# ictnlp/StreamSpeech

Measured on AMD Instinct MI355X. Metric: real-time factor (RTFx = audio seconds / wall seconds) + utterances/sec, offline S2ST fr-en, higher is better.
Workload: dtype f32

## Files before the change

### include/streamspeech_hip.h

```cpp
#ifndef STREAMSPEECH_HIP_H
#define STREAMSPEECH_HIP_H

#include <stddef.h>
#include <stdint.h>

#ifdef __cplusplus
extern "C" {
#endif

#define SS_ABI_VERSION 2

typedef struct ss_model ss_model;
typedef struct ss_vocoder ss_vocoder;
typedef struct ss_scratch ss_scratch;
typedef struct ss_stream_pool ss_stream_pool;

typedef struct ss_config {
  int32_t input_feat, conv_channels, conv_kernel;
  int32_t enc_dim, enc_ffn, enc_heads, enc_layers, dw_kernel;
  int32_t src_vocab, tgt_vocab;
  int32_t mt_layers, dec_dim, dec_ffn, dec_heads;
  int32_t t2u_layers, unit_layers, unit_vocab, ctc_upsample;
  int32_t pad, eos, unk;
  int32_t max_rel_pos;
// ... 155 lines not shown
int ss_flac_unpack(const uint8_t* h_data, size_t n_bytes, int64_t cap, int32_t* h_res, ss_flac_subframe* h_rec, int64_t res_cap,
                   ss_flac_info* h_info);
int ss_flac_restore_host(const int32_t* h_res, const ss_flac_subframe* h_rec, int64_t n_rec, const ss_flac_file* h_files, int n_files,
                         int mono, float* h_out, int32_t* h_pcm);
int ss_flac_restore(void* stream, const int32_t* d_res, const ss_flac_subframe* d_rec, int64_t n_rec, int64_t n_res,
                    const ss_flac_file* h_files, int n_files, int mono, float* d_out, int64_t out_floats,
                    void* d_work, size_t* work_bytes);

enum { SS_PCM_F32LE = 0, SS_PCM_S16LE = 1, SS_PCM_ULAW = 2, SS_PCM_ALAW = 3 };

typedef struct ss_pcm_seg {
  int64_t src_offset;
  int64_t dst_offset;
  int32_t frames;
  int32_t fmt, channels, dst;
} ss_pcm_seg;

int ss_pcm_scatter(void* stream, const void* d_stage, int64_t stage_bytes, const ss_pcm_seg* h_segs, int n_segs,
                   float* const* h_dst, const int64_t* h_dst_cap, int n_dst);
int ss_pcm_pack_s16(void* stream, const float* d_src, int64_t n, int16_t* d_out);
int ss_pcm_decode_host(const void* h_src, int fmt, int channels, int64_t frames, float* h_dst);
int ss_pcm_pack_s16_host(const float* h_src, int64_t n, int16_t* h_out);

typedef struct ss_pcm_emit_seg {
  float* carry;
  const float* tail;
  const float* taps;
  int64_t n_before;
  int64_t k0, k1;
  int64_t out_offset;
  int32_t carry_len;
  int32_t n_new;
  int32_t up, down, half;
  int32_t fmt;
  int32_t finished;
  int32_t reserved;
} ss_pcm_emit_seg;

int64_t ss_pcm_emit_count(int64_t n, int up, int down, int half, int finished);
int ss_pcm_emit(void* stream, const ss_pcm_emit_seg* h_segs, int n_segs, void* d_out, int64_t out_bytes);
int ss_pcm_emit_host(const ss_pcm_emit_seg* h_segs, int n_segs, void* h_out, int64_t out_bytes);
int ss_pcm_encode_host(const float* h_src, int64_t n, int fmt, void* h_out);

enum { SS_VAD_IDLE = 0, SS_VAD_SPEECH = 1 };
enum { SS_VAD_START = 1, SS_VAD_END = 2, SS_VAD_FORCED = 4 };

typedef struct ss_vad_state {
  int64_t onset;
  int64_t last_speech;
  int64_t utt_first_frame;
  float floor;
  int32_t mode;
  int32_t run;
  int32_t reserved;
} ss_vad_state;

typedef struct ss_vad_seg {
  const float* hist;
  ss_vad_state* state;
  float* powers;
  int64_t hist_first;
  int64_t n_hist;
  int64_t first_frame;
  int32_t n_frames;
  int32_t H, W;
  float p_abs, p_min, snr, rise;
  int32_t min_speech, end_silence, post_roll, max_frames;
  int32_t reserved;
} ss_vad_seg;

typedef struct ss_vad_result {
  int64_t consumed;
  int64_t start_frame;
  int64_t cut_sample;
  int64_t last_speech;
  int32_t events;
  int32_t mode;
} ss_vad_result;

int ss_vad_scan(void* stream, const ss_vad_seg* h_segs, int n_segs, ss_vad_result* d_results);
int ss_vad_scan_host(const ss_vad_seg* h_segs, int n_segs, ss_vad_result* h_results);

int ss_row_max_logprob(void* stream, const float* d_logits, int rows, int vocab, int mask0, int mask1, int mask2,
                       float* d_out);

int ss_log_softmax(void* stream, const float* d_logits, int rows, int vocab, int mask0, int mask1, int as_probs,
                   float* d_out);

int ss_encoder_out_len(int T);
int ss_encoder_forward(ss_model* m, void* stream, const float* d_fbank, int T, int attn_chunk,
                       int conv_chunk, float* d_enc_out);

int ss_encoder_stream_reset(ss_model* m);
int ss_encoder_stream_set_tail(ss_model* m, int unsettled_fbank_frames);
int ss_encoder_stream_forward(ss_model* m, void* stream, const float* d_fbank, int T, int attn_chunk,
                              int conv_chunk, float* d_enc_out, int32_t* n_final, int32_t* n_computed);
int ss_encoder_stream_set_deferred(ss_model* m, int on);
int ss_encoder_stream_status(ss_model* m, void* stream, int32_t* repeat);

int ss_stream_pool_create(ss_model* m, int max_sessions, int max_rows, ss_stream_pool** out);
void ss_stream_pool_destroy(ss_stream_pool* p);
int ss_stream_pool_reset(ss_stream_pool* p, int slot);
int ss_stream_pool_set_tail(ss_stream_pool* p, int slot, int unsettled_fbank_frames);
int ss_encoder_stream_forward_batch(ss_model* m, void* stream, ss_stream_pool* p, int n, const int32_t* h_slots,
                                    const float* const* h_fbank, const int32_t* h_T, const int32_t* h_attn_chunk,
                                    const int32_t* h_conv_chunk, float* d_enc_packed, int32_t* h_n_final, int32_t* h_n_computed);
int ss_stream_pool_ctc(ss_model* m, void* stream, ss_stream_pool* p, int head, int n, const int32_t* h_slots,
                       const float* d_enc_packed, int32_t* d_raw, int32_t* d_tokens, int32_t* d_index, int32_t* d_counts);
int ss_stream_pool_set_scores(ss_stream_pool* p, int on);
int ss_stream_pool_ctc_scored(ss_model* m, void* stream, ss_stream_pool* p, int head, int n, const int32_t* h_slots,
                              const float* d_enc_packed, int32_t* d_raw, int32_t* d_tokens, int32_t* d_index, int32_t* d_counts,
                              float* d_lprob, int32_t* d_last, float* d_tok_lprob);
int ss_stream_pool_stats(ss_stream_pool* p, int64_t* launches, int64_t* head_rows);

int ss_ctc_greedy(ss_model* m, void* stream, int head, const float* d_enc_out, int Tp,
                  int32_t* d_raw, int32_t* d_tokens, int32_t* d_index, int32_t* d_count,
                  float* d_logits);

int ss_ctc_greedy_scored(ss_model* m, void* stream, int head, const float* d_enc_out, int Tp,
                         int32_t* d_raw, int32_t* d_tokens, int32_t* d_index, int32_t* d_count,
                         float* d_logits, float* d_lprob, int32_t* d_last, float* d_tok_lprob);

int ss_mt_set_persistent(ss_model* m, int workgroups);
int ss_mt_get_persistent(ss_model* m);

int ss_mt_begin(ss_model* m, void* stream, const float* d_enc_out, int Tp);
int ss_mt_append(ss_model* m, void* stream, const int32_t* d_tokens, int n, int pos0, int ban_eos,
                 int force_eos, float* d_feats, int32_t* d_next, int n_tail_pad);
int ss_mt_greedy(ss_model* m, void* stream, const float* d_enc_out, int Tp, const int32_t* h_prefix,
                 int n_prefix, int max_len, int min_len, int32_t* h_out_tokens, int* h_n_out,
                 float* d_feats, int* h_n_feats);
int ss_mt_truncate(ss_model* m, int len);

int ss_t2u_units(ss_model* m, void* stream, const float* d_mt_feats, int n, int t2u_causal,
                 int mask_eos, int32_t* d_raw, int32_t* d_tokens, int32_t* d_count, float* d_logits,
                 int n_tail_pad);

int ss_vocoder_create(const ss_vocoder_config* cfg, const float* d_blob, size_t blob_floats,
                      const char* const* names, const int64_t* offsets, const int64_t* numels,
                      int n_slots, ss_vocoder** out);
void ss_vocoder_destroy(ss_vocoder* v);
int ss_vocoder_set_bf16x3(ss_vocoder* v, int on);
int ss_vocoder_set_f16(ss_vocoder* v, int on);
int ss_vocoder_forward(ss_vocoder* v, void* stream, const int32_t* d_codes, int K, int dur_prediction,
                       const int32_t* d_forced_dur, float* d_wav, int64_t wav_capacity,
                       int32_t* d_dur, int64_t* h_n_samples);
int ss_vocoder_num_speakers(const ss_vocoder* v);
int ss_vocoder_forward_spkr(ss_vocoder* v, void* stream, const int32_t* d_codes, int K, int dur_prediction,
                            const int32_t* d_forced_dur, float* d_wav, int64_t wav_capacity,
                            int32_t* d_dur, int64_t* h_n_samples, int32_t spkr);

int ss_batch_fbank_cmvn(ss_model* m, void* stream, int B, const float* d_pcm, const int64_t* h_pcm_start,
                        const int32_t* h_n_samples, float pcm_scale, float* d_feat, int32_t* h_T);
int ss_batch_cmvn(ss_model* m, void* stream, const float* d_in, int64_t rows, float* d_out);
int ss_batch_encoder_forward(ss_model* m, void* stream, int B, const float* d_fbank, const int32_t* h_T,
                             int attn_chunk, int conv_chunk, float* d_enc_out, int32_t* h_Tp);
int ss_batch_ctc_greedy(ss_model* m, void* stream, int head, int B, const float* d_enc_out,
                        const int32_t* h_Tp, int32_t* d_raw, int32_t* d_tokens, int32_t* d_index,
                        int32_t* d_counts);
int ss_batch_ctc_greedy_scored(ss_model* m, void* stream, int head, int B, const float* d_enc_out,
                               const int32_t* h_Tp, int32_t* d_raw, int32_t* d_tokens, int32_t* d_index,
                               int32_t* d_counts, float* d_lprob, int32_t* d_last, float* d_tok_lprob);
typedef struct ss_ctc_align_result {
  double score;
  double viterbi;
  int32_t status;
  int32_t n_tokens;
} ss_ctc_align_result;
#define SS_CTC_ALIGN_MAX_FRAMES 1500
#define SS_CTC_ALIGN_MAX_LABELS 1500
int ss_batch_ctc_align(ss_model* m, void* stream, int head, int B, const float* d_enc_out, const int32_t* h_Tp,
                       const int32_t* h_targets, const int32_t* h_n_targets, ss_ctc_align_result* d_results, int32_t* d_path,
                       int32_t* d_first, int32_t* d_last, float* d_tok_lprob);
int ss_ctc_align_host(const float* h_logits, int ld, int V, int pad, int B, const int32_t* h_T, const int32_t* h_targets,
                      const int32_t* h_n_targets, ss_ctc_align_result* h_results, int32_t* h_path, int32_t* h_first, int32_t* h_last,
                      float* h_tok_lprob, float* h_frame_lprob);
int ss_batch_mt_greedy(ss_model* m, void* stream, int B, const float* d_enc_out, const int32_t* h_Tp,
                       const int32_t* h_max_len, int min_len, int32_t* h_out_tokens, int out_stride,
                       int32_t* h_n_out, float* d_feats, int feat_rows);
int ss_batch_mt_beam(ss_model* m, void* stream, int B, int beam, const float* d_enc_out, const int32_t* h_Tp,
                     const int32_t* h_max_len, int min_len, float unk_penalty, int normalize, int32_t* h_out_tokens,
                     int out_stride, int32_t* h_n_out, float* h_scores, float* h_pos_scores, float* d_feats, int feat_rows);
int ss_batch_mt_continue(ss_model* m, void* stream, int B, const float* d_enc_out, const int32_t* h_Tp, const int32_t* h_prefix,
                         const int32_t* h_n_prefix, const int32_t* h_max_len, int min_len, int32_t* h_out_tokens, int out_stride,
                         int32_t* h_n_out, float* d_feats, int feat_rows, int32_t* h_n_feats);
int ss_batch_mt_continue_plan(int B, const int32_t* h_Tp, const int32_t* h_prefix, const int32_t* h_n_prefix, const int32_t* h_max_len,
                              int min_len, int out_stride, int feat_rows, int max_tgt_pos, int vocab, int eos, int32_t* h_dims,
                              int32_t* h_tables, int64_t tables_cap, int64_t* h_n_tables);
int ss_batch_mt_beam_continue(ss_model* m, void* stream, int B, int beam, const float* d_enc_out, const int32_t* h_Tp,
                              const int32_t* h_prefix, const int32_t* h_n_prefix, const int32_t* h_max_len, int min_len,
                              float unk_penalty, int normalize, int32_t* h_out_tokens, int out_stride, int32_t* h_n_out,
                              float* h_scores, float* h_pos_scores, float* d_feats, int feat_rows);
int ss_batch_mt_beam_continue_plan(int B, int beam, const int32_t* h_Tp, const int32_t* h_prefix, const int32_t* h_n_prefix,
                                   const int32_t* h_max_len, int min_len, int out_stride, int feat_rows, int max_tgt_pos, int vocab,
                                   int eos, int pad, int32_t* h_dims, int32_t* h_tables, int64_t tables_cap, int64_t* h_n_tables);
typedef struct ss_mt_search_opts {
  int32_t size;
  int32_t no_repeat_ngram;
  float len_penalty;
  float temperature;
} ss_mt_search_opts;
int ss_batch_mt_beam_opts(ss_model* m, void* stream, int B, int beam, const float* d_enc_out, const int32_t* h_Tp,
                          const int32_t* h_max_len, int min_len, float unk_penalty, int normalize, int32_t* h_out_tokens,
                          int out_stride, int32_t* h_n_out, float* h_scores, float* h_pos_scores, float* d_feats, int feat_rows,
                          const ss_mt_search_opts* opts);
int ss_batch_mt_beam_continue_opts(ss_model* m, void* stream, int B, int beam, const float* d_enc_out, const int32_t* h_Tp,
                                   const int32_t* h_prefix, const int32_t* h_n_prefix, const int32_t* h_max_len, int min_len,
                                   float unk_penalty, int normalize, int32_t* h_out_tokens, int out_stride, int32_t* h_n_out,
                                   float* h_scores, float* h_pos_scores, float* d_feats, int feat_rows,
                                   const ss_mt_search_opts* opts);
int ss_batch_mt_beam_continue_plan_opts(int B, int beam, const int32_t* h_Tp, const int32_t* h_prefix, const int32_t* h_n_prefix,
                                        const int32_t* h_max_len, int min_len, int out_stride, int feat_rows, int max_tgt_pos,
                                        int vocab, int eos, int pad, int32_t* h_dims, int32_t* h_tables, int64_t tables_cap,
                                        int64_t* h_n_tables, const ss_mt_search_opts* opts);
typedef struct ss_mt_sample_opts {
  int32_t size;
  int32_t topk;
  float topp;
  int32_t reserved;
  uint64_t seed;
} ss_mt_sample_opts;
int ss_batch_mt_sample(ss_model* m, void* stream, int B, int beam, const float* d_enc_out, const int32_t* h_Tp,
                       const int32_t* h_max_len, int min_len, float unk_penalty, int normalize, int32_t* h_out_tokens, int out_stride,
                       int32_t* h_n_out, float* h_scores, float* h_pos_scores, float* d_feats, int feat_rows,
                       const ss_mt_search_opts* opts, const int64_t* h_keys, const ss_mt_sample_opts* sample);
int ss_batch_mt_sample_continue(ss_model* m, void* stream, int B, int beam, const float* d_enc_out, const int32_t* h_Tp,
                                const int32_t* h_prefix, const int32_t* h_n_prefix, const int32_t* h_max_len, int min_len,
                                float unk_penalty, int normalize, int32_t* h_out_tokens, int out_stride, int32_t* h_n_out,
                                float* h_scores, float* h_pos_scores, float* d_feats, int feat_rows, const ss_mt_search_opts* opts,
                                const int64_t* h_keys, const ss_mt_sample_opts* sample);
int ss_batch_fbank_frames(ss_model* m, void* stream, int B, const float* const* h_pcm, const int32_t* h_first, const int32_t* h_n,
                          float pcm_scale, float* const* h_feat);
int ss_batch_fbank_frames_sr(ss_model* m, void* stream, int B, const float* const* h_pcm, const int32_t* h_n_in, const int32_t* h_up,
                             const int32_t* h_down, const float* const* h_taps, const int32_t* h_half_len, const int32_t* h_first,
                             const int32_t* h_n, float pcm_scale, float* const* h_feat);
int ss_fbank_sr_rows(int64_t n_in, int up, int down, int half_len, int32_t* h_n_rows, int32_t* h_n_final);
int ss_fbank_mel_ranges(const float* h_melw, int rows, int cols, int32_t* h_lo_hi);
int ss_batch_t2u_units(ss_model* m, void* stream, int B, const float* d_feats, int feat_rows,
                       const int32_t* h_n, int t2u_causal, int mask_eos, int32_t* d_raw, int32_t* d_tokens,
                       int32_t* d_counts);
int ss_batch_vocoder_forward(ss_vocoder* v, void* stream, int B, const int32_t* d_codes, const int32_t* h_K,
                             int dur_prediction, const int32_t* d_forced_dur, float* d_wav,
                             int64_t wav_capacity, int32_t* d_dur, int64_t* h_wav_start,
                             int64_t* h_n_samples);
int ss_batch_vocoder_forward_spkr(ss_vocoder* v, void* stream, int B, const int32_t* d_codes, const int32_t* h_K,
                                  int dur_prediction, const int32_t* d_forced_dur, float* d_wav,
                                  int64_t wav_capacity, int32_t* d_dur, int64_t* h_wav_start,
                                  int64_t* h_n_samples, const int32_t* h_spkr );
int ss_batch_t2u_units_pad(ss_model* m, void* stream, int B, const float* d_feats, int feat_rows, const int32_t* h_n,
                           const int32_t* h_n_tail_pad, int t2u_causal, int mask_eos, int32_t* d_raw, int32_t* d_tokens,
                           int32_t* d_counts);
int ss_batch_mt_features(ss_model* m, void* stream, int B, const float* d_enc_out, const int32_t* h_Tp, const int32_t* h_tokens,
                         const int32_t* h_n_tokens, const int32_t* h_n_tail_pad, float* d_feats, int feat_rows);
int ss_batch_mt_attention(ss_model* m, void* stream, int B, const float* d_enc_out, const int32_t* h_Tp, const int32_t* h_tokens,
                          const int32_t* h_n_tokens, const int32_t* h_first, float* d_feats, int feat_rows, float* d_attn,
                          int64_t* h_attn_off, int64_t attn_capacity, int32_t* d_peak, float* d_stat);
int ss_batch_mt_score(ss_model* m, void* stream, int U, const float* d_enc_out, const int32_t* h_Tp, int B, const int32_t* h_src,
                      const int32_t* h_tokens, const int32_t* h_n_tokens, float* d_feats, int feat_rows, float* d_stat,
                      int32_t* d_idx);
int ss_batch_vocoder_tail(ss_vocoder* v, void* stream, int B, const int32_t* d_codes, const int32_t* h_K, const int32_t* h_n_new,
                          const int32_t* h_ctx, const int32_t* h_rf, int dur_prediction, float* d_out, int64_t out_capacity,
                          int32_t* h_win_first, int32_t* h_dur, int64_t* h_out_start, int64_t* h_n_out);
int ss_batch_vocoder_tail_spkr(ss_vocoder* v, void* stream, int B, const int32_t* d_codes, const int32_t* h_K, const int32_t* h_n_new,
                               const int32_t* h_ctx, const int32_t* h_rf, int dur_prediction, float* d_out, int64_t out_capacity,
                               int32_t* h_win_first, int32_t* h_dur, int64_t* h_out_start, int64_t* h_n_out,
                               const int32_t* h_spkr );

int ss_batch_unit_spans(ss_model* m, void* stream, int B, const int32_t* d_raw, const int32_t* h_n, const int32_t* h_K,
                        const int32_t* h_dur_first, const int32_t* h_unit0, const int32_t* d_dur, const int32_t* h_dur,
                        int32_t* h_spans, int32_t* h_K_out);
int ss_unit_spans_host(int B, const int32_t* h_raw, const int32_t* h_n, const int32_t* h_K, const int32_t* h_dur_first,
                       const int32_t* h_unit0, const int32_t* h_dur, int up, int blank, int pad, int bos, int eos, int32_t* h_spans,
                       int32_t* h_K_out);

int ss_prof_enable(int cls_mask);
int ss_prof_enable_hi(int cls_mask);
int ss_prof_reset(void);
int ss_prof_read(int cls, double* h_ms_total, double* h_flops_total, int64_t* h_launches,
                 double* h_bytes_total);
int ss_prof_totals(int cls, double* h_flops_total, double* h_bytes_total, int64_t* h_launches);
int ss_prof_read_issued(int cls, double* h_issued_flops_total);
int ss_prof_shape_log(int on);
int ss_prof_shape_dump(char* buf, int cap);
int ss_prof_num_classes(void);
const char* ss_prof_class_name(int cls);

int ss_model_set_pack_invariant(ss_model* m, int on);
int ss_model_get_pack_invariant(ss_model* m);
int ss_debug_canon(int mode);

int ss_debug_last_logits(ss_model* m, void* stream, float* d_out, int64_t cap_floats, int* h_rows, int* h_cols);

int ss_op_ffn_fused(void* stream, const float* dX, int ldx, float* dY, int ldy, const float* ln_g, const float* ln_b,
                    const float* dW1, const float* db1, const float* dW2, const float* db2, float alpha,
                    const float* ln2_g, const float* ln2_b, int M, int D, int F);
int ss_debug_ffn(int grid, int row_tiles_per_wave, int enable);
int ss_debug_rtlin(int grid, int enable);
int ss_debug_rtlin_kb(int uw, int order);
int ss_debug_rtlin_kb_last(int32_t out[4]);
int ss_debug_unit_l0_distinct(int on);
int ss_debug_fbank_dense(int dense);
int ss_debug_conv_c64(int enable);
int ss_debug_conv_c256_rows(int rows);
int ss_debug_conv_c32(int enable);
int ss_debug_conv_c16(int enable);
int64_t ss_debug_enc_step_launches(void);
int ss_op_ln_linear(void* stream, const float* dX, int ldx, const float* ln_g, const float* ln_b, const float* dW,
                    const float* dbias, const float* dR, int ldr, float* dC, int ldc, int M, int N, int K, int act, float alpha,
                    int glu);
int ss_op_ln_linear_ex(void* stream, const float* dX, int ldx, const float* ln_g, const float* ln_b, float* ln_out, const float* dW,
                       const float* dbias, const float* dR, int ldr, float* dC, int ldc, int M, int N, int K, int act, float alpha,
                       int glu, int canon);

int ss_debug_force_tile(int bm, int bn, int ks);
int ss_debug_sk_errors(void);
int ss_debug_attention_split(int v);
int ss_debug_attention_q16(int v);
int ss_debug_enc_step_inject_timeout(ss_model* m);
int ss_debug_scratch_audit(ss_scratch* sc, size_t* booked, size_t* held);
int ss_debug_mt_inject_timeout(ss_model* m);

int ss_op_conv_gemm(void* stream, const float* dA, int lda, const float* dW, const float* dbias,
                    const float* dR, int ldr, const float* dR2, int ldr2, float* dC, int ldc,
                    int M, int N, int Cin, int taps, int dil, int stride, int pad, int in_len,
                    int chunk, int in_act, float in_slope, int act, float alpha, float div, int glu);
typedef struct ss_op_conv_args {
  const float* A; const float* W; const float* bias; const float* R; const float* R2; float* C; float* C2;
  int32_t lda, ldc, ldr, ldr2, ldc2;
  int32_t M, N, Cin, taps, dil, stride, pad, in_len, chunk;
  int32_t in_act; float in_slope;
  int32_t act; float act_slope, alpha, div, c2_slope;
  int32_t glu;
  const int32_t* segs; int32_t nseg, max_seg_out;
  int32_t same_rows;
} ss_op_conv_args;
int ss_op_conv_gemm_ex(void* stream, const ss_op_conv_args* a);
int ss_op_conv_gemm_rows(void* stream, const ss_op_conv_args* a, int m_begin, const int32_t* seg_mb, const float* const* seg_A, int canon);
int ss_op_conv_pair(void* stream, const float* dA, int lda, const float* dW1, const float* db1, const float* dW2, const float* db2,
                    float* dC, int ldc, const float* dR2, int ldr2, float div, float* dC2, int ldc2, float c2_slope, int C, int taps,
                    int dil, int M, int in_len, float slope, const int32_t* d_segs, int nseg);
int ss_op_resblock_fused(void* stream, const float* dX, int ldx, const float* const* dW1, const float* const* dB1,
                         const float* const* dW2, const float* const* dB2, const int32_t* dil, float* dY, int ldy, const float* dR2,
                         int ldr2, float div, int C, int taps, int M, float slope, const int32_t* d_segs, int nseg);
int ss_debug_slab(int grid, long long min_rows);
int ss_op_conv_f16(void* stream, const float* dA, const float* dW, const float* dbias, const float* dR, const float* dR2,
                   float* dC, float* dC2, int M, int C, int taps, int dil, int in_act, float in_slope, int act, float div,
                   const int32_t* d_segs, int nseg);
int ss_op_layernorm(void* stream, const float* dx, int ldx, float* dy, int ldy, const float* dg,
                    const float* db, int M, int D, float eps);
int ss_op_attention(void* stream, const float* dQ, int ldq, const float* dK, int ldk, const float* dV,
                    int ldv, float* dO, int ldo, int Tq, int Tk, int H, float scale, int causal,
                    int chunk, const float* dP, int ldp, const float* du, const float* dv);
typedef struct ss_op_attn_args {
  const float* Q; const float* K; const float* V; float* O;
  int32_t ldq, ldk, ldv, ldo;
  int32_t Tq, Tk, H;
  float scale;
  int32_t causal, chunk, q0, k_mask_tail;
  const float* P; int32_t ldp;
  const float* bias_u; const float* bias_v;
  const int32_t* segs; int32_t nseg, max_q, p_tmax;
  const int32_t* seg_tail;
  int32_t no_decode_kernel;
  const int32_t* anc; int32_t anc_ld, anc_slots;
  int32_t use_split;
} ss_op_attn_args;
int ss_op_attention_ex(void* stream, const ss_op_attn_args* a);
typedef struct ss_op_attn_probs_args {
  const float* Q; const float* K;
  int32_t ldq, ldk, H;
  float scale;
  const int32_t* segs; int32_t nseg;
  const int32_t* q_first; const int32_t* row_off; const int64_t* p_off;
  float* P; int32_t* peak; float* stat;
  int32_t max_rows;
} ss_op_attn_probs_args;
int ss_op_attention_probs(void* stream, const ss_op_attn_probs_args* a);
typedef struct ss_op_pool_attn_args {
  const float* Qs; float* cache; float* O;
  int32_t ld, ldo, slot_rows;
  const float* P; int32_t ldp, p_tmax;
  const float* bias_u; const float* bias_v;
  const int32_t* sess; const int32_t* qt_pre;
  int32_t nsess, qtiles, H;
  float scale;
} ss_op_pool_attn_args;
int ss_op_attention_pool(void* stream, const ss_op_pool_attn_args* a);
int ss_debug_attention_no_mfma(int v);
int ss_op_dwconv_bn_silu(void* stream, const float* dx, int ldx, float* dy, int ldy, const float* dwt,
                         int K, const float* mean, const float* var, const float* gamma,
                         const float* beta, float eps, int T, int C, int chunk);
int ss_op_dwconv_bn_silu_ex(void* stream, const float* dx, int ldx, float* dy, int ldy, const float* dwt, int K, const float* mean,
                            const float* var, const float* gamma, const float* beta, float eps, int T, int C, int chunk,
                            const int32_t* segs, int nseg, int t_begin);
int ss_op_pool_dwconv(void* stream, const float* gs, float* cache, int slot_rows, float* y, const float* wt, int K, const float* bn_mean,
                      const float* bn_var, const float* bn_gamma, const float* bn_beta, float bn_eps, int C, const int32_t* sess,
                      int nsess, int max_n);
int ss_op_pool_gather_rows(void* stream, float* out, const float* stk, float* cache, int slot_rows, int W, const int32_t* tab,
                           const int32_t* pre, int nsess, int total);
int ss_op_pool_gather_ids(void* stream, int32_t* out, const int32_t* stk, int32_t* cache, int slot_rows, const int32_t* tab,
                          const int32_t* pre, int nsess, int total);
int ss_op_pool_stack_rows(void* stream, float* out, const float* enc, int W, const int32_t* src, const int32_t* pre, int nsess,
                          int total);

int ss_op_masked_argmax(void* stream, const float* logits, int ld, int M, int N, int mask0, int mask1, int mask2, int force,
                        int32_t* ids, const int32_t* row_max_len, int step, int force_id, const int32_t* row_min_len, int ban_id);
int ss_op_ctc_collapse(void* stream, const int32_t* raw, int T, int blank, int pad, int32_t* tokens, int32_t* index, int32_t* count,
                       const int32_t* segs, int nseg);
int ss_op_masked_argmax_lprob(void* stream, const float* logits, int ld, int M, int N, int mask0, int mask1, int mask2, int32_t* ids,
                              float* lprob);
int ss_op_ctc_collapse_spans(void* stream, const int32_t* raw, const float* lprob, int T, int blank, int pad, int32_t* tokens,
                             int32_t* index, int32_t* last, float* tok_lprob, int32_t* count, const int32_t* segs, int nseg);
int ss_op_mt_token_scores(void* stream, const float* d_logits, int ld, int rows, int V, const int32_t* d_target, float* d_stat,
                          int32_t* d_idx);
int ss_debug_mt_score_form(int force_strided);
int ss_op_ctc_align(void* stream, const float* d_logits, int ld, int V, int pad, int B, const int32_t* h_T, const int32_t* h_targets,
                    const int32_t* h_n_targets, ss_ctc_align_result* d_results, int32_t* d_path, int32_t* d_first, int32_t* d_last,
                    float* d_tok_lprob, float* d_frame_lprob);
int ss_op_unit_spans(void* stream, int B, const int32_t* d_raw, const int32_t* h_n, const int32_t* h_K, const int32_t* h_dur_first,
                     const int32_t* h_unit0, const int32_t* d_dur, int up, int blank, int pad, int bos, int eos, int32_t* d_spans,
                     int32_t* d_K_out);
int ss_op_dur_predict(void* stream, const float* logdur, const int32_t* forced, int K, int32_t* dur, int32_t* cum,
                      const int32_t* segs, int nseg);
int ss_op_repeat_rows(void* stream, const float* emb, const int32_t* cum, int K, int D, float* out, int F, const int32_t* segs,
                      int nseg);
int ss_op_embed_tokens(void* stream, const int32_t* tok, const float* emb, const float* pos_table, float scale, int pos0, float* out,
                       int n, int D, int pos_stride, int pad_id, int vocab);
int ss_op_embed_tokens_rows(void* stream, const int32_t* tok, const float* emb, const float* pos_table, int pos_rows, float scale,
                            int pos0, const int32_t* row_pos, float* out, int n, int D, int pad_id, int vocab);
int ss_op_upsample_add_pos(void* stream, const float* src, int n, int up, const float* pos_row, float pad_value, float* out, int D);
int ss_op_gather_rows(void* stream, const int32_t* idx, const float* table, int D, float* out, int n, int rows);
int ss_op_scatter_rows(void* stream, const int32_t* dst_row, const float* src, int lds, float* dst, int ldd, int D, int n,
                       int dst_rows);
int ss_op_conv_post_tanh(void* stream, const float* x, int T, int C, const float* w, const float* bias, float slope, float* wav,
                         const int32_t* segs, int nseg);
int ss_op_conv_post_tanh_crop(void* stream, const float* x, int C, const float* w, const float* bias, float slope, float* wav,
                              const int32_t* segs, int nseg, int max_keep);
int ss_op_spkr_pre_add(void* stream, const float* x, float* y, int ld, int C0, const float* table, const int32_t* spkr, int spkr0,
                       const int32_t* segs, int nseg, int max_seg_out, int M, int act, float slope);

#define SS_OP_BEAM_CAND 64
int ss_op_beam_topk(void* stream, const float* logits, int R, int V, int k, int t_step, int min_len, const int32_t* max_len,
                    const int32_t* npre, const int32_t* done, const float* cum, int pad, int unk, int eos, float unk_pen,
                    float* cand_s, int32_t* cand_t);
typedef struct ss_op_beam_state {
  int32_t* tok; float* cum; int32_t* anc; float* cand_s; int32_t* cand_t; int32_t* ignore; int32_t* done; int32_t* max_len;
  int32_t* npre;
  int32_t* fin_cnt; float* fin_score; int32_t* fin_len; int32_t* fin_tok; float* fin_pos; int32_t* fin_anc;
} ss_op_beam_state;
int ss_op_beam_merge(void* stream, const ss_op_beam_state* st, int B, int k, int Lc, int V, int t_step, int c0, int eos,
                     int normalize);
int ss_op_beam_prefix_score(void* stream, const float* logits, int rows, int V, const int32_t* ftok, int pad, int unk, float unk_pen,
                            float* lp);
int ss_op_beam_prefix_chain(void* stream, const float* lp, const int32_t* row0, const int32_t* npre, int B, int k, float* cum0,
                            float* pos);
int ss_op_beam_topk_opts(void* stream, const float* logits, int R, int V, int k, int t_step, int min_len, const int32_t* max_len,
                         const int32_t* npre, const int32_t* done, const float* cum, int pad, int unk, int eos, float unk_pen,
                         float* cand_s, int32_t* cand_t, float temperature, int no_repeat_ngram, const int32_t* tok,
                         const int32_t* anc, int Lc, int c0, const int32_t* ptok, const int32_t* row0, float* row_scores);
int ss_op_beam_merge_opts(void* stream, const ss_op_beam_state* st, int B, int k, int Lc, int V, int t_step, int c0, int eos,
                          int normalize, float len_penalty);
int ss_op_beam_prefix_score_opts(void* stream, const float* logits, int rows, int V, const int32_t* ftok, int pad, int unk,
                                 float unk_pen, float* lp, float temperature);
int ss_op_sample_step(void* stream, const float* logits, int R, int V, int t_step, int min_len, const int32_t* max_len,
                      const int32_t* npre, int pad, int unk, int eos, float unk_pen, float temperature, int no_repeat_ngram,
                      const int32_t* tok, const int32_t* anc, int Lc, int c0, const int32_t* ptok, const int32_t* row0,
                      const int32_t* row_j, const int64_t* keys, const ss_mt_sample_opts* sample, int32_t* out_tok, float* out_score,
                      float* out_u, int32_t* out_kept);
int ss_op_sample_uniform(void* stream, int n, const uint64_t* seed, const int64_t* key, const int32_t* step, const int32_t* j,
                         float* u, uint32_t* words);

#ifdef __cplusplus
}
#endif
#endif
```

### streamspeech_amd/csrc/conv_c64w.hip

```cpp
#include "slab_common.hpp"

#include <type_traits>

namespace ss {

using u32x4 = __attribute__((ext_vector_type(4))) unsigned;

#ifndef CW_TIMING
#define CW_TIMING 0
#endif
#if CW_TIMING
__device__ unsigned long long g_cw_dbg[1024 * 8];
#define CW_STAMP(k) do { if (t == 0) { const unsigned long long _n = __builtin_amdgcn_s_memtime(); cw_acc[k] += _n - cw_last; cw_last = _n; } } while (0)
#else
#define CW_STAMP(k) do { } while (0)
#endif

namespace {
constexpr int CW_MAXSEG = 256;
constexpr int CW_MAXROWS = 320;
constexpr int CW_MAXROWS_128 = 192;
[[maybe_unused]] constexpr int CW_NUM_RECORDS = 0x7ffffff0;
constexpr int cw_bme(int dil, int rows = 256) { return rows == 128 ? (dil == 1 ? 128 : dil == 3 ? 126 : 120) : (dil == 1 ? 256 : dil == 3 ? 252 : 240); }
[[maybe_unused]] __host__ __device__ constexpr int cw_nc(int kind) { return kind == 0 ? 4 : kind == 1 ? 2 : 3; }
// ... 43 lines not shown
  const int t = threadIdx.x, lane = t & 63;
  const int wave = __builtin_amdgcn_readfirstlane((t >> 6) & (ROWS == 128 ? 1 : 3));
  const int cs = CH <= 64 ? 0 : __builtin_amdgcn_readfirstlane(ROWS == 128 ? t >> 7 : t >> 8);
  const int colh = CH == 256 && ROWS == 256 ? (int)((blockIdx.x >> 3) & 1) : 0;
  const int col0 = colh * 128 + cs * 64;
  const int r = lane & 15, g = lane >> 4;
  const int Kw = groups * 4 * C;

  SlabWalk<GemmArgs> w(p, s_blk, BME);
  __syncthreads();
  const int nblocks = w.nblocks();
  const float slope = p.in_act == ACT_LRELU ? p.in_slope : 1.0f;

  const __amdgpu_buffer_rsrc_t rsW = __builtin_amdgcn_make_buffer_rsrc((void*)p.W, 0, CW_NUM_RECORDS, 0x00020000);
  const int vo = (r * Kw + 4 * g) * 4;
  auto wload = [&](int idx, int cc, int ct, int kh) -> f32x4 {
    const int so = __builtin_amdgcn_readfirstlane(((col0 + ct * 16) * Kw + idx * C + kh * CS + cc * 16) * 4);
    const u32x4 v = __builtin_amdgcn_raw_buffer_load_b128(rsW, vo, so, 0);
    return f32x4{__uint_as_float(v[0]), __uint_as_float(v[1]), __uint_as_float(v[2]), __uint_as_float(v[3])};
  };

  constexpr bool HALVES = CH == 256 && ROWS == 256;
  int blk = HALVES ? (int)((blockIdx.x & 7) + 8 * (blockIdx.x >> 4)) : (int)blockIdx.x;
  const int blk_stride = HALVES ? (int)(gridDim.x >> 1) : (int)gridDim.x;
  if (blk >= nblocks) return;
  f32x4 ring[RING];
#pragma unroll
  for (int q = 0; q < RING; ++q) ring[q] = wload(q / CT, 0, q % CT, 0);

  int toff[2];
  bool pv[2];
#pragma unroll
  for (int i = 0; i < 2; ++i) {
    const int pp = wave * 32 + i * 16 + r;
    pv[i] = pp < NPAIR;
    const int pc = pv[i] ? pp : NPAIR - 1;
    toff[i] = 2 * DIL * (pc / DIL) + pc % DIL;
  }

#if CW_TIMING
  unsigned long long cw_acc[4] = {0, 0, 0, 0}, cw_last = __builtin_amdgcn_s_memtime(), cw_begin = cw_last, cw_blocks = 0;
#endif
  for (; blk < nblocks; blk += blk_stride) {
#if CW_TIMING
    ++cw_blocks;
#endif
    w.locate(blk, p.in_len);
    const int m0 = w.m0, seg_lo = w.seg_lo, seg_hi = w.seg_hi;
    const int m_hi = p.nseg > 0 ? seg_hi : min(seg_hi, p.M);
    const bool edge = (m0 - p.pad < seg_lo) || (m0 - p.pad + slab_rows > seg_hi);
    const int row_hi = ROWS == 128 ? min(seg_hi, m0 - p.pad + slab_rows) : seg_hi;
    f32x4 acc[4][2][CT];
#pragma unroll
    for (int f = 0; f < 4; ++f)
#pragma unroll
      for (int i = 0; i < 2; ++i)
#pragma unroll
        for (int j = 0; j < CT; ++j) acc[f][i][j] = f32x4{0.f, 0.f, 0.f, 0.f};
#pragma unroll 1
    for (int kh = 0; kh < KH; ++kh) {
    const int kh_wrap = kh + 1 < KH ? kh + 1 : 0;
    __syncthreads();
    CW_STAMP(kh == 0 ? 3 : 1);
#pragma unroll 1
    for (int u0 = 0; u0 < NP && (ROWS != 128 || u0 * RPP < slab_rows); u0 += NPC) {
      f32x4 pre[NPC];
#pragma unroll
      for (int u = 0; u < NPC; ++u) {
        const int rho = t / TPR + RPP * (u0 + u);
        const int gc = min(max(m0 - p.pad + rho, seg_lo), row_hi - 1);
        pre[u] = *reinterpret_cast<const f32x4*>(p.A + (size_t)gc * p.lda + kh * CS + (t % TPR) * 4);
      }
      float* dst = sA + (t / TPR + RPP * u0) * LDA + (t % TPR) * 4;
#pragma unroll
      for (int u = 0; u < NPC; ++u) {
        const int rho = t / TPR + RPP * (u0 + u);
        f32x4 v = pre[u];
        if (edge) {
          const int gin = m0 - p.pad + rho;
          const bool ok = gin >= seg_lo && gin < seg_hi;
#pragma unroll
          for (int e = 0; e < 4; ++e) v[e] = ok ? v[e] : 0.f;
        }
#pragma unroll
        for (int e = 0; e < 4; ++e) v[e] = fmaxf(v[e], v[e] * slope);
        if (rho < slab_rows) *reinterpret_cast<f32x4*>(dst + u * RPP * LDA) = v;
      }
    }
    __syncthreads();
    CW_STAMP(0);

    const float* pa0 = sA + toff[0] * LDA + 4 * g;
    const float* pa1 = sA + toff[1] * LDA + 4 * g;
    auto rd = [&](const float* base, int j, int cc) -> f32x4 { return *reinterpret_cast<const f32x4*>(base + j * DIL * LDA + cc * 16); };
    auto xform = [&](int op, const f32x4 a, const f32x4 b) -> f32x4 { return op == 1 ? a + b : op == 0 ? a : a - b; };
    f32x4 xa[2];
    xa[0] = xform(-1, rd(pa0, 0, 0), rd(pa0, 2, 0));
    xa[1] = xform(-1, rd(pa1, 0, 0), rd(pa1, 2, 0));
    auto group = [&](auto KIND, const int grp, const int kind_next, const float* pn0, const float* pn1, const int grp_next, const int kh_next) __attribute__((always_inline)) {
      constexpr int K = decltype(KIND)::value, NC = cw_nc(K), NS = CB * NC;
      static_assert(NS % 2 == 0 && NS >= 2, "ring slots keep their parity across groups");
#pragma unroll
      for (int ss = 0; ss < NS; ++ss) {
        const int slot = cw_slot(K, ss % NC);
        f32x4 na0, nb0, na1, nb1;
        if (ss + 1 < NS) {
          const int ccn = (ss + 1) / NC, nn = (ss + 1) % NC;
          na0 = rd(pa0, cw_ja(K, nn), ccn); nb0 = rd(pa0, cw_jb(K, nn), ccn);
          na1 = rd(pa1, cw_ja(K, nn), ccn); nb1 = rd(pa1, cw_jb(K, nn), ccn);
        } else {
          const int jb = kind_next == 0 ? 2 : 1;
          na0 = rd(pn0, 0, 0); nb0 = *reinterpret_cast<const f32x4*>(pn0 + jb * (DIL * LDA));
          na1 = rd(pn1, 0, 0); nb1 = *reinterpret_cast<const f32x4*>(pn1 + jb * (DIL * LDA));
        }
        f32x4 wf[CT];
#pragma unroll
        for (int j = 0; j < CT; ++j) {
          const int q = ss * CT + j;
          wf[j] = ring[q % RING];
          const int s2 = ss + 2;
          if (s2 < NS) ring[q % RING] = wload(grp * 4 + cw_slot(K, s2 % NC), s2 / NC, j, kh);
          else ring[q % RING] = wload(grp_next * 4 + (s2 == NS ? 0 : (kind_next == 1 ? 3 : 1)), 0, j, kh_next);
        }
#pragma unroll
        for (int e = 0; e < 4; ++e)
#pragma unroll
          for (int i = 0; i < 2; ++i)
#pragma unroll
            for (int j = 0; j < CT; ++j)
              acc[slot][i][j] = __builtin_amdgcn_mfma_f32_16x16x4f32(wf[j][e], xa[i][e], acc[slot][i][j], 0, 0, 0);
        if (ss + 1 < NS) {
          xa[0] = xform(cw_op(K, (ss + 1) % NC), na0, nb0);
          xa[1] = xform(cw_op(K, (ss + 1) % NC), na1, nb1);
        } else {
          xa[0] = kind_next == 1 ? na0 : na0 - nb0;
          xa[1] = kind_next == 1 ? na1 : na1 - nb1;
        }
        __builtin_amdgcn_sched_barrier(0);
      }
    };
    constexpr int tail = TAIL;
    const int groups_full = groups - (tail ? 1 : 0);
#pragma unroll 1
    for (int grp = 0; grp < groups_full; ++grp) {
      const bool more = grp + 1 < groups;
      const float* pn0 = more ? pa0 + 3 * DIL * LDA : pa0;
      const float* pn1 = more ? pa1 + 3 * DIL * LDA : pa1;
      group(std::integral_constant<int, 0>{}, grp, (more && grp + 1 == groups_full) ? tail : 0, pn0, pn1, more ? grp + 1 : 0, more ? kh : kh_wrap);
      pa0 = pn0;
      pa1 = pn1;
    }
    if constexpr (TAIL == 1) group(std::integral_constant<int, 1>{}, groups_full, 0, pa0, pa1, 0, kh_wrap);
    if constexpr (TAIL == 2) group(std::integral_constant<int, 2>{}, groups_full, 0, pa0, pa1, 0, kh_wrap);
    CW_STAMP(1);
    }

    int le = lane;
    asm volatile("" : "+v"(le));
    const int g_e = le >> 4;
    const int cole = col0 + g_e * 4;
    f32x4 y[4 * CT];
    int mrow[4];
#pragma unroll
    for (int i = 0; i < 2; ++i) {
#pragma unroll
      for (int j = 0; j < CT; ++j) {
        y[(i * 2) * CT + j] = (acc[0][i][j] + acc[1][i][j]) + acc[2][i][j];
        y[(i * 2 + 1) * CT + j] = (acc[1][i][j] - acc[2][i][j]) - acc[3][i][j];
      }
      mrow[i * 2] = m0 + toff[i];
      mrow[i * 2 + 1] = m0 + toff[i] + DIL;
    }
#pragma unroll
    for (int n = 0; n < 4 * CT; ++n) asm volatile("" : "+v"(y[n]));
    f32x4 bb[CT];
#pragma unroll
    for (int j = 0; j < CT; ++j) bb[j] = f32x4{0.f, 0.f, 0.f, 0.f};
    if (p.bias) {
#pragma unroll
      for (int j = 0; j < CT; ++j) bb[j] = *reinterpret_cast<const f32x4*>(p.bias + cole + j * 16);
    }
    slab_epi_batch(p, y, bb, [&](int q, int n) -> size_t {
      return (size_t)min(mrow[n / CT], m_hi - 1) * (q == 0 ? p.ldr : p.ldr2) + cole + (n % CT) * 16;
    });
#pragma unroll
    for (int q = 0; q < 4; ++q) {
      if (pv[q / 2] && mrow[q] < m_hi) {
#pragma unroll
        for (int j = 0; j < CT; ++j) slab_epi_store<CH >= 128>(p, mrow[q], cole + j * 16, y[q * CT + j]);
      }
    }
    CW_STAMP(2);
  }
#if CW_TIMING
  if (t == 0) {
    unsigned long long* d = g_cw_dbg + (size_t)(blockIdx.x & 1023) * 8;
    d[0] = cw_acc[0]; d[1] = cw_acc[1]; d[2] = cw_acc[2]; d[3] = cw_acc[3]; d[4] = cw_blocks; d[5] = cw_begin; d[6] = __builtin_amdgcn_s_memtime(); d[7] = 1;
  }
#endif
#endif
}

#if CW_TIMING
extern "C" int ss_debug_cw_timing(unsigned long long* h_out, int cap_wgs) {
  const int n = cap_wgs < 1024 ? cap_wgs : 1024;
  if (hipMemcpyFromSymbol(h_out, HIP_SYMBOL(g_cw_dbg), (size_t)n * 8 * sizeof(unsigned long long)) != hipSuccess) return -1;
  static unsigned long long zeros[1024 * 8];
  (void)hipMemcpyToSymbol(HIP_SYMBOL(g_cw_dbg), zeros, sizeof(zeros));
  return n;
}
#endif

void conv_c64w_debug(int enable) { if (enable >= 0) dispatch_edit([enable](Dispatch& d) { d.c64w_on = enable ? 1 : 0; }); }
bool conv_c64w_enabled() { return disp().c64w_on != 0; }
void conv_c128w_debug(int enable) { if (enable >= 0) dispatch_edit([enable](Dispatch& d) { d.c128w_on = enable ? 1 : 0; }); }
bool conv_c128w_enabled() { return disp().c128w_on != 0; }

void conv_c256w_debug(int enable) { if (enable >= 0) dispatch_edit([enable](Dispatch& d) { d.c256w_on = enable ? 1 : 0; }); }
bool conv_c256w_enabled() { return disp().c256w_on != 0; }

static int cw_groups(const GemmArgs& a) { return (a.taps + 2) / 3; }
static size_t cw_lds(const GemmArgs& a, int ch, int rows = 256) { return slab_lds_bytes(cw_bme(a.dil, rows) + 3 * cw_groups(a) * a.dil, ch + 4, CW_MAXSEG); }
static bool cw_rows128(const GemmArgs& a) {
  return disp().c256w_rows == 128 && cw_bme(a.dil, 128) + 3 * cw_groups(a) * a.dil <= CW_MAXROWS_128;
}

bool conv_c64w_eligible(const GemmArgs& a) {
  if (!disp().c64w_on || !a.Wwino || a.taps < disp().c64w_min_k || a.taps < 3 || (a.dil != 1 && a.dil != 3 && a.dil != 5) || a.C2) return false;
  if (a.pad != a.dil * (a.taps - 1) / 2) return false;
  if (a.taps <= 8 && a.taps > 3 && a.dil == 5) return false;
  const int slab_rows = cw_bme(a.dil) + 3 * cw_groups(a) * a.dil;
  return slab_rows <= CW_MAXROWS && 2 * cw_lds(a, 64) <= 158 * 1024 && (size_t)cw_groups(a) * 4 * 64 * 64 * 4 < 0x7ff00000ull;
}

bool conv_wide_winograd_eligible(const GemmArgs& a, int ch) {
  if (ch != 128 && ch != 256) return false;
  const Dispatch& d = disp();
  if (!(ch == 128 ? d.c128w_on : d.c256w_on) || !a.Wwino || !slab_conv_ok(a, ch)) return false;
  if (a.taps < 3 || (a.dil != 1 && a.dil != 3 && a.dil != 5) || a.pad != a.dil * (a.taps - 1) / 2) return false;
  if (a.nseg > CW_MAXSEG || a.M < (ch == 128 ? d.c128w_min_rows : d.c256w_min_rows) || !slab_rows_ok(a.M)) return false;
  if (ch == 256 && (size_t)256 * cw_groups(a) * 4 * 256 * 4 >= 0x7ff00000ull) return false;
  if (ch == 256 && cw_rows128(a)) return cw_lds(a, 128, 128) <= 160 * 1024;
  const int slab_rows = cw_bme(a.dil) + 3 * cw_groups(a) * a.dil;
  return slab_rows <= CW_MAXROWS && cw_lds(a, 128) <= 160 * 1024;
}

int launch_wino_pack(const float* W, float* WW, int C, int taps, hipStream_t stream) {
  const int groups = (taps + 2) / 3, n = C * groups * C;
  hipLaunchKernelGGL(wino_pack_kernel, dim3((n + 255) / 256), dim3(256), 0, stream, W, WW, C, taps, groups);
  SS_LAUNCH_CHECK();
  return SS_OK;
}

template <int DIL, int CH, int TAIL, int ROWS = 256>
static int launch_cw_t(GemmArgs a, hipStream_t stream) {
  if constexpr (CH == 256 && ROWS == 256) {
    if (cw_rows128(a)) return launch_cw_t<DIL, CH, TAIL, 128>(a, stream);
  }
  constexpr int BME = cw_bme(DIL, ROWS);
  const int groups = cw_groups(a);
  const int slab_rows = BME + 3 * groups * DIL;
  const size_t lds = cw_lds(a, CH == 256 ? 128 : CH, ROWS);
  SS_MAX_LDS_ONCE((&conv_c64w_kernel<DIL, CH, TAIL, ROWS>), CH >= 128 ? 160 * 1024 : 96 * 1024);
  SkWorkspace* st = nullptr;
  int rc = sk_workspace_acquire(stream, &st);
  if (rc != SS_OK) return rc;
  int grid = slab_grid(CH >= 128 ? 1 : CH == 64 ? 2 : 3, st->cus, a.M, BME, a.nseg);
  if (CH == 256 && ROWS == 256) {
    long long want = std::min<long long>(st->cus, 2 * ((slab_max_blocks(a.M, BME, a.nseg) + 7) / 8 * 8));
    if (disp().slab_grid_cap > 0) want = std::min<long long>(want, disp().slab_grid_cap);
    grid = (int)std::max<long long>(16, want / 16 * 16);
  }
  ProfRec rec{}; bool prof = false;
  rc = prof_begin(a, stream, CH == 64 ? PROF_CONV_C64W : CH == 128 ? PROF_CONV_C128W : CH == 256 ? PROF_CONV_C256W : PROF_CONV_C32W, rec, prof);
  if (rc != SS_OK) return rc;
  a.W = a.Wwino;
  hipLaunchKernelGGL((conv_c64w_kernel<DIL, CH, TAIL, ROWS>), dim3(grid), dim3(CH >= 128 ? 512 : 256), lds, stream, a, groups, slab_rows);
  SS_LAUNCH_CHECK();
  return prof_end(stream, rec, prof);
}

template <int CH>
static int launch_cw(const GemmArgs& a, hipStream_t stream) {
  if (a.in_act != ACT_NONE && a.in_act != ACT_LRELU) return SS_ERR_ARG;
  const int key = a.dil * 10 + a.taps % 3;
  switch (key) {
    case 10: return launch_cw_t<1, CH, 0>(a, stream);
    case 11: return launch_cw_t<1, CH, 1>(a, stream);
    case 12: return launch_cw_t<1, CH, 2>(a, stream);
    case 30: return launch_cw_t<3, CH, 0>(a, stream);
    case 31: return launch_cw_t<3, CH, 1>(a, stream);
    case 32: return launch_cw_t<3, CH, 2>(a, stream);
    case 50: return launch_cw_t<5, CH, 0>(a, stream);
    case 51: return launch_cw_t<5, CH, 1>(a, stream);
    case 52: return launch_cw_t<5, CH, 2>(a, stream);
    default: return SS_ERR_ARG;
  }
}

int launch_conv_c64w(const GemmArgs& a, hipStream_t stream) {
  if (!conv_c64_eligible(a) || !conv_c64w_eligible(a)) return SS_ERR_ARG;
  return launch_cw<64>(a, stream);
}
void conv_c32w_debug(int enable) { if (enable >= 0) dispatch_edit([enable](Dispatch& d) { d.c32w_on = enable ? 1 : 0; }); }
bool conv_c32w_enabled() { return disp().c32w_on != 0; }
bool conv_c32w_eligible(const GemmArgs& a) {
  if (!disp().c32w_on || !a.Wwino || a.taps < 3 || (a.dil != 1 && a.dil != 3 && a.dil != 5) || a.C2) return false;
  if (a.pad != a.dil * (a.taps - 1) / 2) return false;
  const int slab_rows = cw_bme(a.dil) + 3 * cw_groups(a) * a.dil;
  return slab_rows <= CW_MAXROWS && 3 * cw_lds(a, 32) <= 158 * 1024;
}
int launch_conv_c32w(const GemmArgs& a, hipStream_t stream) {
  if (!conv_c32_eligible(a) || !conv_c32w_eligible(a)) return SS_ERR_ARG;
  return launch_cw<32>(a, stream);
}
int launch_conv_c128w(const GemmArgs& a, hipStream_t stream) {
  if (!conv_wide_winograd_eligible(a, 128)) return SS_ERR_ARG;
  return launch_cw<128>(a, stream);
}
int launch_conv_c256w(const GemmArgs& a, hipStream_t stream) {
  if (!conv_wide_winograd_eligible(a, 256)) return SS_ERR_ARG;
  return launch_cw<256>(a, stream);
}

}
```

### streamspeech_amd/csrc/debug_ops.hip

```cpp
#include "model_internal.hpp"
#include "ctc_align.hpp"

static int op_bind_wino(GemmArgs& a, void* stream) {
  static thread_local std::map<hipStream_t, DevBuf> wino_tmps;
  DevBuf& wino_tmp = wino_tmps[(hipStream_t)stream];
  const int N = a.N, Cin = a.Cin, taps = a.taps;
  if ((conv_c64w_enabled() && N == 64 && Cin == 64 && taps >= 3 && conv_c64_eligible(a)) ||
      (conv_c128w_enabled() && N == 128 && Cin == 128 && taps >= 3 && a.same_rows && !a.glu) ||
      (conv_c256w_enabled() && N == 256 && Cin == 256 && taps >= 3 && a.same_rows && !a.glu) ||
      (conv_c32w_enabled() && N == 32 && Cin == 32 && taps >= 3 && conv_c32_eligible(a))) {
    RET(wino_tmp.ensure((size_t)N * ((taps + 2) / 3) * 4 * N * sizeof(float)));
    RET(launch_wino_pack(a.W, wino_tmp.f(), N, taps, (hipStream_t)stream));
    a.Wwino = wino_tmp.f();
  }
  return SS_OK;
}

extern "C" int ss_op_conv_gemm(void* stream, const float* dA, int lda, const float* dW, const float* dbias,
                               const float* dR, int ldr, const float* dR2, int ldr2, float* dC, int ldc, int M,
                               int N, int Cin, int taps, int dil, int stride, int pad, int in_len, int chunk,
                               int in_act, float in_slope, int act, float alpha, float div, int glu) {
  GemmArgs a;
  a.A = dA; a.lda = lda; a.W = dW; a.bias = dbias; a.R = dR; a.ldr = ldr; a.R2 = dR2; a.ldr2 = ldr2; a.C = dC; a.ldc = ldc;
  a.M = M; a.N = N; a.Cin = Cin; a.taps = taps; a.dil = dil; a.stride = stride; a.pad = pad; a.in_len = in_len;
  a.chunk = chunk; a.in_act = in_act; a.in_slope = in_slope; a.act = act; a.alpha = alpha; a.div = div; a.glu = glu;
  a.same_rows = (stride == 1 && M == in_len) ? 1 : 0;
  RET(op_bind_wino(a, stream));
  return launch_conv_gemm(a, (hipStream_t)stream);
}

static void op_fill_conv(GemmArgs& a, const ss_op_conv_args* x) {
  a.A = x->A; a.W = x->W; a.bias = x->bias; a.R = x->R; a.R2 = x->R2; a.C = x->C; a.C2 = x->C2;
  a.lda = x->lda; a.ldc = x->ldc; a.ldr = x->ldr; a.ldr2 = x->ldr2; a.ldc2 = x->ldc2;
  a.M = x->M; a.N = x->N; a.Cin = x->Cin; a.taps = x->taps; a.dil = x->dil; a.stride = x->stride; a.pad = x->pad;
  a.in_len = x->in_len; a.chunk = x->chunk;
  a.in_act = x->in_act; a.in_slope = x->in_slope; a.act = x->act; a.act_slope = x->act_slope; a.alpha = x->alpha; a.div = x->div;
  a.c2_slope = x->c2_slope; a.glu = x->glu;
  a.segs = x->segs; a.nseg = x->nseg; a.max_seg_out = x->max_seg_out; a.same_rows = x->same_rows;
}
extern "C" int ss_op_conv_gemm_ex(void* stream, const ss_op_conv_args* x) {
  if (!x) return SS_ERR_ARG;
  GemmArgs a;
  op_fill_conv(a, x);
  if (a.W && a.N > 0 && a.taps > 0) RET(op_bind_wino(a, stream));
  return launch_conv_gemm(a, (hipStream_t)stream);
}
extern "C" int ss_op_conv_gemm_rows(void* stream, const ss_op_conv_args* x, int m_begin, const int32_t* seg_mb,
                                    const float* const* seg_A, int canon) {
  if (!x || canon < 0 || canon > 2) return SS_ERR_ARG;
  GemmArgs a;
  op_fill_conv(a, x);
  a.m_begin = m_begin; a.seg_mb = seg_mb; a.seg_A = seg_A; a.canon = canon;
  if (a.W && a.N > 0 && a.taps > 0) RET(op_bind_wino(a, stream));
  return launch_conv_gemm(a, (hipStream_t)stream);
}
extern "C" int ss_op_conv_pair(void* stream, const float* dA, int lda, const float* dW1, const float* db1, const float* dW2,
                               const float* db2, float* dC, int ldc, const float* dR2, int ldr2, float div, float* dC2, int ldc2,
                               float c2_slope, int Cch, int taps, int dil, int M, int in_len, float slope, const int32_t* d_segs,
                               int nseg) {
  return launch_conv_pair(dA, lda, dW1, db1, dW2, db2, dC, ldc, dR2, ldr2, div, dC2, ldc2, c2_slope, Cch, taps, dil, M, in_len, slope,
                          d_segs, nseg, (hipStream_t)stream);
}
extern "C" int ss_op_resblock_fused(void* stream, const float* dX, int ldx, const float* const* dW1, const float* const* dB1,
                                    const float* const* dW2, const float* const* dB2, const int32_t* dil, float* dY, int ldy,
                                    const float* dR2, int ldr2, float div, int Cch, int taps, int M, float slope,
                                    const int32_t* d_segs, int nseg) {
  if (!dW1 || !dB1 || !dW2 || !dB2 || !dil) return SS_ERR_ARG;
  return launch_resblock_fused(dX, ldx, dW1, dB1, dW2, dB2, dil, dY, ldy, dR2, ldr2, div, Cch, taps, M, slope, d_segs, nseg,
                               (hipStream_t)stream);
}
extern "C" int ss_debug_slab(int grid, long long min_rows) {
  if (grid < 0) return SS_ERR_ARG;
  slab_debug(grid, min_rows);
  return SS_OK;
}

extern "C" int ss_op_conv_f16(void* stream, const float* dA, const float* dW, const float* dbias, const float* dR, const float* dR2,
                              float* dC, float* dC2, int M, int Cch, int taps, int dil, int in_act, float in_slope, int act, float div,
                              const int32_t* d_segs, int nseg) {
  if (!dA || !dW || !dC || M <= 0 || taps < 1 || dil < 1 || nseg < 0 || (nseg > 0 && !d_segs)) return SS_ERR_ARG;
  if (!(Cch == 64 || Cch == 128 || Cch == 256)) return SS_ERR_ARG;
  static thread_local std::map<hipStream_t, DevBuf> f16_tmps;
  DevBuf& wh = f16_tmps[(hipStream_t)stream];
  RET(wh.ensure(f16_pack_halves(Cch, taps) * sizeof(uint16_t)));
  RET(launch_f16_pack(dW, wh.p, Cch, taps, (hipStream_t)stream));
  GemmArgs a;
  a.A = dA; a.lda = Cch; a.W = dW; a.Wf16 = wh.p; a.bias = dbias; a.R = dR; a.ldr = Cch; a.R2 = dR2; a.ldr2 = Cch;
  a.C = dC; a.ldc = Cch; a.C2 = dC2; a.ldc2 = Cch; a.c2_slope = 0.1f;
  a.M = M; a.N = Cch; a.Cin = Cch; a.taps = taps; a.dil = dil; a.stride = 1; a.pad = dil * (taps - 1) / 2; a.in_len = M;
  a.same_rows = 1; a.in_act = in_act; a.in_slope = in_slope; a.act = act; a.act_slope = 0.1f; a.div = div;
  a.segs = d_segs; a.nseg = nseg;
  return launch_conv_f16(a, (hipStream_t)stream);
}

extern "C" int ss_debug_last_logits(ss_model* m, void* stream, float* d_out, int64_t cap_floats, int* h_rows, int* h_cols) {
  if (!m || !h_rows || !h_cols) return SS_ERR_ARG;
  *h_rows = m->sc->dbg_rows; *h_cols = m->sc->dbg_cols;
  if (!d_out) return SS_OK;
  if (!m->sc->dbg_logits || cap_floats < (int64_t)m->sc->dbg_rows * m->sc->dbg_cols) return SS_ERR_CAPACITY;
  SS_HIP_CHECK(hipMemcpyAsync(d_out, m->sc->dbg_logits, (size_t)m->sc->dbg_rows * m->sc->dbg_cols * sizeof(float), hipMemcpyDeviceToDevice,
                              (hipStream_t)stream));
  return SS_OK;
}

extern "C" int ss_op_ffn_fused(void* stream, const float* dX, int ldx, float* dY, int ldy, const float* ln_g, const float* ln_b,
                               const float* dW1, const float* db1, const float* dW2, const float* db2, float alpha,
                               const float* ln2_g, const float* ln2_b, int M, int D, int F) {
  return launch_ffn_fused(dX, ldx, dY, ldy, ln_g, ln_b, dW1, db1, dW2, db2, alpha, ln2_g, ln2_b, M, D, F, (hipStream_t)stream,
                          canon_mode() == CANON_SEQ);
}
extern "C" int ss_debug_canon(int mode) {
  if (mode < 0 || mode > 2) return SS_ERR_ARG;
  canon_debug_set(mode);
  return SS_OK;
}
extern "C" int ss_op_ln_linear(void* stream, const float* dX, int ldx, const float* ln_g, const float* ln_b, const float* dW,
                               const float* dbias, const float* dR, int ldr, float* dC, int ldc, int M, int N, int K, int act,
                               float alpha, int glu) {
  GemmArgs a;
  a.A = dX; a.lda = ldx; a.W = dW; a.bias = dbias; a.R = dR; a.ldr = ldr; a.C = dC; a.ldc = ldc;
  a.M = M; a.N = N; a.Cin = K; a.in_len = M; a.act = act; a.alpha = alpha; a.glu = glu; a.same_rows = 1;
  a.ln_g = ln_g; a.ln_b = ln_b;
  return launch_conv_gemm(a, (hipStream_t)stream);
}
extern "C" int ss_op_ln_linear_ex(void* stream, const float* dX, int ldx, const float* ln_g, const float* ln_b, float* ln_out,
                                  const float* dW, const float* dbias, const float* dR, int ldr, float* dC, int ldc, int M, int N, int K,
                                  int act, float alpha, int glu, int canon) {
  if (canon < 0 || canon > 2 || (ln_g == nullptr) != (ln_b == nullptr) || (ln_out && !ln_g)) return SS_ERR_ARG;
  GemmArgs a;
  a.A = dX; a.lda = ldx; a.W = dW; a.bias = dbias; a.R = dR; a.ldr = ldr; a.C = dC; a.ldc = ldc;
  a.M = M; a.N = N; a.Cin = K; a.in_len = M; a.act = act; a.alpha = alpha; a.glu = glu; a.same_rows = 1;
  a.ln_g = ln_g; a.ln_b = ln_b; a.ln_out = ln_out; a.canon = canon;
  return launch_conv_gemm(a, (hipStream_t)stream);
}
extern "C" int ss_debug_conv_c64(int enable) {
  if (enable == 4 || enable == 5) { conv_c64w_debug(enable == 5); return SS_OK; }
  if (enable == 6 || enable == 7) { conv_c128w_debug(enable == 7); return SS_OK; }
  if (enable == 8 || enable == 9) { conv_c256w_debug(enable == 9); return SS_OK; }
  conv_c64_debug(enable);
  return SS_OK;
}
extern "C" int ss_debug_conv_c256_rows(int rows) { return conv_c256w_rows_debug(rows); }
extern "C" int ss_debug_conv_c32(int enable) {
  if (enable == 4 || enable == 5) { conv_c32w_debug(enable == 5); return SS_OK; }
  conv_c32_debug(enable);
  return SS_OK;
}
extern "C" int ss_debug_conv_c16(int enable) { conv_c16_debug(enable); return SS_OK; }
extern "C" int64_t ss_debug_enc_step_launches(void) { return (int64_t)enc_step_launch_count(); }
extern "C" int ss_debug_scratch_audit(ss_scratch* sc, size_t* booked, size_t* held) {
  if (!sc || !booked || !held) return SS_ERR_ARG;
  size_t sum = 0;
  bool foreign = false;
  for (DevBuf* b : sc->all()) {
    sum += b->bytes;
    if (b->acct != &sc->acct) foreign = true;
  }
  *booked = sc->acct.used;
  *held = sum;
  return foreign ? SS_ERR_ARG : SS_OK;
}
extern "C" int ss_debug_rtlin(int grid, int enable) {
  if (grid < 0) return SS_ERR_ARG;
  rtlin_debug(grid, enable);
  return SS_OK;
}
extern "C" int ss_debug_rtlin_kb(int uw, int order) {
  if (!(uw == 0 || uw == 1 || uw == 2 || uw == 4) || order < -1 || order > 2) return SS_ERR_ARG;
  rtlin_kb_debug(uw, order);
  return SS_OK;
}
extern "C" int ss_debug_rtlin_kb_last(int32_t out[4]) {
  if (!out) return SS_ERR_ARG;
  int v[4];
  rtlin_kb_last(v);
  for (int i = 0; i < 4; ++i) out[i] = v[i];
  return SS_OK;
}
extern "C" int ss_debug_unit_l0_distinct(int on) {
  if (on < -1 || on > 1) return SS_ERR_ARG;
  dispatch_edit([on](Dispatch& d) { d.unit_l0_distinct = on < 0 ? (getenv("SS_UNIT_L0_DISTINCT") ? atoi(getenv("SS_UNIT_L0_DISTINCT")) != 0 : 1) : on; });
  return SS_OK;
}
extern "C" int ss_debug_fbank_dense(int dense) {
  if (dense < -1 || dense > 1) return SS_ERR_ARG;
  dispatch_edit([dense](Dispatch& d) { d.fbank_dense = dense < 0 ? (getenv("SS_FBANK_DENSE") ? atoi(getenv("SS_FBANK_DENSE")) != 0 : 0) : dense; });
  return SS_OK;
}
extern "C" int ss_debug_ffn(int grid, int row_tiles_per_wave, int enable) {
  if (grid < 0 || row_tiles_per_wave < -1 || row_tiles_per_wave > 4) return SS_ERR_ARG;
  ffn_fused_debug_grid(grid);
  ffn_fused_debug_rows(row_tiles_per_wave);
  if (enable >= 0) dispatch_edit([enable](Dispatch& d) { d.ffn_fusion = enable ? 1 : 0; });
  return SS_OK;
}

extern "C" int ss_op_layernorm(void* stream, const float* dx, int ldx, float* dy, int ldy, const float* dg,
                               const float* db, int M, int D, float eps) {
  return launch_layernorm(dx, ldx, dy, ldy, dg, db, M, D, eps, (hipStream_t)stream);
}

extern "C" int ss_op_masked_argmax(void* stream, const float* logits, int ld, int M, int N, int mask0, int mask1, int mask2, int force,
                                   int32_t* ids, const int32_t* row_max_len, int step, int force_id, const int32_t* row_min_len,
                                   int ban_id) {
  return launch_masked_argmax(logits, ld, M, N, mask0, mask1, mask2, force, ids, (hipStream_t)stream, row_max_len, step, force_id,
                              row_min_len, ban_id);
}
extern "C" int ss_op_ctc_collapse(void* stream, const int32_t* raw, int T, int blank, int pad, int32_t* tokens, int32_t* index,
                                  int32_t* count, const int32_t* segs, int nseg) {
  return launch_ctc_collapse(raw, T, blank, pad, tokens, index, count, (hipStream_t)stream, segs, nseg);
}
extern "C" int ss_op_masked_argmax_lprob(void* stream, const float* logits, int ld, int M, int N, int mask0, int mask1, int mask2,
                                         int32_t* ids, float* lprob) {
  return launch_masked_argmax_lprob(logits, ld, M, N, mask0, mask1, mask2, ids, lprob, (hipStream_t)stream);
}
static int g_mt_score_form = 0;
extern "C" int ss_debug_mt_score_form(int v) { g_mt_score_form = v ? 1 : 0; return SS_OK; }
extern "C" int ss_op_mt_token_scores(void* stream, const float* d_logits, int ld, int rows, int V, const int32_t* d_target,
                                     float* d_stat, int32_t* d_idx) {
  return launch_mt_token_scores(d_logits, ld, rows, V, d_target, d_stat, d_idx, (hipStream_t)stream, g_mt_score_form);
}
extern "C" int ss_op_ctc_collapse_spans(void* stream, const int32_t* raw, const float* lprob, int T, int blank, int pad, int32_t* tokens,
                                        int32_t* index, int32_t* last, float* tok_lprob, int32_t* count, const int32_t* segs, int nseg) {
  return launch_ctc_collapse_spans(raw, lprob, T, blank, pad, tokens, index, last, tok_lprob, count, (hipStream_t)stream, segs, nseg);
}
extern "C" int ss_op_ctc_align(void* stream, const float* d_logits, int ld, int V, int pad, int B, const int32_t* h_T,
                               const int32_t* h_targets, const int32_t* h_n_targets, ss_ctc_align_result* d_results, int32_t* d_path,
                               int32_t* d_first, int32_t* d_last, float* d_tok_lprob, float* d_frame_lprob) {
  if (!d_logits || ld < V || !d_results) return SS_ERR_ARG;
  CtcAlignPlan plan;
  RET(ctc_align_plan(V, pad, B, h_T, h_targets, h_n_targets, plan));
  if (plan.labels > 0 && (!d_first || !d_last || !d_tok_lprob)) return SS_ERR_ARG;
  static thread_local std::map<hipStream_t, std::pair<DevBuf, DevBuf>> tmps;
  auto& tmp = tmps[(hipStream_t)stream];
  RET(tmp.first.ensure(ctc_align_table_bytes(plan)));
  RET(tmp.second.ensure(plan.work_bytes()));
  return launch_ctc_align(d_logits, ld, V, plan, h_targets, tmp.first.p, tmp.second.p, d_results, d_path, d_first, d_last, d_tok_lprob,
                          d_frame_lprob, (hipStream_t)stream);
}
extern "C" int ss_op_dur_predict(void* stream, const float* logdur, const int32_t* forced, int K, int32_t* dur, int32_t* cum,
                                 const int32_t* segs, int nseg) {
  return launch_dur_predict(logdur, forced, K, dur, cum, (hipStream_t)stream, segs, nseg);
}
extern "C" int ss_op_repeat_rows(void* stream, const float* emb, const int32_t* cum, int K, int D, float* out, int F,
                                 const int32_t* segs, int nseg) {
  return launch_repeat_rows(emb, cum, K, D, out, F, (hipStream_t)stream, segs, nseg);
}
extern "C" int ss_op_embed_tokens(void* stream, const int32_t* tok, const float* emb, const float* pos_table, float scale, int pos0,
                                  float* out, int n, int D, int pos_stride, int pad_id, int vocab) {
  return launch_embed_tokens(tok, emb, pos_table, scale, pos0, out, n, D, (hipStream_t)stream, pos_stride, pad_id, vocab);
}
extern "C" int ss_op_embed_tokens_rows(void* stream, const int32_t* tok, const float* emb, const float* pos_table, int pos_rows,
                                       float scale, int pos0, const int32_t* row_pos, float* out, int n, int D, int pad_id, int vocab) {
  return launch_embed_tokens_rows(tok, emb, pos_table, pos_rows, scale, pos0, row_pos, out, n, D, (hipStream_t)stream, pad_id, vocab);
}
extern "C" int ss_op_upsample_add_pos(void* stream, const float* src, int n, int up, const float* pos_row, float pad_value, float* out,
                                      int D) {
  return launch_upsample_add_pos(src, n, up, pos_row, pad_value, out, D, (hipStream_t)stream);
}
extern "C" int ss_op_gather_rows(void* stream, const int32_t* idx, const float* table, int D, float* out, int n, int rows) {
  return launch_gather_rows(idx, table, D, out, n, (hipStream_t)stream, rows);
}
extern "C" int ss_op_scatter_rows(void* stream, const int32_t* dst_row, const float* src, int lds, float* dst, int ldd, int D, int n,
                                  int dst_rows) {
  return launch_scatter_rows(dst_row, src, lds, dst, ldd, D, n, dst_rows, (hipStream_t)stream);
}
extern "C" int ss_op_conv_post_tanh(void* stream, const float* x, int T, int C, const float* w, const float* bias, float slope,
                                    float* wav, const int32_t* segs, int nseg) {
  return launch_conv_post_tanh(x, T, C, w, bias, slope, wav, (hipStream_t)stream, segs, nseg);
}
extern "C" int ss_op_conv_post_tanh_crop(void* stream, const float* x, int C, const float* w, const float* bias, float slope, float* wav,
                                         const int32_t* segs, int nseg, int max_keep) {
  return launch_conv_post_tanh_crop(x, C, w, bias, slope, wav, segs, nseg, max_keep, (hipStream_t)stream);
}
extern "C" int ss_op_spkr_pre_add(void* stream, const float* x, float* y, int ld, int C0, const float* table, const int32_t* spkr,
                                   int spkr0, const int32_t* segs, int nseg, int max_seg_out, int M, int act, float slope) {
  return launch_spkr_pre_add(x, y, ld, C0, table, spkr, spkr0, segs, nseg, max_seg_out, M, act, slope, (hipStream_t)stream);
}

static int op_attn_bind_split(AttnArgs& a) {
  static void* scratch = nullptr;
  if (!scratch) {
    SS_HIP_CHECK(hipMalloc(&scratch, attention_split_bytes()));
    SS_HIP_CHECK(hipMemset(scratch, 0, attention_split_bytes()));
  }
  attention_bind_split(a, scratch);
  return SS_OK;
}

extern "C" int ss_op_attention(void* stream, const float* dQ, int ldq, const float* dK, int ldk, const float* dV,
                               int ldv, float* dO, int ldo, int Tq, int Tk, int H, float scale, int causal, int chunk,
                               const float* dP, int ldp, const float* du, const float* dv) {
  AttnArgs a;
  a.Q = dQ; a.ldq = ldq; a.K = dK; a.ldk = ldk; a.V = dV; a.ldv = ldv; a.O = dO; a.ldo = ldo;
  a.Tq = Tq; a.Tk = Tk; a.H = H; a.scale = scale; a.causal = causal; a.chunk = chunk;
  a.P = dP; a.ldp = ldp; a.bias_u = du; a.bias_v = dv;
  if (dP) RET(op_attn_bind_split(a));
  return launch_attention(a, (hipStream_t)stream);
}

extern "C" int ss_op_attention_ex(void* stream, const ss_op_attn_args* x) {
  if (!x) return SS_ERR_ARG;
  AttnArgs a;
  a.Q = x->Q; a.K = x->K; a.V = x->V; a.O = x->O;
  a.ldq = x->ldq; a.ldk = x->ldk; a.ldv = x->ldv; a.ldo = x->ldo;
  a.Tq = x->Tq; a.Tk = x->Tk; a.H = x->H; a.scale = x->scale;
  a.causal = x->causal; a.chunk = x->chunk; a.q0 = x->q0; a.k_mask_tail = x->k_mask_tail;
  a.P = x->P; a.ldp = x->ldp; a.bias_u = x->bias_u; a.bias_v = x->bias_v;
  a.segs = x->segs; a.nseg = x->nseg; a.max_q = x->max_q; a.p_tmax = x->p_tmax;
  a.seg_tail = x->seg_tail;
  a.no_decode_kernel = x->no_decode_kernel;
  a.anc = x->anc; a.anc_ld = x->anc_ld; a.anc_slots = x->anc_slots;
  if (x->use_split) RET(op_attn_bind_split(a));
  return launch_attention(a, (hipStream_t)stream);
}

extern "C" int ss_op_attention_probs(void* stream, const ss_op_attn_probs_args* x) {
  if (!x) return SS_ERR_ARG;
  AttnProbsArgs a;
  a.Q = x->Q; a.K = x->K; a.ldq = x->ldq; a.ldk = x->ldk; a.H = x->H; a.scale = x->scale;
  a.segs = x->segs; a.nseg = x->nseg; a.q_first = x->q_first; a.row_off = x->row_off;
  a.p_off = reinterpret_cast<const long long*>(x->p_off);
  a.P = x->P; a.peak = x->peak; a.stat = x->stat; a.max_rows = x->max_rows;
  return launch_attention_probs(a, (hipStream_t)stream);
}

extern "C" int ss_op_attention_pool(void* stream, const ss_op_pool_attn_args* x) {
  if (!x) return SS_ERR_ARG;
  PoolAttnArgs a;
  a.Qs = x->Qs; a.cache = x->cache; a.O = x->O;
  a.ld = x->ld; a.ldo = x->ldo; a.slot_rows = x->slot_rows;
  a.P = x->P; a.ldp = x->ldp; a.p_tmax = x->p_tmax;
  a.bias_u = x->bias_u; a.bias_v = x->bias_v;
  a.sess = x->sess; a.qt_pre = x->qt_pre;
  a.nsess = x->nsess; a.qtiles = x->qtiles; a.H = x->H; a.scale = x->scale;
  return launch_attention_pool(a, (hipStream_t)stream);
}

extern "C" int ss_debug_attention_split(int v) { attention_debug_split(v); return SS_OK; }
extern "C" int ss_debug_attention_q16(int v) { attention_debug_q16(v); return SS_OK; }
extern "C" int ss_debug_attention_no_mfma(int v) { attention_debug_no_mfma(v); return SS_OK; }

extern "C" int ss_op_dwconv_bn_silu(void* stream, const float* dx, int ldx, float* dy, int ldy, const float* dwt,
                                    int K, const float* mean, const float* var, const float* gamma,
                                    const float* beta, float eps, int T, int C, int chunk) {
  return launch_dwconv_bn_silu(dx, ldx, dy, ldy, dwt, K, mean, var, gamma, beta, eps, T, C, chunk, (hipStream_t)stream);
}

extern "C" int ss_op_dwconv_bn_silu_ex(void* stream, const float* dx, int ldx, float* dy, int ldy, const float* dwt, int K,
                                       const float* mean, const float* var, const float* gamma, const float* beta, float eps, int T,
                                       int C, int chunk, const int32_t* segs, int nseg, int t_begin) {
  return launch_dwconv_bn_silu(dx, ldx, dy, ldy, dwt, K, mean, var, gamma, beta, eps, T, C, chunk, (hipStream_t)stream, segs, nseg,
                               t_begin);
}

extern "C" int ss_prof_enable(int cls_mask) { prof_enable(cls_mask); return SS_OK; }
extern "C" int ss_prof_enable_hi(int cls_mask) { prof_enable_hi(cls_mask); return SS_OK; }
extern "C" int ss_prof_reset(void) { prof_reset(); return SS_OK; }
extern "C" int ss_prof_read(int cls, double* ms, double* flops, int64_t* launches, double* bytes) {
  long long n = 0;
  int rc = prof_read(cls, ms, flops, &n, bytes);
  if (launches) *launches = n;
  return rc;
}
extern "C" int ss_prof_totals(int cls, double* flops, double* bytes, int64_t* launches) {
  long long n = 0;
  int rc = prof_totals(cls, flops, bytes, &n);
  if (launches) *launches = n;
  return rc;
}
extern "C" int ss_prof_read_issued(int cls, double* issued_flops) { return prof_read_issued(cls, issued_flops); }
extern "C" int ss_prof_shape_log(int on) { prof_shape_log(on); return SS_OK; }
extern "C" int ss_prof_shape_dump(char* buf, int cap) { return prof_shape_dump(buf, cap); }
extern "C" int ss_prof_num_classes(void) { return kNumTileCfg; }
extern "C" const char* ss_prof_class_name(int cls) { return prof_cfg_name(cls); }

extern "C" int ss_debug_force_tile(int bm, int bn, int ks) {
  if (!(bm >= 0 && bm <= 6) && bm != 32 && bm != 64 && bm != 128) return SS_ERR_ARG;
  if (bm == 6 || bm == 0) dispatch_edit([bm](Dispatch& d) { d.no_resblock_fusion = (bm == 6); });
  if (bm == 3 || bm == 0) dispatch_edit([bm](Dispatch& d) { d.no_pair_fusion = (bm == 3); });
  debug_force_tile((bm == 3 || bm == 6) ? 0 : bm, bn, ks);
  return SS_OK;
}
extern "C" int ss_debug_sk_errors(void) { return conv_sk_error_count() + conv_sk2_error_count() + g_mt_timeouts.load(std::memory_order_relaxed); }
```

### streamspeech_amd/csrc/dispatch.hip

```cpp
#include "gemm.hpp"

#include <atomic>
#include <cstdlib>
#include <map>
#include <mutex>
#include <utility>
#include <vector>

namespace ss {

namespace {
std::mutex g_disp_mu;
std::atomic<unsigned> g_disp_gen{1};
Dispatch env_defaults() {
  Dispatch d;
  auto I = [](const char* k, int dflt) { const char* e = getenv(k); return e ? atoi(e) : dflt; };
  auto L = [](const char* k, long long dflt) { const char* e = getenv(k); return e ? atoll(e) : dflt; };
  d.attn_split = I("SS_ATTN_NO_SPLIT", 0) ? -1 : 0; d.attn_q16 = I("SS_ATTN_Q16", d.attn_q16);
  d.c16_off = I("SS_NO_CONV_C16", 0) ? 1 : 0; d.c32_off = I("SS_NO_CONV_C32", 0) ? 1 : 0; d.c64_off = I("SS_NO_CONV_C64", 0) ? 1 : 0;
  d.c16_min_rows = L("SS_CONV_C16_MIN_ROWS", d.c16_min_rows); d.c32_min_rows = L("SS_CONV_C32_MIN_ROWS", d.c32_min_rows);
  d.c64_min_rows = L("SS_CONV_C64_MIN_ROWS", d.c64_min_rows);
  d.c64w_on = I("SS_CONV_C64_WINOGRAD", 1); d.c128w_on = I("SS_CONV_C128_WINOGRAD", 1); d.c256w_on = I("SS_CONV_C256_WINOGRAD", 1);
  d.c32w_on = I("SS_CONV_C32_WINOGRAD", 1); d.c64w_min_k = I("SS_CONV_C64_WINOGRAD_MIN_K", 3);
  d.c128w_min_rows = L("SS_CONV_C128_MIN_ROWS", d.c128w_min_rows); d.c256w_min_rows = L("SS_CONV_C256_MIN_ROWS", d.c256w_min_rows);
  if (const int r = I("SS_CONV_C256_ROWS", d.c256w_rows); r == 128 || r == 256) d.c256w_rows = r;
  if (getenv("SS_FFN_WM")) { d.ffn_wm = I("SS_FFN_WM", 3); d.ffn_wm_forced = 1; d.ffn_wm_env = d.ffn_wm; }
  d.ffn_fusion = I("SS_NO_FFN_FUSION", 0) ? 0 : 1; d.ffn_min_rows = I("SS_FFN_MIN_ROWS", d.ffn_min_rows);
  if (getenv("SS_SK_MIN_GFLOP")) d.sk_min_flops = 1e9 * atof(getenv("SS_SK_MIN_GFLOP"));
  d.no_resblock_fusion = I("SS_NO_RESBLOCK_FUSION", 0); d.no_pair_fusion = I("SS_NO_PAIR_FUSION", 0);
  d.rt_off = I("SS_NO_RTLIN", 0) ? 1 : 0; d.rt_min_rows = I("SS_RTLIN_MIN_ROWS", d.rt_min_rows); d.rt_min_units = L("SS_RTLIN_MIN_UNITS", d.rt_min_units);
  d.rt_kb_min_units = L("SS_RTLIN_KB_MIN_UNITS", d.rt_kb_min_units); d.rt_kb_uw = I("SS_RTLIN_KB_UW", d.rt_kb_uw); d.rt_kb_xmap = I("SS_RTLIN_KB_XMAP", d.rt_kb_xmap);
  d.smallm_max_rows = I("SS_SMALLM_MAX_ROWS", d.smallm_max_rows); d.sk_min_units = L("SS_SK_MIN_UNITS", d.sk_min_units);
  d.no_sk2 = I("SS_NO_SK2", 0) ? 1 : 0; d.sk2_min_k64 = I("SS_SK2_MINK64", d.sk2_min_k64); d.sk2_spare_cus = I("SS_SK2_SPARE_CUS", 0);
  d.rt_wg_per_cu = I("SS_RTLIN_WG_PER_CU", 0); d.c32_min_k = I("SS_CONV_C32_MIN_K", d.c32_min_k); d.c16_min_k = I("SS_CONV_C16_MIN_K", d.c16_min_k);
  d.unit_l0_distinct = I("SS_UNIT_L0_DISTINCT", 1) ? 1 : 0; d.fbank_dense = I("SS_FBANK_DENSE", 0) ? 1 : 0;
  return d;
}
Dispatch& process_settings() { static Dispatch d = env_defaults(); return d; }
thread_local const Dispatch* t_disp = nullptr;
thread_local CtxDispatch t_disp_own;
}
void dispatch_edit(const std::function<void(Dispatch&)>& fn) {
  std::lock_guard<std::mutex> lk(g_disp_mu);
  fn(process_settings());
  g_disp_gen.fetch_add(1, std::memory_order_release);
}
void slab_debug(int grid, long long min_rows) {
  const Dispatch dflt = env_defaults();
  dispatch_edit([=](Dispatch& d) {
    d.slab_grid_cap = grid > 0 ? grid : 0;
    const bool set = min_rows >= 0;
    d.c16_min_rows = set ? min_rows : dflt.c16_min_rows; d.c32_min_rows = set ? min_rows : dflt.c32_min_rows;
    d.c64_min_rows = set ? min_rows : dflt.c64_min_rows;
    d.c128w_min_rows = set ? min_rows : dflt.c128w_min_rows; d.c256w_min_rows = set ? min_rows : dflt.c256w_min_rows;
  });
}
int conv_c256w_rows_debug(int rows) {
  if (rows != 0 && rows != 128 && rows != 256) return SS_ERR_ARG;
  const int dflt = env_defaults().c256w_rows;
  dispatch_edit([=](Dispatch& d) { d.c256w_rows = rows ? rows : dflt; });
  return SS_OK;
}
const Dispatch* CtxDispatch::refresh() {
  const unsigned now = g_disp_gen.load(std::memory_order_acquire);
  if (gen != now) {
    std::lock_guard<std::mutex> lk(g_disp_mu);
    d = process_settings();
    gen = g_disp_gen.load(std::memory_order_relaxed);
  }
  return &d;
}
const Dispatch& disp() { return t_disp ? *t_disp : *t_disp_own.refresh(); }
DispatchScope::DispatchScope(const Dispatch* d) : prev(t_disp) { t_disp = d; }
DispatchScope::~DispatchScope() { t_disp = prev; }

void debug_force_tile(int bm, int bn, int ks) {
  dispatch_edit([=](Dispatch& d) { d.force_bm = bm; d.force_bn = bn; d.force_ks = ks; d.sk_groups = (bm == 1 && bn == 8); });
}
bool debug_tile_forced() { return disp().force_bm != 0; }

static thread_local int t_canon = CANON_NONE;
CanonScope::CanonScope(int mode) : prev(t_canon) { t_canon = mode; }
CanonScope::~CanonScope() { t_canon = prev; }
int canon_mode() { return t_canon; }
void canon_debug_set(int mode) { t_canon = mode; }

constexpr size_t SKW_SYNC_BYTES = (16 + 1024) * sizeof(unsigned) + 256;
static std::mutex g_skw_mu;
static std::vector<SkWorkspace*> g_skw_live;
static std::map<std::pair<int, hipStream_t>, SkWorkspace*> g_skw_fallback;
static thread_local SkWorkspace* t_skw = nullptr;

SkWorkspace* sk_workspace_new() {
  SkWorkspace* w = new SkWorkspace();
  std::lock_guard<std::mutex> lk(g_skw_mu);
  g_skw_live.push_back(w);
  return w;
}
void sk_workspace_free(SkWorkspace* w) {
  if (!w) return;
  {
    std::lock_guard<std::mutex> lk(g_skw_mu);
    for (size_t i = 0; i < g_skw_live.size(); ++i)
      if (g_skw_live[i] == w) { g_skw_live.erase(g_skw_live.begin() + i); break; }
  }
  if (w->ws) (void)hipFree(w->ws);
  if (w->sync1) (void)hipFree(w->sync1);
  if (w->sync2) (void)hipFree(w->sync2);
  if (w->sync3) (void)hipFree(w->sync3);
  if (w->dbg) (void)hipFree(w->dbg);
  delete w;
}
SkScope::SkScope(SkWorkspace* w) : prev(t_skw), prev_disp(t_disp) { t_skw = w; t_disp = w ? w->disp.refresh() : nullptr; }
SkScope::~SkScope() { t_skw = prev; t_disp = prev_disp; }

int sk_workspace_acquire(hipStream_t stream, SkWorkspace** out) {
  *out = nullptr;
  int dev = 0;
  SS_HIP_CHECK(hipGetDevice(&dev));
  SkWorkspace* w = t_skw;
  if (!w) {
    std::lock_guard<std::mutex> lk(g_skw_mu);
    SkWorkspace*& slot = g_skw_fallback[std::make_pair(dev, stream)];
    if (!slot) { slot = new SkWorkspace(); g_skw_live.push_back(slot); }
    w = slot;
  }
  if (!w->ws) {
    int cus = 0;
    SS_HIP_CHECK(hipDeviceGetAttribute(&cus, hipDeviceAttributeMultiprocessorCount, dev));
    if (cus <= 0) cus = 256;
    if (cus > 512) cus = 512;
    w->dev = dev; w->cus = cus;
    SS_HIP_CHECK(hipMalloc(&w->ws, (size_t)cus * 256 * 128 * sizeof(float)));
    SS_HIP_CHECK(hipMalloc(&w->sync1, SKW_SYNC_BYTES));
    SS_HIP_CHECK(hipMalloc(&w->sync2, SKW_SYNC_BYTES));
    SS_HIP_CHECK(hipMemsetAsync(w->sync1, 0, SKW_SYNC_BYTES, stream));
    SS_HIP_CHECK(hipMemsetAsync(w->sync2, 0, SKW_SYNC_BYTES, stream));
    SS_HIP_CHECK(hipMalloc(&w->sync3, 4096 * sizeof(unsigned)));
    SS_HIP_CHECK(hipMemsetAsync(w->sync3, 0, 4096 * sizeof(unsigned), stream));
    SS_HIP_CHECK(hipStreamSynchronize(stream));
  } else if (w->dev != dev) {
    return SS_ERR_ARG;
  }
  *out = w;
  return SS_OK;
}

int device_cus(int& cus) {
  static std::mutex mu;
  static int n[128] = {0};
  int dev = 0;
  SS_HIP_CHECK(hipGetDevice(&dev));
  if (dev < 0 || dev >= 128) return SS_ERR_ARG;
  std::lock_guard<std::mutex> lk(mu);
  if (n[dev] == 0) {
    int v = 0;
    SS_HIP_CHECK(hipDeviceGetAttribute(&v, hipDeviceAttributeMultiprocessorCount, dev));
    n[dev] = v > 0 ? v : 256;
  }
  cus = n[dev];
  return SS_OK;
}

int sk_workspace_error_count() {
  std::lock_guard<std::mutex> lk(g_skw_mu);
  int total = 0;
  for (SkWorkspace* w : g_skw_live)
    for (unsigned* sy : {w->sync1, w->sync2}) {
      unsigned v = 0;
      if (sy && hipMemcpy(&v, sy + 8, sizeof(v), hipMemcpyDeviceToHost) == hipSuccess) total += (int)v;
    }
  return total;
}

}
```

### streamspeech_amd/csrc/dispatch.hpp

```cpp
#pragma once
#include <functional>

namespace ss {

struct Dispatch {
  int attn_no_mfma = 0;
  int attn_q16 = 1;
  int attn_split = 0;
  int c16_off = 0, c32_off = 0, c64_off = 0;
  long long c16_min_rows = 131072, c32_min_rows = 65536, c64_min_rows = 32768;
  int c64w_on = 1, c128w_on = 1, c256w_on = 1, c32w_on = 1;
  int c64w_min_k = 3;
  long long c128w_min_rows = 65536, c256w_min_rows = 32768;
  int c256w_rows = 128;
  int c32_min_k = 7, c16_min_k = 11;
  int slab_grid_cap = 0;
  int sk_groups = 0;
  int sk2_spare_cus = 0;
  int ffn_force_g = 0;
  int ffn_wm = 3, ffn_wm_forced = 0;
  int ffn_wm_env = 0;
  int ffn_fusion = 1;
  int ffn_min_rows = 1000;
  int force_bm = 0, force_bn = 0, force_ks = 0;
  double sk_min_flops = 4e9;
  int smallm_max_rows = 192;
  long long sk_min_units = 12 * 512;
  int no_sk2 = 0;
  int sk2_min_k64 = 192;
  int no_resblock_fusion = 0, no_pair_fusion = 0;
  int rt_off = 0, rt_min_rows = 193, rt_force_g = 0;
  long long rt_min_units = 4000;
  int rt_wg_per_cu = 0;
  long long rt_kb_min_units = 256;
  int rt_kb_xmap = 1;
  int rt_kb_uw = 0;
  int rt_kb_order = 1;
  int unit_l0_distinct = 1;
  int fbank_dense = 0;
};

const Dispatch& disp();
void dispatch_edit(const std::function<void(Dispatch&)>& fn);

struct CtxDispatch {
  Dispatch d;
  unsigned gen = 0xffffffffu;
  const Dispatch* refresh();
};
struct DispatchScope {
  explicit DispatchScope(const Dispatch* d);
  ~DispatchScope();
  const Dispatch* prev;
};

}
```

### streamspeech_amd/csrc/gemm.hpp

```cpp
#pragma once
#include "common.hpp"
#include "dispatch.hpp"
#include "prof.hpp"

namespace ss {

struct GemmArgs {
  const float* A = nullptr;
  const float* W = nullptr;
  const float* Wwino = nullptr;
  const void* Wf16 = nullptr;
  const float* bias = nullptr;
  const float* R = nullptr;
  const float* R2 = nullptr;
  float* C = nullptr;
  int lda = 0, ldc = 0, ldr = 0, ldr2 = 0;
  int M = 0, N = 0, Cin = 0;
  int taps = 1, dil = 1, stride = 1, pad = 0;
  int in_len = 0;
  int chunk = 0;
  int m_begin = 0;
  int in_act = ACT_NONE;
  float in_slope = 0.1f;
  int act = ACT_NONE;
  float alpha = 1.0f;
  float div = 0.0f;
  float act_slope = 0.1f;
  float* C2 = nullptr;
  int ldc2 = 0;
  float c2_slope = 0.1f;
  int glu = 0;
  const int* segs = nullptr;
  int nseg = 0;
  int max_seg_out = 0;
  const int* seg_mb = nullptr;
  const float* const* seg_A = nullptr;
  double algo_flops = 0.0;
  double algo_bytes = 0.0;
  const float* ln_g = nullptr;
  const float* ln_b = nullptr;
  float* ln_out = nullptr;
  int same_rows = 0;
  int x3 = 0;
  int canon = 0;
};
constexpr int CANON_NONE = 0, CANON_SEQ = 1, CANON_SMALLM = 2;
constexpr int CANON_KBLOCK = 64;
struct CanonScope {
  explicit CanonScope(int mode);
  ~CanonScope();
  int prev;
};
int canon_mode();
void canon_debug_set(int mode);

struct SkWorkspace {
  int dev = -1, cus = 0;
  float* ws = nullptr;
  unsigned* sync1 = nullptr;
  unsigned* sync2 = nullptr;
  unsigned* sync3 = nullptr;
  unsigned base1[8] = {0, 0, 0, 0, 0, 0, 0, 0}, epoch1 = 0;
  unsigned base2 = 0, epoch2 = 0;
  unsigned long long* dbg = nullptr;
  CtxDispatch disp;
};
SkWorkspace* sk_workspace_new();
void sk_workspace_free(SkWorkspace* w);
struct SkScope {
  explicit SkScope(SkWorkspace* w);
  ~SkScope();
  SkWorkspace* prev;
  const Dispatch* prev_disp;
};
int sk_workspace_acquire(hipStream_t stream, SkWorkspace** out);
int sk_workspace_error_count();

bool conv_sk_eligible(const GemmArgs& a);
int launch_conv_sk(const GemmArgs& a, hipStream_t stream, int g_force = 0);
int conv_sk_error_count();
void conv_sk_set_groups(int on);

bool conv_sk2_eligible(const GemmArgs& a);
int launch_conv_sk2(const GemmArgs& a, hipStream_t stream, int g_force = 0);
int conv_sk2_error_count();

inline bool slab_rows_ok(long long rows) { return rows > 0 && rows < (1ll << 30); }

inline size_t slab_lds_bytes(int slab_rows, int lda, int maxseg) {
  return (size_t)((slab_rows * lda + 3) & ~3) * sizeof(float) + (maxseg + 2) * sizeof(int);
}
inline long long slab_max_blocks(int M, int bm, int nseg) { return (long long)cdiv(M, bm) + (nseg > 0 ? nseg : 1); }
inline int slab_grid(int occ, int cus, int M, int bm, int nseg) {
  const long long g = std::min<long long>((long long)occ * cus, std::max<long long>(1, slab_max_blocks(M, bm, nseg)));
  const int cap = disp().slab_grid_cap;
  return (int)(cap > 0 ? std::min<long long>(g, cap) : g);
}
void slab_debug(int grid, long long min_rows);
bool slab_layout_ok(const GemmArgs& a);
bool slab_conv_ok(const GemmArgs& a, int c);
int device_cus(int& cus);

bool conv_slab_eligible(const GemmArgs& a);
int launch_conv_slab(const GemmArgs& a, hipStream_t stream);

bool conv_pair_eligible(int C, int taps, int dil, int lda, int ldc, int nseg, long long M);
int launch_conv_pair(const float* A, int lda, const float* W1, const float* b1, const float* W2, const float* b2, float* C,
                     int ldc, const float* R2, int ldr2, float div, float* C2, int ldc2, float c2_slope, int Cch, int taps,
                     int dil, int M, int in_len, float slope, const int* segs, int nseg, hipStream_t stream);

bool resblock_fused_eligible(int C, int taps, const int* dil, int ldx, int ldy, int nseg, long long M);
int launch_resblock_fused(const float* X, int ldx, const float* const* W1, const float* const* B1, const float* const* W2,
                          const float* const* B2, const int* dil, float* Y, int ldy, const float* R2, int ldr2, float div, int C,
                          int taps, int M, float slope, const int* segs, int nseg, hipStream_t stream);

bool conv_c64_eligible(const GemmArgs& a);
bool conv_c64_enabled();
int launch_conv_c64(const GemmArgs& a, hipStream_t stream);
bool conv_c64w_eligible(const GemmArgs& a);
int launch_conv_c64w(const GemmArgs& a, hipStream_t stream);
int launch_wino_pack(const float* W, float* WW, int C, int taps, hipStream_t stream);
void conv_c64w_debug(int enable);
bool conv_c64w_enabled();
bool conv_wide_winograd_eligible(const GemmArgs& a, int ch);
int launch_conv_c128w(const GemmArgs& a, hipStream_t stream);
void conv_c128w_debug(int enable);
bool conv_c128w_enabled();
int launch_conv_c256w(const GemmArgs& a, hipStream_t stream);
void conv_c256w_debug(int enable);
int conv_c256w_rows_debug(int rows);
bool conv_c256w_enabled();
bool conv_c32w_eligible(const GemmArgs& a);
int launch_conv_c32w(const GemmArgs& a, hipStream_t stream);
void conv_c32w_debug(int enable);
bool conv_c32w_enabled();
void conv_c64_debug(int enable);

bool conv_c32_eligible(const GemmArgs& a);
bool conv_c32_enabled();
int launch_conv_c32(const GemmArgs& a, hipStream_t stream);
void conv_c32_debug(int enable);

bool conv_c16_eligible(const GemmArgs& a);
bool conv_c16_enabled();
int launch_conv_c16(const GemmArgs& a, hipStream_t stream);
void conv_c16_debug(int enable);

bool conv_f16_eligible(const GemmArgs& a);
bool conv_f16_geometry_ok(int C, int taps, int dil);
int launch_conv_f16(const GemmArgs& a, hipStream_t stream);
size_t f16_pack_halves(int C, int taps);
int launch_f16_pack(const float* W, void* Wf, int C, int taps, hipStream_t stream);

bool rtlin_eligible(const GemmArgs& a);
bool rtlin_shape_ok(const GemmArgs& a);
int launch_rtlin(const GemmArgs& a, hipStream_t stream);
void rtlin_debug(int grid, int enable);
bool rtlin_kb_shape_ok(const GemmArgs& a);
bool rtlin_kb_eligible(const GemmArgs& a);
int launch_rtlin_kb(const GemmArgs& a, hipStream_t stream);
void rtlin_kb_debug(int uw, int order);
void rtlin_kb_last(int out[4]);

bool ffn_fused_eligible(int D, int F, int act, int M, int ldx, int ldy, bool canon = false);
int launch_ffn_fused(const float* X, int ldx, float* Y, int ldy, const float* ln_g, const float* ln_b, const float* W1,
                     const float* b1, const float* W2, const float* b2, float alpha, const float* ln2_g, const float* ln2_b,
                     int M, int D, int F, hipStream_t stream, int canon = 0);
void ffn_fused_debug_grid(int g);
void ffn_fused_debug_rows(int wm);

bool gemv_eligible(const GemmArgs& a);
bool smallm_eligible(const GemmArgs& a);

void debug_force_tile(int bm, int bn, int ks);
bool debug_tile_forced();

int launch_conv_gemm(const GemmArgs& a, hipStream_t stream);

}
```

### streamspeech_amd/csrc/prof.hip

```cpp
#include "gemm.hpp"

#include <atomic>
#include <cstdio>
#include <cstdlib>
#include <cstring>
#include <map>
#include <mutex>
#include <string>
#include <tuple>
#include <utility>
#include <vector>

namespace ss {

static const char* kTileNames[] = {
    "conv_gemm<128,16,16,4,1>", "conv_gemm<128,32,32,4,1>", "conv_gemm<128,32,16,4,1>", "conv_gemm<16,128,32,1,4>",
    "conv_gemm<16,128,16,1,4>", "conv_gemm<128,128,16,2,2>", "conv_gemm<128,64,32,2,2>", "conv_gemm<64,64,32,2,2>",
    "conv_gemm<64,64,16,2,2>", "conv_gemm<32,64,32,2,2>", "conv_gemm<32,64,16,2,2>", "conv_gemm<32,32,32,2,2>",
    "smallm_gemm<4,1>", "smallm_gemm<2,2>", "smallm_gemm<1,4>", "conv_sk<128,BN,32>",
    "conv_slab<32>", "conv_slab<16>", "conv_sk2<256,128,32>", "conv_sk2_bf16x3<256,128,32>",
    "resblock_fused<32>", "resblock_fused<16>", "ffn_fused<256,2048>", "rt_linear<48,256>", "conv_c64<256,64>", "conv_c32<256,32>", "conv_c16<256,16>", "conv_c64w<256,64>", "conv_c128w<256,128>", "conv_c32w<256,32>", "conv_c256w<256,128>", "rt_linear_kb<48,256>",
    "conv_f16<64>", "conv_f16<128>", "conv_f16<256>"};
static_assert(sizeof(kTileNames) / sizeof(kTileNames[0]) == kNumTileCfg, "one name per ProfCls, in enum order");
static std::atomic<int> g_prof_mask{0};
static std::atomic<int> g_prof_mask_hi{0};
static std::vector<ProfRec> g_prof_recs;
static std::vector<std::pair<hipEvent_t, hipEvent_t>> g_prof_pool;
static std::mutex g_prof_mu;

void prof_enable(int cls_mask) { g_prof_mask.store(cls_mask, std::memory_order_relaxed); }
void prof_enable_hi(int cls_mask) { g_prof_mask_hi.store(cls_mask, std::memory_order_relaxed); }
const char* prof_cfg_name(int cls) { return (cls >= 0 && cls < kNumTileCfg) ? kTileNames[cls] : "?"; }
void prof_reset() {
  for (auto& r : g_prof_recs) g_prof_pool.push_back({r.e0, r.e1});
  g_prof_recs.clear();
}
int prof_read_issued(int cls, double* issued) {
  double v = 0;
  for (auto& r : g_prof_recs) if (r.cls == cls) v += r.issued;
  if (issued) *issued = v;
  return SS_OK;
}
int prof_read(int cls, double* ms_total, double* flops_total, long long* launches, double* bytes_total) {
  double ms = 0, fl = 0, by = 0; long long n = 0;
  for (auto& r : g_prof_recs) {
    if (r.cls != cls) continue;
    if (hipEventSynchronize(r.e1) != hipSuccess) return SS_ERR_HIP;
    float t = 0.f;
    if (hipEventElapsedTime(&t, r.e0, r.e1) != hipSuccess) return SS_ERR_HIP;
    ms += t; fl += r.flops; by += r.bytes; ++n;
  }
  if (ms_total) *ms_total = ms;
  if (flops_total) *flops_total = fl;
  if (launches) *launches = n;
  if (bytes_total) *bytes_total = by;
  return SS_OK;
}

struct ProfTotals { std::atomic<unsigned long long> flops{0}, bytes{0}, launches{0}; };
static ProfTotals g_prof_totals[kNumTileCfg];
static std::mutex g_tot_mu;
struct ShapeTot { long launches = 0; double rows = 0, flops = 0, bytes = 0; };
using ShapeKey = std::tuple<int, int, int, int, int>;
static std::map<ShapeKey, ShapeTot>* g_shapes = nullptr;
static std::string shape_table() {
  std::string out = "class N taps Cin operands launches mean_rows gflop_per_launch mbyte_per_launch\n";
  if (!g_shapes) return out;
  char line[256];
  for (auto& kv : *g_shapes) {
    const ShapeTot& z = kv.second;
    snprintf(line, sizeof line, "%d %d %d %d %d %ld %.0f %.3f %.2f\n", std::get<0>(kv.first), std::get<1>(kv.first), std::get<2>(kv.first),
             std::get<3>(kv.first), std::get<4>(kv.first), z.launches, z.rows / z.launches, z.flops / z.launches * 1e-9, z.bytes / z.launches * 1e-6);
    out += line;
  }
  return out;
}
static void shape_log_dump() {
  const char* path = getenv("SS_SHAPE_LOG");
  FILE* f = path ? fopen(path, "w") : nullptr;
  if (!f) return;
  std::lock_guard<std::mutex> lk(g_tot_mu);
  fputs(shape_table().c_str(), f);
  fclose(f);
}
static std::atomic<int> g_shape_log{getenv("SS_SHAPE_LOG") != nullptr ? 1 : 0};
void prof_shape_log(int on) {
  std::lock_guard<std::mutex> lk(g_tot_mu);
  if (on && g_shapes && !getenv("SS_SHAPE_LOG")) g_shapes->clear();
  g_shape_log.store(on ? 1 : 0, std::memory_order_relaxed);
}
int prof_shape_dump(char* buf, int cap) {
  std::lock_guard<std::mutex> lk(g_tot_mu);
  const std::string t = shape_table();
  if (buf && cap > 0) { const int n = (int)std::min<size_t>(t.size(), (size_t)cap - 1); memcpy(buf, t.data(), n); buf[n] = 0; }
  return (int)t.size() + 1;
}
int prof_totals(int cls, double* flops, double* bytes, long long* launches) {
  if (cls < 0 || cls >= kNumTileCfg) return SS_ERR_ARG;
  if (flops) *flops = (double)g_prof_totals[cls].flops.load(std::memory_order_relaxed);
  if (bytes) *bytes = (double)g_prof_totals[cls].bytes.load(std::memory_order_relaxed);
  if (launches) *launches = (long long)g_prof_totals[cls].launches.load(std::memory_order_relaxed);
  return SS_OK;
}
static void algo_work(const GemmArgs& a, double& flops, double& bytes) {
  flops = a.algo_flops > 0 ? a.algo_flops : 2.0 * (double)a.M * a.N * a.taps * a.Cin;
  const double ncols = a.glu ? a.N / 2 : a.N;
  bytes = 4.0 * ((double)a.N * a.taps * a.Cin + (a.bias ? a.N : 0) + (double)a.in_len * a.Cin +
                 (double)a.M * ncols * (1 + (a.R ? 1 : 0) + (a.R2 ? 1 : 0)));
  if (a.algo_bytes > 0) bytes = a.algo_bytes;
}

static bool prof_cls_winograd(ProfCls cls) { return cls >= PROF_CONV_C64W && cls <= PROF_CONV_C256W; }

int prof_begin(const GemmArgs& a, hipStream_t stream, ProfCls cls, ProfRec& rec, bool& prof) {
  {
    double fl, by;
    algo_work(a, fl, by);
    g_prof_totals[cls].flops.fetch_add((unsigned long long)(fl + 0.5), std::memory_order_relaxed);
    g_prof_totals[cls].bytes.fetch_add((unsigned long long)(by + 0.5), std::memory_order_relaxed);
    g_prof_totals[cls].launches.fetch_add(1ull, std::memory_order_relaxed);
    if (g_shape_log.load(std::memory_order_relaxed)) {
      std::lock_guard<std::mutex> lk(g_tot_mu);
      if (!g_shapes) { g_shapes = new std::map<ShapeKey, ShapeTot>(); if (getenv("SS_SHAPE_LOG")) atexit(shape_log_dump); }
      const int ops = (a.R ? 1 : 0) | (a.R2 ? 2 : 0) | (a.C2 ? 4 : 0) | (a.in_act != ACT_NONE ? 8 : 0) | (a.act != ACT_NONE ? 16 : 0) | (a.glu ? 32 : 0) | (a.nseg > 0 ? 64 : 0);
      ShapeTot& z = (*g_shapes)[ShapeKey(cls, a.N, a.taps, a.Cin, ops)];
      z.launches += 1; z.rows += a.M; z.flops += fl; z.bytes += by;
    }
  }
  prof = cls < 32 ? ((unsigned)g_prof_mask.load(std::memory_order_relaxed) >> cls) & 1u
                  : ((unsigned)g_prof_mask_hi.load(std::memory_order_relaxed) >> (cls - 32)) & 1u;
  if (!prof) return SS_OK;
  std::lock_guard<std::mutex> lk(g_prof_mu);
  if (!g_prof_pool.empty()) { rec.e0 = g_prof_pool.back().first; rec.e1 = g_prof_pool.back().second; g_prof_pool.pop_back(); }
  else { SS_HIP_CHECK(hipEventCreate(&rec.e0)); SS_HIP_CHECK(hipEventCreate(&rec.e1)); }
  rec.cls = cls;
  algo_work(a, rec.flops, rec.bytes);
  rec.issued = (prof_cls_winograd(cls) && a.taps >= 3) ? rec.flops * (4.0 * (a.taps / 3) + (a.taps % 3 ? a.taps % 3 + 1 : 0)) / (2.0 * a.taps) : rec.flops;
  SS_HIP_CHECK(hipEventRecord(rec.e0, stream));
  return SS_OK;
}
int prof_end(hipStream_t stream, ProfRec& rec, bool prof) {
  if (prof) {
    std::lock_guard<std::mutex> lk(g_prof_mu);
    SS_HIP_CHECK(hipEventRecord(rec.e1, stream));
    g_prof_recs.push_back(rec);
  }
  return SS_OK;
}

}
```

### streamspeech_amd/csrc/prof.hpp

```cpp
#pragma once
#include "common.hpp"

namespace ss {

struct GemmArgs;

enum ProfCls : int {
  PROF_GEMM_128x16x16 = 0, PROF_GEMM_128x32x32 = 1, PROF_GEMM_128x32x16 = 2, PROF_GEMM_16x128x32 = 3, PROF_GEMM_16x128x16 = 4,
  PROF_GEMM_128x128x16 = 5, PROF_GEMM_128x64x32 = 6, PROF_GEMM_64x64x32 = 7, PROF_GEMM_64x64x16 = 8, PROF_GEMM_32x64x32 = 9,
  PROF_GEMM_32x64x16 = 10, PROF_GEMM_32x32x32 = 11,
  PROF_SMALLM_4x1 = 12, PROF_SMALLM_2x2 = 13, PROF_SMALLM_1x4 = 14,
  PROF_CONV_SK = 15, PROF_CONV_SLAB32 = 16, PROF_CONV_SLAB16 = 17, PROF_CONV_SK2 = 18, PROF_CONV_SK2_BF16X3 = 19,
  PROF_RESBLOCK32 = 20, PROF_RESBLOCK16 = 21, PROF_FFN = 22, PROF_RTLIN = 23,
  PROF_CONV_C64 = 24, PROF_CONV_C32 = 25, PROF_CONV_C16 = 26,
  PROF_CONV_C64W = 27, PROF_CONV_C128W = 28, PROF_CONV_C32W = 29, PROF_CONV_C256W = 30,
  PROF_RTLIN_KB = 31,
  PROF_CONV_F16_64 = 32, PROF_CONV_F16_128 = 33, PROF_CONV_F16_256 = 34,
};
constexpr int kNumTileCfg = PROF_CONV_F16_256 + 1;
void prof_enable(int cls_mask);
void prof_enable_hi(int cls_mask);
void prof_reset();
int prof_read(int cls, double* ms_total, double* flops_total, long long* launches, double* bytes_total = nullptr);
const char* prof_cfg_name(int cls);
int prof_totals(int cls, double* flops, double* bytes, long long* launches);
int prof_read_issued(int cls, double* issued_flops_total);
void prof_shape_log(int on);
int prof_shape_dump(char* buf, int cap);

struct ProfRec { hipEvent_t e0, e1; double flops, bytes, issued; int cls; };
int prof_begin(const GemmArgs& a, hipStream_t stream, ProfCls cls, ProfRec& rec, bool& prof);
int prof_end(hipStream_t stream, ProfRec& rec, bool prof);

}
```

### streamspeech_amd/csrc/vocoder.hip

```cpp
#include "model_internal.hpp"

#include <cstdint>
#include <tuple>


namespace {
struct WinoShared { DevBuf buf; size_t floats = 0; int refs = 0; };
struct WinoKey {
  int dev; const float* blob; uint64_t sig;
  bool operator<(const WinoKey& o) const { return std::tie(dev, blob, sig) < std::tie(o.dev, o.blob, o.sig); }
};
std::mutex g_wino_mu;
std::map<WinoKey, WinoShared> g_wino;
inline uint64_t fnv(uint64_t h, uint64_t v) { for (int i = 0; i < 8; ++i) { h ^= (v >> (8 * i)) & 0xff; h *= 1099511628211ull; } return h; }
uint64_t blob_sig(const ss_vocoder* v, const float* d_blob) {
  const ss_vocoder_config* cfg = &v->cfg;
  uint64_t sig = fnv(fnv(fnv(14695981039346656037ull, (uint64_t)cfg->upsample_initial_channel), (uint64_t)cfg->n_up), (uint64_t)cfg->n_res);
  for (int j = 0; j < cfg->n_res; ++j) sig = fnv(sig, (uint64_t)cfg->resblock_kernel_sizes[j]);
  for (size_t i = 0; i < v->rb_c1.size(); ++i) sig = fnv(fnv(sig, (uint64_t)(v->rb_c1[i].w - d_blob)), (uint64_t)(v->rb_c2[i].w - d_blob));
  return sig;
}
std::mutex g_f16_mu;
std::map<WinoKey, WinoShared> g_f16;
bool f16_stage(int ch) { return ch == 64 || ch == 128 || ch == 256; }
// ... 15 lines not shown
  v->dur_c1 = {w.get("voc.dur.conv1.w", (int64_t)Hd * kd * E), w.get("voc.dur.conv1.b", Hd)};
  v->dur_ln1 = {w.get("voc.dur.ln1.g", Hd), w.get("voc.dur.ln1.b", Hd)};
  v->dur_c2 = {w.get("voc.dur.conv2.w", (int64_t)Hd * kd * Hd), w.get("voc.dur.conv2.b", Hd)};
  v->dur_ln2 = {w.get("voc.dur.ln2.g", Hd), w.get("voc.dur.ln2.b", Hd)};
  v->dur_proj = {w.get("voc.dur.proj.w", Hd), w.get("voc.dur.proj.b", 1)};
  const int C0 = cfg->upsample_initial_channel;
  v->pre = {w.get("voc.pre.w", (int64_t)C0 * 7 * cfg->model_in_dim), w.get("voc.pre.b", C0)};
  int C = C0;
  for (int i = 0; i < cfg->n_up; ++i) {
    const int Co = C / 2, st = cfg->upsample_rates[i];
    v->ups.push_back({w.get("voc.up" + std::to_string(i) + ".w", (int64_t)st * Co * 3 * C),
                      w.get("voc.up" + std::to_string(i) + ".b", (int64_t)st * Co)});
    for (int j = 0; j < cfg->n_res; ++j) {
      const int kr = cfg->resblock_kernel_sizes[j];
      for (int dd = 0; dd < 3; ++dd) {
        const std::string p = "voc.rb" + std::to_string(i * cfg->n_res + j);
        v->rb_c1.push_back({w.get(p + ".c1." + std::to_string(dd) + ".w", (int64_t)Co * kr * Co),
                            w.get(p + ".c1." + std::to_string(dd) + ".b", Co)});
        v->rb_c2.push_back({w.get(p + ".c2." + std::to_string(dd) + ".w", (int64_t)Co * kr * Co),
                            w.get(p + ".c2." + std::to_string(dd) + ".b", Co)});
      }
    }
    C = Co;
  }
  v->post = {w.get("voc.post.w", (int64_t)7 * C), w.get("voc.post.b", 1)};
  {
    auto it = w.map.find("voc.spkr.table");
    if (it != w.map.end()) {
      const int64_t per = (int64_t)16 * C0;
      if (it->second.n <= 0 || it->second.n % per || it->second.n / per > INT32_MAX || (C0 & 3)) { scratch_unref(v->sc); delete v; return SS_ERR_ARG; }
      v->spk_table = it->second.p;
      v->n_spk = (int)(it->second.n / per);
    }
  }
  if (!w.missing.empty()) { scratch_unref(v->sc); delete v; return SS_ERR_MISSING_WEIGHT; }
  {
    auto wino_stage = [](int ch) { return ch == 32 || ch == 64 || ch == 128 || ch == 256; };
    size_t need = 0;
    int Cs = C0;
    for (int i = 0; i < cfg->n_up; ++i) {
      Cs /= 2;
      if (wino_stage(Cs)) for (int j = 0; j < cfg->n_res; ++j) need += 6 * (size_t)Cs * ((cfg->resblock_kernel_sizes[j] + 2) / 3) * 4 * Cs;
    }
    if (need) {
      int dev = 0;
      if (hipGetDevice(&dev) != hipSuccess) { scratch_unref(v->sc); delete v; return SS_ERR_HIP; }
      std::lock_guard<std::mutex> lk(g_wino_mu);
      const WinoKey key{dev, d_blob, blob_sig(v, d_blob)};
      WinoShared& sh = g_wino[key];
      const bool fresh = sh.refs == 0;
      if (!fresh && sh.floats != need) { scratch_unref(v->sc); delete v; return SS_ERR_ARG; }
      if (fresh) {
        rc = sh.buf.ensure(need * sizeof(float));
        if (rc != SS_OK) { g_wino.erase(key); scratch_unref(v->sc); delete v; return rc; }
        sh.floats = need;
      }
      float* dst = sh.buf.f();
      Cs = C0;
      for (int i = 0; i < cfg->n_up && rc == SS_OK; ++i) {
        Cs /= 2;
        if (!wino_stage(Cs)) continue;
        for (int j = 0; j < cfg->n_res && rc == SS_OK; ++j) {
          const int kr = cfg->resblock_kernel_sizes[j];
          const size_t n = (size_t)Cs * ((kr + 2) / 3) * 4 * Cs;
          for (int dd = 0; dd < 3 && rc == SS_OK; ++dd) {
            const int idx = (i * cfg->n_res + j) * 3 + dd;
            if (fresh) rc = launch_wino_pack(v->rb_c1[idx].w, dst, Cs, kr, nullptr);
            v->rb_c1[idx].ww = dst; dst += n;
            if (fresh && rc == SS_OK) rc = launch_wino_pack(v->rb_c2[idx].w, dst, Cs, kr, nullptr);
            v->rb_c2[idx].ww = dst; dst += n;
          }
        }
      }
      if (fresh && rc == SS_OK && hipDeviceSynchronize() != hipSuccess) rc = SS_ERR_HIP;
      if (rc != SS_OK) {
        if (fresh) { sh.buf.release(); g_wino.erase(key); }
        scratch_unref(v->sc); delete v; return rc;
      }
      ++sh.refs;
      v->wino = sh.buf.f(); v->wino_key = d_blob;
    }
  }
  *out = v;
  return SS_OK;
}

extern "C" int ss_vocoder_num_speakers(const ss_vocoder* v) { return v ? v->n_spk : 0; }

extern "C" int ss_vocoder_set_bf16x3(ss_vocoder* v, int on) {
  if (!v) return SS_ERR_ARG;
  v->x3 = on ? 1 : 0;
  return SS_OK;
}

static int f16_take(ss_vocoder* v) {
  const ss_vocoder_config& c = v->cfg;
  size_t need = 0;
  for (int i = 0, Cs = c.upsample_initial_channel; i < c.n_up; ++i) {
    Cs /= 2;
    if (f16_stage(Cs)) for (int j = 0; j < c.n_res; ++j) need += 6 * f16_pack_halves(Cs, c.resblock_kernel_sizes[j]);
  }
  if (!need) return SS_OK;
  for (int i = 0, Cs = c.upsample_initial_channel; i < c.n_up; ++i) {
    Cs /= 2;
    if (!f16_stage(Cs)) continue;
    for (int j = 0; j < c.n_res; ++j)
      for (int dd = 0; dd < 3; ++dd)
        if (!conv_f16_geometry_ok(Cs, c.resblock_kernel_sizes[j], c.resblock_dilations[j][dd]) ||
            !conv_f16_geometry_ok(Cs, c.resblock_kernel_sizes[j], 1))
          return SS_ERR_ARG;
  }
  int dev = 0;
  if (hipGetDevice(&dev) != hipSuccess) return SS_ERR_HIP;
  std::lock_guard<std::mutex> lk(g_f16_mu);
  const WinoKey key{dev, v->blob, blob_sig(v, v->blob)};
  WinoShared& sh = g_f16[key];
  const bool fresh = sh.refs == 0;
  if (!fresh && sh.floats != need) return SS_ERR_ARG;
  int rc = SS_OK;
  if (fresh) {
    rc = sh.buf.ensure(need * sizeof(uint16_t));
    if (rc != SS_OK) { g_f16.erase(key); return rc; }
    sh.floats = need;
  }
  char* dst = static_cast<char*>(sh.buf.p);
  std::vector<ConvW> rb1 = v->rb_c1, rb2 = v->rb_c2;
  for (int i = 0, Cs = c.upsample_initial_channel; i < c.n_up && rc == SS_OK; ++i) {
    Cs /= 2;
    if (!f16_stage(Cs)) continue;
    for (int j = 0; j < c.n_res && rc == SS_OK; ++j) {
      const int kr = c.resblock_kernel_sizes[j];
      const size_t n = f16_pack_halves(Cs, kr) * sizeof(uint16_t);
      for (int dd = 0; dd < 3 && rc == SS_OK; ++dd) {
        const int idx = (i * c.n_res + j) * 3 + dd;
        if (fresh) rc = launch_f16_pack(rb1[idx].w, dst, Cs, kr, nullptr);
        rb1[idx].wh = dst; dst += n;
        if (fresh && rc == SS_OK) rc = launch_f16_pack(rb2[idx].w, dst, Cs, kr, nullptr);
        rb2[idx].wh = dst; dst += n;
      }
    }
  }
  if (fresh && rc == SS_OK && hipDeviceSynchronize() != hipSuccess) rc = SS_ERR_HIP;
  if (rc != SS_OK) {
    if (fresh) { sh.buf.release(); g_f16.erase(key); }
    return rc;
  }
  ++sh.refs;
  v->rb_c1.swap(rb1); v->rb_c2.swap(rb2);
  v->f16w = sh.buf.p;
  return SS_OK;
}

extern "C" int ss_vocoder_set_f16(ss_vocoder* v, int on) {
  if (!v) return SS_ERR_ARG;
  if (on && !v->f16w) RET(f16_take(v));
  v->f16 = on ? 1 : 0;
  return SS_OK;
}

extern "C" void ss_vocoder_destroy(ss_vocoder* v) {
  if (!v) return;
  if (v->f16w) {
    std::lock_guard<std::mutex> lk(g_f16_mu);
    for (auto it = g_f16.begin(); it != g_f16.end(); ++it)
      if (it->first.blob == v->blob && it->second.buf.p == v->f16w) {
        if (--it->second.refs == 0) { it->second.buf.release(); g_f16.erase(it); }
        break;
      }
  }
  if (v->wino_key) {
    std::lock_guard<std::mutex> lk(g_wino_mu);
    for (auto it = g_wino.begin(); it != g_wino.end(); ++it)
      if (it->first.blob == v->wino_key && it->second.buf.f() == v->wino) {
        if (--it->second.refs == 0) { it->second.buf.release(); g_wino.erase(it); }
        break;
      }
  }
  scratch_unref(v->sc);
  delete v;
}

extern "C" int ss_vocoder_bind_scratch(ss_vocoder* v, ss_scratch* sc) {
  if (!v || !sc) return SS_ERR_ARG;
  if (sc != v->sc) {
    sc->refs.fetch_add(1);
    scratch_unref(v->sc);
    v->sc = sc;
  }
  return SS_OK;
}

struct GenBufs { float *bx, *bt, *br, *bs, *bxa, *bra, *bsa, *br2; };
struct SpkSel { const int* seg = nullptr; int one = 0; int max_frames = 0; };

template <class ConvFn, class StageFn, class GeomFn>
static int hifigan_stack(const ss_vocoder* v, hipStream_t s, ConvFn&& conv, StageFn&& on_stage, GeomFn&& geom,
                         const float* frames, int Ft, const GenBufs& b, int* out_scale, int* out_C, const SpkSel* spk = nullptr) {
  const ss_vocoder_config& c = v->cfg;
  const bool f16 = v->f16 && v->f16w;
  const bool x3 = v->x3 && !f16;
  auto slab_stage = [&](int channels) {
    if (x3 || !(channels == 64 ? conv_c64_enabled() : channels == 32 ? conv_c32_enabled() : channels == 16 ? conv_c16_enabled() : false)) return false;
    long long rows = Ft; int ch = c.upsample_initial_channel; bool found = false;
    for (int i = 0; i < c.n_up && !found; ++i) { rows *= c.upsample_rates[i]; ch /= 2; found = ch == channels; }
    if (!found || rows >= (1ll << 30)) return false;
    GemmArgs probe;
    probe.same_rows = 1; probe.Cin = probe.N = probe.lda = probe.ldc = channels; probe.taps = 3; probe.dil = 1; probe.pad = 1;
    probe.M = probe.in_len = (int)rows; probe.in_act = ACT_LRELU;
    return channels == 64 ? conv_c64_eligible(probe) : channels == 32 ? conv_c32_eligible(probe) : conv_c16_eligible(probe);
  };
  const bool c64 = slab_stage(64), c32 = slab_stage(32), c16 = slab_stage(16);
  auto wino_slab_stage = [&](int channels) {
    if (f16 || x3 || !(channels == 128 ? conv_c128w_enabled() : conv_c256w_enabled())) return false;
    long long rows = Ft; int ch = c.upsample_initial_channel, stage = -1;
    for (int i = 0; i < c.n_up && stage < 0; ++i) { rows *= c.upsample_rates[i]; ch /= 2; if (ch == channels) stage = i; }
    if (stage < 0 || rows >= (1ll << 30)) return false;
    int sc = 1, gM = 0, gnseg = 0; const int* gsegs = nullptr;
    for (int i = 0; i <= stage; ++i) sc *= c.upsample_rates[i];
    geom(sc, gM, gsegs, gnseg);
    for (int j = 0; j < c.n_res; ++j)
      for (int dd = 0; dd < 3; ++dd)
        for (int which = 0; which < 2; ++which) {
          const int idx = (stage * c.n_res + j) * 3 + dd;
          GemmArgs probe;
          probe.same_rows = 1; probe.Cin = probe.N = probe.lda = probe.ldc = probe.ldr = probe.ldr2 = probe.ldc2 = channels;
          probe.taps = c.resblock_kernel_sizes[j]; probe.dil = which ? 1 : c.resblock_dilations[j][dd];
          probe.pad = probe.dil * (probe.taps - 1) / 2; probe.M = probe.in_len = gM; probe.nseg = gnseg; probe.in_act = ACT_LRELU;
          probe.Wwino = which ? v->rb_c2[idx].ww : v->rb_c1[idx].ww;
          if (!conv_wide_winograd_eligible(probe, channels)) return false;
        }
    return true;
  };
  const bool c128 = wino_slab_stage(128), c256 = wino_slab_stage(256);
  auto preact = [c64, c128, c256, f16](int channels) {
    return channels >= 64 && !(c64 && channels == 64) && !(c128 && channels == 128) && !(c256 && channels == 256) && !(f16 && f16_stage(channels));
  };
  auto up_preact = [c64](int channels) { return channels >= 64 && !(c64 && channels == 64); };
  auto mk = [x3, f16](const float* A, int Cin, const ConvW& cw, int Cout, int k, int dil, float* Cc, int ldc) {
    GemmArgs a;
    a.A = A; a.lda = Cin; a.W = cw.w; a.Wwino = cw.ww; a.bias = cw.b; a.C = Cc; a.ldc = ldc; a.ldr = ldc; a.ldr2 = ldc; a.ldc2 = ldc;
    a.N = Cout; a.Cin = Cin; a.taps = k; a.dil = dil; a.stride = 1; a.pad = dil * (k - 1) / 2; a.same_rows = 1;
    a.x3 = x3;
    if (f16) a.Wf16 = cw.wh;
    return a;
  };
  int scale = 1, C = c.upsample_initial_channel;
  RET(on_stage(scale));
  {
    GemmArgs a = mk(frames, c.model_in_dim, v->pre, C, 7, 1, b.bx, C);
    if (up_preact(C) && !spk) a.C2 = b.bxa;
    if (f16) a.canon = CANON_SEQ;
    RET(conv(a, scale));
    if (spk) {
      int gM = 0, gnseg = 0; const int* gsegs = nullptr;
      geom(scale, gM, gsegs, gnseg);
      const bool pa0 = up_preact(C);
      RET(launch_spkr_pre_add(b.bx, pa0 ? b.bxa : b.bx, C, C, v->spk_table, spk->seg, spk->one, gsegs, gnseg, spk->max_frames, gM, pa0 ? 1 : 0,
                              0.1f, s));
    }
  }
  for (int i = 0; i < c.n_up; ++i) {
    const int st = c.upsample_rates[i], Co = C / 2;
    const bool pa_in = up_preact(C), pa = preact(Co);
    {
      GemmArgs a = mk(pa_in ? b.bxa : b.bx, C, v->ups[i], st * Co, 3, 1, b.bs, st * Co);
      if (!pa_in) { a.in_act = ACT_LRELU; a.in_slope = 0.1f; }
      if (pa) a.C2 = b.bsa;
      a.algo_flops = 2.0 * Ft * scale * C * Co * c.upsample_kernel_sizes[i];
      if (f16 && Co >= 64) a.canon = CANON_SEQ;
      RET(conv(a, scale));
    }
    scale *= st; C = Co;
    RET(on_stage(scale));
    const bool pa_next = (i + 1 < c.n_up) && up_preact(C);
    for (int j = 0; j < c.n_res; ++j) {
      const int kr = c.resblock_kernel_sizes[j];
      int gM = 0, gnseg = 0; const int* gsegs = nullptr;
      geom(scale, gM, gsegs, gnseg);
      const bool per_conv = (c32 && C == 32 && kr >= disp().c32_min_k) || (c16 && C == 16 && kr >= disp().c16_min_k);
      if (!pa && !per_conv && !disp().no_resblock_fusion && resblock_fused_eligible(C, kr, c.resblock_dilations[j], C, C, gnseg, gM)) {
        const float *W1[3], *B1[3], *W2[3], *B2[3];
        for (int dd = 0; dd < 3; ++dd) {
          const int idx = (i * c.n_res + j) * 3 + dd;
          W1[dd] = v->rb_c1[idx].w; B1[dd] = v->rb_c1[idx].b; W2[dd] = v->rb_c2[idx].w; B2[dd] = v->rb_c2[idx].b;
        }
        RET(launch_resblock_fused(b.bs, C, W1, B1, W2, B2, c.resblock_dilations[j], b.bx, C, j > 0 ? b.bx : nullptr, C,
                                  j == c.n_res - 1 ? (float)c.n_res : 0.f, C, kr, gM, 0.1f, gsegs, gnseg, s));
        continue;
      }
      const bool fuse = !pa && !per_conv && !disp().no_pair_fusion && kr == 3 &&
                        conv_pair_eligible(C, kr, c.resblock_dilations[j][2], C, C, gnseg, gM);
      const float* cur = b.bs;
      for (int dd = 0; dd < 3; ++dd) {
        const int idx = (i * c.n_res + j) * 3 + dd;
        if (fuse) {
          float* out = dd == 0 ? b.br : dd == 1 ? b.br2 : b.bx;
          const float* R2 = (dd == 2 && j > 0) ? b.bx : nullptr;
          const float div = (dd == 2 && j == c.n_res - 1) ? (float)c.n_res : 0.f;
          RET(launch_conv_pair(cur, C, v->rb_c1[idx].w, v->rb_c1[idx].b, v->rb_c2[idx].w, v->rb_c2[idx].b, out, C, R2, C, div,
                               nullptr, C, 0.1f, C, kr, c.resblock_dilations[j][dd], gM, gM, 0.1f, gsegs, gnseg, s));
          cur = out;
          continue;
        }
        const float* rin = dd == 0 ? b.bs : b.br;
        const float* rin_act = dd == 0 ? b.bsa : b.bra;
        GemmArgs a1 = mk(pa ? rin_act : rin, C, v->rb_c1[idx], C, kr, c.resblock_dilations[j][dd], b.bt, C);
        if (pa) { a1.act = ACT_LRELU; a1.act_slope = 0.1f; }
        else { a1.in_act = ACT_LRELU; a1.in_slope = 0.1f; }
        RET(conv(a1, scale));
        GemmArgs a2 = mk(b.bt, C, v->rb_c2[idx], C, kr, 1, dd < 2 ? b.br : b.bx, C);
        if (!pa) { a2.in_act = ACT_LRELU; a2.in_slope = 0.1f; }
        a2.R = rin;
        if (dd < 2) {
          if (pa) a2.C2 = b.bra;
        } else {
          a2.R2 = j == 0 ? nullptr : b.bx;
          a2.div = (j == c.n_res - 1) ? (float)c.n_res : 0.f;
          if (pa_next && j == c.n_res - 1) a2.C2 = b.bxa;
        }
        RET(conv(a2, scale));
      }
    }
  }
  *out_scale = scale; *out_C = C;
  return SS_OK;
}

static int conv1d(hipStream_t s, const float* A, int T, int Cin, const ConvW& cw, int Cout, int k, int dil,
                  float* C, int in_act, float slope, int act, const float* R, const float* R2, float div) {
  GemmArgs a;
  a.A = A; a.lda = Cin; a.W = cw.w; a.bias = cw.b; a.C = C; a.ldc = Cout; a.R = R; a.ldr = Cout; a.R2 = R2; a.ldr2 = Cout;
  a.M = T; a.N = Cout; a.Cin = Cin; a.taps = k; a.dil = dil; a.stride = 1; a.pad = dil * (k - 1) / 2; a.in_len = T;
  a.in_act = in_act; a.in_slope = slope; a.act = act; a.div = div; a.same_rows = 1;
  return launch_conv_gemm(a, s);
}

static bool spkr_args_ok(const ss_vocoder* v, bool have, const int32_t* h_spkr, int B) {
  if (!have) return v->n_spk == 0;
  if (v->n_spk == 0 || !h_spkr) return false;
  for (int b = 0; b < B; ++b)
    if (h_spkr[b] < 0 || h_spkr[b] >= v->n_spk) return false;
  return true;
}

static int vocoder_forward(ss_vocoder* v, void* stream, const int32_t* d_codes, int K, int dur_prediction,
                           const int32_t* d_forced_dur, float* d_wav, int64_t wav_capacity,
                           int32_t* d_dur, int64_t* h_n_samples, const int32_t* h_spkr) {
  if (!v || K <= 0 || !d_codes || !d_wav || !d_dur) return SS_ERR_ARG;
  if (!spkr_args_ok(v, h_spkr != nullptr, h_spkr, 1)) return SS_ERR_ARG;
  SkScope sk_scope(v->sc->skws);
  hipStream_t s = (hipStream_t)stream;
  const ss_vocoder_config& c = v->cfg;
  const int E = c.embedding_dim, Hd = c.dur_hidden;
  RET(v->sc->v_small.ensure(((size_t)K * (E + 2 * Hd + 1) + 2 * (K + 2)) * sizeof(float)));
  float* emb = v->sc->v_small.f();
  float* t1 = emb + (size_t)K * E;
  float* t2 = t1 + (size_t)K * Hd;
  float* logdur = t2 + (size_t)K * Hd;
  int* cum = reinterpret_cast<int*>(logdur + K);
  int* ones = cum + K + 1;
  RET(launch_gather_rows(d_codes, v->dict, E, emb, K, s, v->cfg.num_embeddings));
  const int* forced = d_forced_dur;
  if (!forced && dur_prediction) {
    RET(conv1d(s, emb, K, E, v->dur_c1, Hd, c.dur_kernel, 1, t1, ACT_NONE, 0.f, ACT_RELU, nullptr, nullptr, 0.f));
    RET(launch_layernorm(t1, Hd, t1, Hd, v->dur_ln1.g, v->dur_ln1.b, K, Hd, 1e-5f, s));
    RET(conv1d(s, t1, K, Hd, v->dur_c2, Hd, c.dur_kernel, 1, t2, ACT_NONE, 0.f, ACT_RELU, nullptr, nullptr, 0.f));
    RET(launch_layernorm(t2, Hd, t2, Hd, v->dur_ln2.g, v->dur_ln2.b, K, Hd, 1e-5f, s));
    RET(conv1d(s, t2, K, Hd, v->dur_proj, 1, 1, 1, logdur, ACT_NONE, 0.f, ACT_NONE, nullptr, nullptr, 0.f));
  } else if (!forced) {
    SS_HIP_CHECK(hipMemsetD32Async(reinterpret_cast<hipDeviceptr_t>(ones), 1, K, s));
    forced = ones;
  }
  RET(launch_dur_predict(logdur, forced, K, d_dur, cum, s));
  int total = 0;
  SS_HIP_CHECK(hipMemcpyAsync(&total, cum + K, sizeof(int), hipMemcpyDeviceToHost, s));
  SS_HIP_CHECK(hipStreamSynchronize(s));
  const int Fr = total;
  int hop = 1;
  for (int i = 0; i < c.n_up; ++i) hop *= c.upsample_rates[i];
  const int64_t S = (int64_t)Fr * hop;
  if (h_n_samples) *h_n_samples = S;
  if (S > wav_capacity) return SS_ERR_CAPACITY;
  if (Fr <= 0) return SS_OK;

  size_t stage_max = (size_t)Fr * c.upsample_initial_channel;
  {
    int T = Fr, C = c.upsample_initial_channel;
    for (int i = 0; i < c.n_up; ++i) { T *= c.upsample_rates[i]; C /= 2; stage_max = std::max(stage_max, (size_t)T * C); }
  }
  RET(v->sc->v_ws.ensure((8 * stage_max + (size_t)Fr * E) * sizeof(float)));
  float* frames = v->sc->v_ws.f();
  GenBufs gb;
  gb.bx = frames + (size_t)Fr * E;
  gb.bt = gb.bx + stage_max;
  gb.br = gb.bt + stage_max;
  gb.bs = gb.br + stage_max;
  gb.bxa = gb.bs + stage_max;
  gb.bra = gb.bxa + stage_max;
  gb.bsa = gb.bra + stage_max;
  gb.br2 = gb.bsa + stage_max;
  RET(launch_repeat_rows(emb, cum, K, E, frames, Fr, s));
  int T = 1, C = 0;
  SpkSel sel;
  if (h_spkr) { sel.one = h_spkr[0]; sel.max_frames = Fr; }
  RET(hifigan_stack(v, s, [&](GemmArgs& a, int scale) { a.M = Fr * scale; a.in_len = Fr * scale; return launch_conv_gemm(a, s); },
                    [](int) { return SS_OK; },
                    [&](int scale, int& M, const int*& segs, int& nseg) { M = Fr * scale; segs = nullptr; nseg = 0; },
                    frames, Fr, gb, &T, &C, h_spkr ? &sel : nullptr));
  T *= Fr;
  float* bx = gb.bx;
  return launch_conv_post_tanh(bx, T, C, v->post.w, v->post.b, 0.01f, d_wav, s);
}

extern "C" int ss_vocoder_forward(ss_vocoder* v, void* stream, const int32_t* d_codes, int K, int dur_prediction,
                                  const int32_t* d_forced_dur, float* d_wav, int64_t wav_capacity,
                                  int32_t* d_dur, int64_t* h_n_samples) {
  return vocoder_forward(v, stream, d_codes, K, dur_prediction, d_forced_dur, d_wav, wav_capacity, d_dur, h_n_samples, nullptr);
}

extern "C" int ss_vocoder_forward_spkr(ss_vocoder* v, void* stream, const int32_t* d_codes, int K, int dur_prediction,
                                       const int32_t* d_forced_dur, float* d_wav, int64_t wav_capacity,
                                       int32_t* d_dur, int64_t* h_n_samples, int32_t spkr) {
  return vocoder_forward(v, stream, d_codes, K, dur_prediction, d_forced_dur, d_wav, wav_capacity, d_dur, h_n_samples, &spkr);
}


static int batch_vocoder_forward(ss_vocoder* v, void* stream, int B, const int32_t* d_codes, const int32_t* h_K,
                                 int dur_prediction, const int32_t* d_forced_dur, float* d_wav,
                                 int64_t wav_capacity, int32_t* d_dur, int64_t* h_wav_start,
                                 int64_t* h_n_samples, bool with_spkr, const int32_t* h_spkr) {
  if (!v || B <= 0 || !d_codes || !d_wav || !d_dur) return SS_ERR_ARG;
  if (!spkr_args_ok(v, with_spkr, h_spkr, B)) return SS_ERR_ARG;
  SkScope sk_scope(v->sc->skws);
  hipStream_t s = (hipStream_t)stream;
  const ss_vocoder_config& c = v->cfg;
  const int E = c.embedding_dim, Hd = c.dur_hidden;
  for (int b = 0; b < B; ++b)
    if (h_K[b] <= 0) return SS_ERR_ARG;
  const Offsets ok = prefix(h_K, B);
  const int Kt = ok.total;
  RET(v->sc->v_small.ensure(((size_t)Kt * (E + 2 * Hd + 1) + 2 * (Kt + B + 2)) * sizeof(float)));
  float* emb = v->sc->v_small.f();
  float* t1 = emb + (size_t)Kt * E;
  float* t2 = t1 + (size_t)Kt * Hd;
  float* logdur = t2 + (size_t)Kt * Hd;
  int* cum = reinterpret_cast<int*>(logdur + Kt);
  int* ones = cum + Kt + B + 1;
  std::vector<int> tk(6 * B);
  for (int b = 0; b < B; ++b) {
    int* a = &tk[4 * b]; a[0] = ok.off[b]; a[1] = h_K[b]; a[2] = ok.off[b]; a[3] = h_K[b];
    tk[4 * B + 2 * b] = ok.off[b]; tk[4 * B + 2 * b + 1] = h_K[b];
  }
  RET(v->sc->v_segs.ensure((6 * B + 16 * B + (with_spkr ? B : 0)) * sizeof(int)));
  int* dk = (int*)v->sc->v_segs.p;
  RET(upload(s, dk, tk));
  RET(launch_gather_rows(d_codes, v->dict, E, emb, Kt, s, v->cfg.num_embeddings));
  const int* forced = d_forced_dur;
  auto sconv = [&](const float* A, int Cin, const ConvW& cw, int Cout, int k, float* Cc, int act) {
    GemmArgs a;
    a.A = A; a.lda = Cin; a.W = cw.w; a.bias = cw.b; a.C = Cc; a.ldc = Cout; a.N = Cout; a.Cin = Cin; a.taps = k;
    a.pad = (k - 1) / 2; a.act = act; a.segs = dk; a.nseg = B; a.max_seg_out = ok.mx; a.M = Kt; a.in_len = Kt;
    a.canon = CANON_SEQ;
    return launch_conv_gemm(a, s);
  };
  if (!forced && dur_prediction) {
    RET(sconv(emb, E, v->dur_c1, Hd, c.dur_kernel, t1, ACT_RELU));
    RET(launch_layernorm(t1, Hd, t1, Hd, v->dur_ln1.g, v->dur_ln1.b, Kt, Hd, 1e-5f, s));
    RET(sconv(t1, Hd, v->dur_c2, Hd, c.dur_kernel, t2, ACT_RELU));
    RET(launch_layernorm(t2, Hd, t2, Hd, v->dur_ln2.g, v->dur_ln2.b, Kt, Hd, 1e-5f, s));
    RET(sconv(t2, Hd, v->dur_proj, 1, 1, logdur, ACT_NONE));
  } else if (!forced) {
    std::vector<int> one(Kt, 1);
    RET(upload(s, ones, one));
    forced = ones;
  }
  RET(launch_dur_predict(logdur, forced, 0, d_dur, cum, s, dk + 4 * B, B));
  std::vector<int> hcum(Kt + B);
  SS_HIP_CHECK(hipMemcpyAsync(hcum.data(), cum, (size_t)(Kt + B) * sizeof(int), hipMemcpyDeviceToHost, s));
  SS_HIP_CHECK(hipStreamSynchronize(s));
  int hop = 1;
  for (int i = 0; i < c.n_up; ++i) hop *= c.upsample_rates[i];
  std::vector<int> Fr(B);
  for (int b = 0; b < B; ++b) Fr[b] = hcum[ok.off[b] + b + h_K[b]];
  const Offsets of = prefix(Fr.data(), B);
  for (int b = 0; b < B; ++b) { h_wav_start[b] = (int64_t)of.off[b] * hop; h_n_samples[b] = (int64_t)Fr[b] * hop; }
  if ((int64_t)of.total * hop > wav_capacity) return SS_ERR_CAPACITY;
  if (of.total <= 0) return SS_OK;
  const int Ft = of.total;

  size_t stage_max = (size_t)Ft * c.upsample_initial_channel;
  {
    int T = Ft, C = c.upsample_initial_channel;
    for (int i = 0; i < c.n_up; ++i) { T *= c.upsample_rates[i]; C /= 2; stage_max = std::max(stage_max, (size_t)T * C); }
  }
  RET(v->sc->v_ws.ensure((8 * stage_max + (size_t)Ft * E) * sizeof(float)));
  float* frames = v->sc->v_ws.f();
  GenBufs gb;
  gb.bx = frames + (size_t)Ft * E;
  gb.bt = gb.bx + stage_max;
  gb.br = gb.bt + stage_max;
  gb.bs = gb.br + stage_max;
  gb.bxa = gb.bs + stage_max;
  gb.bra = gb.bxa + stage_max;
  gb.bsa = gb.bra + stage_max;
  gb.br2 = gb.bsa + stage_max;
  int* dseg = dk + 6 * B;
  int* drep = dseg + 4 * B;
  int* dwav = drep + 4 * B;
  auto stage_segs = [&](int scale) {
    std::vector<int> t(4 * B);
    for (int b = 0; b < B; ++b) { t[4 * b] = of.off[b] * scale; t[4 * b + 1] = Fr[b] * scale; t[4 * b + 2] = t[4 * b]; t[4 * b + 3] = t[4 * b + 1]; }
    return upload(s, dseg, t);
  };
  {
    std::vector<int> t(4 * B);
    for (int b = 0; b < B; ++b) { t[4 * b] = ok.off[b]; t[4 * b + 1] = h_K[b]; t[4 * b + 2] = of.off[b]; t[4 * b + 3] = Fr[b]; }
    RET(upload(s, drep, t));
  }
  RET(launch_repeat_rows(emb, cum, 0, E, frames, of.mx, s, drep, B));
  SpkSel sel;
  if (with_spkr) {
    int* dspk = dk + 6 * B + 16 * B;
    RET(upload(s, dspk, std::vector<int>(h_spkr, h_spkr + B)));
    sel.seg = dspk; sel.max_frames = of.mx;
  }
  int scale = 1, C = 0;
  RET(hifigan_stack(v, s,
                    [&](GemmArgs& a, int sc) {
                      a.segs = dseg; a.nseg = B; a.max_seg_out = of.mx * sc; a.M = Ft * sc; a.in_len = Ft * sc;
                      return launch_conv_gemm(a, s);
                    },
                    stage_segs,
                    [&](int sc, int& M, const int*& segs, int& nseg) { M = Ft * sc; segs = dseg; nseg = B; },
                    frames, Ft, gb, &scale, &C, with_spkr ? &sel : nullptr));
  float* bx = gb.bx;
  {
    std::vector<int> t(2 * B);
    for (int b = 0; b < B; ++b) { t[2 * b] = of.off[b] * scale; t[2 * b + 1] = Fr[b] * scale; }
    RET(upload(s, dwav, t));
  }
  return launch_conv_post_tanh(bx, of.mx * scale, C, v->post.w, v->post.b, 0.01f, d_wav, s, dwav, B);
}

extern "C" int ss_batch_vocoder_forward(ss_vocoder* v, void* stream, int B, const int32_t* d_codes, const int32_t* h_K,
                                        int dur_prediction, const int32_t* d_forced_dur, float* d_wav,
                                        int64_t wav_capacity, int32_t* d_dur, int64_t* h_wav_start,
                                        int64_t* h_n_samples) {
  return batch_vocoder_forward(v, stream, B, d_codes, h_K, dur_prediction, d_forced_dur, d_wav, wav_capacity, d_dur, h_wav_start,
                               h_n_samples, false, nullptr);
}

extern "C" int ss_batch_vocoder_forward_spkr(ss_vocoder* v, void* stream, int B, const int32_t* d_codes, const int32_t* h_K,
                                             int dur_prediction, const int32_t* d_forced_dur, float* d_wav,
                                             int64_t wav_capacity, int32_t* d_dur, int64_t* h_wav_start,
                                             int64_t* h_n_samples, const int32_t* h_spkr) {
  return batch_vocoder_forward(v, stream, B, d_codes, h_K, dur_prediction, d_forced_dur, d_wav, wav_capacity, d_dur, h_wav_start,
                               h_n_samples, true, h_spkr);
}


static int batch_vocoder_tail(ss_vocoder* v, void* stream, int B, const int32_t* d_codes, const int32_t* h_K,
                              const int32_t* h_n_new, const int32_t* h_ctx, const int32_t* h_rf, int dur_prediction,
                              float* d_out, int64_t out_capacity, int32_t* h_win_first, int32_t* h_dur, int64_t* h_out_start,
                              int64_t* h_n_out, bool with_spkr, const int32_t* h_spkr) {
  if (!v || B <= 0 || B > 32768 || !d_codes || !h_K || !h_n_new || !h_ctx || !h_rf || !d_out || !h_win_first || !h_dur ||
      !h_out_start || !h_n_out)
    return SS_ERR_ARG;
  if (!spkr_args_ok(v, with_spkr, h_spkr, B)) return SS_ERR_ARG;
  const ss_vocoder_config& c = v->cfg;
  const int E = c.embedding_dim, Hd = c.dur_hidden;
  for (int b = 0; b < B; ++b)
    if (h_K[b] <= 0 || h_n_new[b] <= 0 || h_n_new[b] > h_K[b] || h_ctx[b] < 0 || (h_ctx[b] > 0 && h_rf[b] < 0)) return SS_ERR_ARG;
  const Offsets ok = prefix(h_K, B);
  std::vector<int> cu, cl, csrc, fall(B, -1);
  for (int b = 0; b < B; ++b) {
    const bool win = h_ctx[b] > 0 && h_K[b] > h_n_new[b] + h_ctx[b];
    const int first = win ? h_K[b] - (h_n_new[b] + h_ctx[b]) : 0;
    csrc.push_back(ok.off[b] + first); cl.push_back(h_K[b] - first);
  }
  for (int b = 0; b < B; ++b)
    if (cl[b] < h_K[b]) { fall[b] = (int)cl.size(); csrc.push_back(ok.off[b]); cl.push_back(h_K[b]); }
  const int S = (int)cl.size();
  const Offsets oc = prefix(cl.data(), S);
  const int Kc = oc.total;
  cu.assign(oc.off.begin(), oc.off.end() - 1);
  const size_t n_small = (size_t)ok.total * E + (size_t)Kc * (E + 2 * Hd + 1) + 3 * ((size_t)Kc + S + 2);
  RET(v->sc->v_small.ensure(n_small * sizeof(float)));
  RET(v->sc->v_segs.ensure(((size_t)Kc + 6 * S + 12 * B + (with_spkr ? B : 0)) * sizeof(int)));
  SkScope sk_scope(v->sc->skws);
  hipStream_t s = (hipStream_t)stream;
  float* emb_all = v->sc->v_small.f();
  float* emb = emb_all + (size_t)ok.total * E;
  float* t1 = emb + (size_t)Kc * E;
  float* t2 = t1 + (size_t)Kc * Hd;
  float* logdur = t2 + (size_t)Kc * Hd;
  int* dur = reinterpret_cast<int*>(logdur + Kc);
  int* cum = dur + Kc;
  int* aux = cum + Kc + S + 2;
  int* dk = (int*)v->sc->v_segs.p;
  {
    std::vector<int> tk((size_t)Kc + 6 * S);
    for (int z = 0; z < S; ++z) {
      for (int i = 0; i < cl[z]; ++i) tk[cu[z] + i] = csrc[z] + i;
      int* a = &tk[Kc + 4 * z]; a[0] = cu[z]; a[1] = cl[z]; a[2] = cu[z]; a[3] = cl[z];
      tk[Kc + 4 * S + 2 * z] = cu[z]; tk[Kc + 4 * S + 2 * z + 1] = cl[z];
    }
    RET(upload(s, dk, tk));
  }
  const int* dmap = dk;
  const int* dconv = dk + Kc;
  const int* ddur = dconv + 4 * S;
  RET(launch_gather_rows(d_codes, v->dict, E, emb_all, ok.total, s, v->cfg.num_embeddings));
  RET(launch_gather_rows(dmap, emb_all, E, emb, Kc, s, ok.total));
  const int* forced = nullptr;
  if (dur_prediction) {
    int mx = 0;
    for (int z = 0; z < S; ++z) mx = std::max(mx, cl[z]);
    auto sconv = [&](const float* A, int Cin, const ConvW& cw, int Cout, int k, float* Cc, int act) {
      GemmArgs a;
      a.A = A; a.lda = Cin; a.W = cw.w; a.bias = cw.b; a.C = Cc; a.ldc = Cout; a.N = Cout; a.Cin = Cin; a.taps = k;
      a.pad = (k - 1) / 2; a.act = act; a.segs = dconv; a.nseg = S; a.max_seg_out = mx; a.M = Kc; a.in_len = Kc;
      a.canon = CANON_SEQ;
      return launch_conv_gemm(a, s);
// ... 130 lines not shown
```

### streamspeech_amd/lib.py

```python
import ctypes as C
import os

_HERE = os.path.dirname(os.path.abspath(__file__))
LIB_PATH = os.environ.get("SS_HIP_LIB") or os.path.join(_HERE, "libstreamspeech_hip.so")


class SSConfig(C.Structure):
    _fields_ = [(n, C.c_int32) for n in (
        "input_feat", "conv_channels", "conv_kernel", "enc_dim", "enc_ffn", "enc_heads", "enc_layers",
        "dw_kernel", "src_vocab", "tgt_vocab", "mt_layers", "dec_dim", "dec_ffn", "dec_heads",
        "t2u_layers", "unit_layers", "unit_vocab", "ctc_upsample", "pad", "eos", "unk",
        "max_rel_pos", "max_tgt_pos")]


class SSVocoderConfig(C.Structure):
    _fields_ = [
        ("num_embeddings", C.c_int32), ("embedding_dim", C.c_int32), ("model_in_dim", C.c_int32),
        ("upsample_initial_channel", C.c_int32),
        ("n_up", C.c_int32), ("upsample_rates", C.c_int32 * 8), ("upsample_kernel_sizes", C.c_int32 * 8),
        ("n_res", C.c_int32), ("resblock_kernel_sizes", C.c_int32 * 4), ("resblock_dilations", (C.c_int32 * 3) * 4),
        ("dur_hidden", C.c_int32), ("dur_kernel", C.c_int32)]


_vp, _i, _f, _i64 = C.c_void_p, C.c_int, C.c_float, C.c_int64


class SSPcmSeg(C.Structure):
    _fields_ = [("src_offset", C.c_int64), ("dst_offset", C.c_int64), ("frames", C.c_int32), ("fmt", C.c_int32),
                ("channels", C.c_int32), ("dst", C.c_int32)]


class SSPcmEmitSeg(C.Structure):
    _fields_ = [("carry", _vp), ("tail", _vp), ("taps", _vp), ("n_before", C.c_int64), ("k0", C.c_int64), ("k1", C.c_int64),
                ("out_offset", C.c_int64), ("carry_len", C.c_int32), ("n_new", C.c_int32), ("up", C.c_int32), ("down", C.c_int32),
                ("half", C.c_int32), ("fmt", C.c_int32), ("finished", C.c_int32), ("reserved", C.c_int32)]


class SSVadState(C.Structure):
    _fields_ = [("onset", C.c_int64), ("last_speech", C.c_int64), ("utt_first_frame", C.c_int64), ("floor", C.c_float),
                ("mode", C.c_int32), ("run", C.c_int32), ("reserved", C.c_int32)]


class SSVadSeg(C.Structure):
    _fields_ = [("hist", _vp), ("state", _vp), ("powers", _vp), ("hist_first", C.c_int64), ("n_hist", C.c_int64),
                ("first_frame", C.c_int64), ("n_frames", C.c_int32), ("H", C.c_int32), ("W", C.c_int32),
                ("p_abs", C.c_float), ("p_min", C.c_float), ("snr", C.c_float), ("rise", C.c_float),
                ("min_speech", C.c_int32), ("end_silence", C.c_int32), ("post_roll", C.c_int32), ("max_frames", C.c_int32),
                ("reserved", C.c_int32)]


class SSVadResult(C.Structure):
    _fields_ = [("consumed", C.c_int64), ("start_frame", C.c_int64), ("cut_sample", C.c_int64), ("last_speech", C.c_int64),
                ("events", C.c_int32), ("mode", C.c_int32)]


class SSCtcAlignResult(C.Structure):
    _fields_ = [("score", C.c_double), ("viterbi", C.c_double), ("status", C.c_int32), ("n_tokens", C.c_int32)]


CTC_ALIGN_MAX_FRAMES = 1500
CTC_ALIGN_MAX_LABELS = 1500


class SSOpAttnArgs(C.Structure):
    _fields_ = [
        ("Q", _vp), ("K", _vp), ("V", _vp), ("O", _vp),
        ("ldq", C.c_int32), ("ldk", C.c_int32), ("ldv", C.c_int32), ("ldo", C.c_int32),
        ("Tq", C.c_int32), ("Tk", C.c_int32), ("H", C.c_int32),
        ("scale", _f),
        ("causal", C.c_int32), ("chunk", C.c_int32), ("q0", C.c_int32), ("k_mask_tail", C.c_int32),
        ("P", _vp), ("ldp", C.c_int32),
        ("bias_u", _vp), ("bias_v", _vp),
        ("segs", _vp), ("nseg", C.c_int32), ("max_q", C.c_int32), ("p_tmax", C.c_int32),
        ("seg_tail", _vp),
        ("no_decode_kernel", C.c_int32),
        ("anc", _vp), ("anc_ld", C.c_int32), ("anc_slots", C.c_int32),
        ("use_split", C.c_int32)]


class SSOpConvArgs(C.Structure):
    _fields_ = [
        ("A", _vp), ("W", _vp), ("bias", _vp), ("R", _vp), ("R2", _vp), ("C", _vp), ("C2", _vp),
        ("lda", C.c_int32), ("ldc", C.c_int32), ("ldr", C.c_int32), ("ldr2", C.c_int32), ("ldc2", C.c_int32),
        ("M", C.c_int32), ("N", C.c_int32), ("Cin", C.c_int32), ("taps", C.c_int32), ("dil", C.c_int32), ("stride", C.c_int32),
        ("pad", C.c_int32), ("in_len", C.c_int32), ("chunk", C.c_int32),
        ("in_act", C.c_int32), ("in_slope", _f),
        ("act", C.c_int32), ("act_slope", _f), ("alpha", _f), ("div", _f), ("c2_slope", _f),
        ("glu", C.c_int32),
        ("segs", _vp), ("nseg", C.c_int32), ("max_seg_out", C.c_int32),
        ("same_rows", C.c_int32)]


class SSOpPoolAttnArgs(C.Structure):
    _fields_ = [
        ("Qs", _vp), ("cache", _vp), ("O", _vp),
        ("ld", C.c_int32), ("ldo", C.c_int32), ("slot_rows", C.c_int32),
        ("P", _vp), ("ldp", C.c_int32), ("p_tmax", C.c_int32),
        ("bias_u", _vp), ("bias_v", _vp),
        ("sess", _vp), ("qt_pre", _vp),
        ("nsess", C.c_int32), ("qtiles", C.c_int32), ("H", C.c_int32),
        ("scale", _f)]

class SSOpAttnProbsArgs(C.Structure):
    _fields_ = [
        ("Q", _vp), ("K", _vp),
        ("ldq", C.c_int32), ("ldk", C.c_int32), ("H", C.c_int32),
        ("scale", _f),
        ("segs", _vp), ("nseg", C.c_int32),
        ("q_first", _vp), ("row_off", _vp), ("p_off", _vp),
        ("P", _vp), ("peak", _vp), ("stat", _vp),
        ("max_rows", C.c_int32)]


class SSOpBeamState(C.Structure):
    _fields_ = [(n, _vp) for n in (
        "tok", "cum", "anc", "cand_s", "cand_t", "ignore", "done", "max_len", "npre",
        "fin_cnt", "fin_score", "fin_len", "fin_tok", "fin_pos", "fin_anc")]


class SSMtSearchOpts(C.Structure):
    _fields_ = [("size", C.c_int32), ("no_repeat_ngram", C.c_int32), ("len_penalty", _f), ("temperature", _f)]


def search_opts(len_penalty: float = 1.0, temperature: float = 1.0, no_repeat_ngram_size: int = 0):
    if float(len_penalty) == 1.0 and float(temperature) == 1.0 and int(no_repeat_ngram_size) == 0:
        return None
    return SSMtSearchOpts(C.sizeof(SSMtSearchOpts), int(no_repeat_ngram_size), float(len_penalty), float(temperature))


class SSMtSampleOpts(C.Structure):
    _fields_ = [("size", C.c_int32), ("topk", C.c_int32), ("topp", _f), ("reserved", C.c_int32), ("seed", C.c_uint64)]


def sample_opts(topk: int = 0, topp: float = 0.0, seed: int = 1):
    return SSMtSampleOpts(C.sizeof(SSMtSampleOpts), int(topk), float(topp), 0, int(seed) & 0xFFFFFFFFFFFFFFFF)


SS_OP_BEAM_CAND = 64

SIGNATURES = {
    "ss_abi_version": (_i, []),
    "ss_error_string": (C.c_char_p, [_i]),
    "ss_model_create": (_i, [C.POINTER(SSConfig), _vp, C.c_size_t, C.POINTER(C.c_char_p), C.POINTER(_i64),
                             C.POINTER(_i64), _i, C.POINTER(_vp)]),
    "ss_model_destroy": (None, [_vp]),
    "ss_scratch_create": (_i, [C.POINTER(_vp)]),
    "ss_scratch_destroy": (None, [_vp]),
    "ss_scratch_set_cap": (_i, [_vp, C.c_size_t]),
    "ss_scratch_trim": (_i, [_vp, C.c_size_t]),
    "ss_scratch_bytes": (C.c_size_t, [_vp]),
    "ss_model_bind_scratch": (_i, [_vp, _vp]),
    "ss_vocoder_bind_scratch": (_i, [_vp, _vp]),
    "ss_fbank_num_frames": (_i, [_i]),
    "ss_fbank_cmvn": (_i, [_vp, _vp, _vp, _i, _f, _vp, C.POINTER(_i)]),
    "ss_encoder_out_len": (_i, [_i]),
    "ss_resample": (_i, [_vp, _vp, _i64, _i, _i, _vp, _i, _vp, _i64]),
    "ss_mp3_probe": (_i, [_vp, C.c_size_t, _vp]),
    "ss_mp3_unpack": (_i, [_vp, C.c_size_t, _i64, _vp, _vp, _vp]),
    "ss_mp3_synthesize": (_i, [_vp, _vp, _vp, _i64, _vp, _i, _i, _vp, _i64, _vp, C.POINTER(C.c_size_t)]),
    "ss_mp3_stream_create": (_i, [_i, C.POINTER(_vp)]),
    "ss_mp3_stream_destroy": (None, [_vp]),
    "ss_mp3_stream_reset": (_i, [_vp]),
    "ss_mp3_stream_bound": (_i64, [_vp, C.c_size_t]),
    "ss_mp3_stream_push": (_i, [_vp, _vp, C.c_size_t, _i, _i64, _vp, _vp, _vp, C.POINTER(_i64), _vp]),
    "ss_mp3_stream_query": (_i, [_vp, _vp]),
    "ss_mp3_stream_copy": (_i, [_vp, _vp]),
    "ss_mp3_stream_synthesize": (_i, [_vp, _vp, _vp, _i64, _vp, _i, C.POINTER(_vp), C.POINTER(_vp), C.POINTER(_i64), _i, _i, _vp,
                                      C.POINTER(C.c_size_t)]),
    "ss_flac_streaminfo": (_i, [_vp, C.c_size_t, _vp]),
    "ss_flac_probe": (_i, [_vp, C.c_size_t, _vp]),
    "ss_flac_unpack": (_i, [_vp, C.c_size_t, _i64, _vp, _vp, _i64, _vp]),
    "ss_flac_restore_host": (_i, [_vp, _vp, _i64, _vp, _i, _i, _vp, _vp]),
    "ss_flac_restore": (_i, [_vp, _vp, _vp, _i64, _i64, _vp, _i, _i, _vp, _i64, _vp, C.POINTER(C.c_size_t)]),
    "ss_pcm_scatter": (_i, [_vp, _vp, _i64, _vp, _i, C.POINTER(_vp), C.POINTER(_i64), _i]),
    "ss_pcm_pack_s16": (_i, [_vp, _vp, _i64, _vp]),
    "ss_pcm_decode_host": (_i, [_vp, _i, _i, _i64, _vp]),
    "ss_pcm_pack_s16_host": (_i, [_vp, _i64, _vp]),
    "ss_pcm_emit_count": (_i64, [_i64, _i, _i, _i, _i]),
    "ss_pcm_emit": (_i, [_vp, _vp, _i, _vp, _i64]),
    "ss_pcm_emit_host": (_i, [_vp, _i, _vp, _i64]),
    "ss_pcm_encode_host": (_i, [_vp, _i64, _i, _vp]),
    "ss_vad_scan": (_i, [_vp, _vp, _i, _vp]),
    "ss_vad_scan_host": (_i, [_vp, _i, _vp]),
    "ss_row_max_logprob": (_i, [_vp, _vp, _i, _i, _i, _i, _i, _vp]),
    "ss_log_softmax": (_i, [_vp, _vp, _i, _i, _i, _i, _i, _vp]),
    "ss_encoder_forward": (_i, [_vp, _vp, _vp, _i, _i, _i, _vp]),
    "ss_encoder_stream_reset": (_i, [_vp]),
    "ss_encoder_stream_set_tail": (_i, [_vp, _i]),
    "ss_encoder_stream_set_deferred": (_i, [_vp, _i]),
    "ss_encoder_stream_status": (_i, [_vp, _vp, _vp]),
    "ss_debug_enc_step_inject_timeout": (_i, [_vp]),
    "ss_encoder_stream_forward": (_i, [_vp, _vp, _vp, _i, _i, _i, _vp, C.POINTER(C.c_int32), C.POINTER(C.c_int32)]),
    "ss_ctc_greedy_scored": (_i, [_vp, _vp, _i, _vp, _i, _vp, _vp, _vp, _vp, _vp, _vp, _vp, _vp]),
    "ss_ctc_greedy": (_i, [_vp, _vp, _i, _vp, _i, _vp, _vp, _vp, _vp, _vp]),
    "ss_stream_pool_create": (_i, [_vp, _i, _i, C.POINTER(_vp)]),
    "ss_stream_pool_destroy": (None, [_vp]),
    "ss_stream_pool_reset": (_i, [_vp, _i]),
    "ss_stream_pool_set_tail": (_i, [_vp, _i, _i]),
    "ss_encoder_stream_forward_batch": (_i, [_vp, _vp, _vp, _i, C.POINTER(C.c_int32), C.POINTER(_vp), C.POINTER(C.c_int32),
                                             C.POINTER(C.c_int32), C.POINTER(C.c_int32), _vp, C.POINTER(C.c_int32),
                                             C.POINTER(C.c_int32)]),
    "ss_stream_pool_set_scores": (_i, [_vp, _i]),
    "ss_stream_pool_ctc_scored": (_i, [_vp, _vp, _vp, _i, _i, C.POINTER(C.c_int32), _vp, _vp, _vp, _vp, _vp, _vp, _vp, _vp]),
    "ss_stream_pool_ctc": (_i, [_vp, _vp, _vp, _i, _i, C.POINTER(C.c_int32), _vp, _vp, _vp, _vp, _vp]),
    "ss_stream_pool_stats": (_i, [_vp, C.POINTER(_i64), C.POINTER(_i64)]),
    "ss_mt_begin": (_i, [_vp, _vp, _vp, _i]),
    "ss_mt_set_persistent": (_i, [_vp, _i]),
    "ss_model_set_pack_invariant": (_i, [_vp, _i]),
    "ss_model_get_pack_invariant": (_i, [_vp]),
    "ss_debug_canon": (_i, [_i]),
    "ss_mt_get_persistent": (_i, [_vp]),
    "ss_debug_mt_inject_timeout": (_i, [_vp]),
    "ss_mt_append": (_i, [_vp, _vp, _vp, _i, _i, _i, _i, _vp, _vp, _i]),
    "ss_mt_truncate": (_i, [_vp, _i]),
    "ss_mt_greedy": (_i, [_vp, _vp, _vp, _i, C.POINTER(C.c_int32), _i, _i, _i, C.POINTER(C.c_int32), C.POINTER(_i),
                          _vp, C.POINTER(_i)]),
    "ss_t2u_units": (_i, [_vp, _vp, _vp, _i, _i, _i, _vp, _vp, _vp, _vp, _i]),
    "ss_vocoder_create": (_i, [C.POINTER(SSVocoderConfig), _vp, C.c_size_t, C.POINTER(C.c_char_p),
                               C.POINTER(_i64), C.POINTER(_i64), _i, C.POINTER(_vp)]),
    "ss_vocoder_destroy": (None, [_vp]),
    "ss_vocoder_set_bf16x3": (_i, [_vp, _i]),
    "ss_vocoder_set_f16": (_i, [_vp, _i]),
    "ss_vocoder_forward": (_i, [_vp, _vp, _vp, _i, _i, _vp, _vp, _i64, _vp, C.POINTER(_i64)]),
    "ss_vocoder_num_speakers": (_i, [_vp]),
    "ss_vocoder_forward_spkr": (_i, [_vp, _vp, _vp, _i, _i, _vp, _vp, _i64, _vp, C.POINTER(_i64), C.c_int32]),
    "ss_batch_vocoder_forward_spkr": (_i, [_vp, _vp, _i, _vp, C.POINTER(C.c_int32), _i, _vp, _vp, _i64, _vp,
                                           C.POINTER(_i64), C.POINTER(_i64), C.POINTER(C.c_int32)]),
    "ss_batch_vocoder_tail_spkr": (_i, [_vp, _vp, _i, _vp, C.POINTER(C.c_int32), C.POINTER(C.c_int32), C.POINTER(C.c_int32),
                                        C.POINTER(C.c_int32), _i, _vp, _i64, C.POINTER(C.c_int32), C.POINTER(C.c_int32),
                                        C.POINTER(_i64), C.POINTER(_i64), C.POINTER(C.c_int32)]),
    "ss_batch_fbank_cmvn": (_i, [_vp, _vp, _i, _vp, C.POINTER(_i64), C.POINTER(C.c_int32), _f, _vp, C.POINTER(C.c_int32)]),
    "ss_batch_cmvn": (_i, [_vp, _vp, _vp, _i64, _vp]),
    "ss_batch_encoder_forward": (_i, [_vp, _vp, _i, _vp, C.POINTER(C.c_int32), _i, _i, _vp, C.POINTER(C.c_int32)]),
    "ss_batch_ctc_greedy_scored": (_i, [_vp, _vp, _i, _i, _vp, C.POINTER(C.c_int32), _vp, _vp, _vp, _vp, _vp, _vp, _vp]),
    "ss_batch_ctc_greedy": (_i, [_vp, _vp, _i, _i, _vp, C.POINTER(C.c_int32), _vp, _vp, _vp, _vp]),
    "ss_batch_ctc_align": (_i, [_vp, _vp, _i, _i, _vp, C.POINTER(C.c_int32), C.POINTER(C.c_int32), C.POINTER(C.c_int32), _vp, _vp, _vp,
                                _vp, _vp]),
    "ss_ctc_align_host": (_i, [_vp, _i, _i, _i, _i, C.POINTER(C.c_int32), C.POINTER(C.c_int32), C.POINTER(C.c_int32), _vp, _vp, _vp,
                               _vp, _vp, _vp]),
    "ss_batch_mt_greedy": (_i, [_vp, _vp, _i, _vp, C.POINTER(C.c_int32), C.POINTER(C.c_int32), _i,
                                C.POINTER(C.c_int32), _i, C.POINTER(C.c_int32), _vp, _i]),
    "ss_batch_mt_beam": (_i, [_vp, _vp, _i, _i, _vp, C.POINTER(C.c_int32), C.POINTER(C.c_int32), _i, _f, _i,
                              C.POINTER(C.c_int32), _i, C.POINTER(C.c_int32), C.POINTER(_f), C.POINTER(_f), _vp, _i]),
    "ss_batch_mt_continue": (_i, [_vp, _vp, _i, _vp, C.POINTER(C.c_int32), C.POINTER(C.c_int32), C.POINTER(C.c_int32),
                                  C.POINTER(C.c_int32), _i, C.POINTER(C.c_int32), _i, C.POINTER(C.c_int32), _vp, _i,
                                  C.POINTER(C.c_int32)]),
    "ss_batch_mt_continue_plan": (_i, [_i, C.POINTER(C.c_int32), C.POINTER(C.c_int32), C.POINTER(C.c_int32),
                                       C.POINTER(C.c_int32), _i, _i, _i, _i, _i, _i, C.POINTER(C.c_int32), C.POINTER(C.c_int32),
                                       _i64, C.POINTER(_i64)]),
    "ss_batch_mt_beam_continue": (_i, [_vp, _vp, _i, _i, _vp, C.POINTER(C.c_int32), C.POINTER(C.c_int32), C.POINTER(C.c_int32),
                                       C.POINTER(C.c_int32), _i, _f, _i, C.POINTER(C.c_int32), _i, C.POINTER(C.c_int32),
                                       C.POINTER(_f), C.POINTER(_f), _vp, _i]),
    "ss_batch_mt_beam_continue_plan": (_i, [_i, _i, C.POINTER(C.c_int32), C.POINTER(C.c_int32), C.POINTER(C.c_int32),
                                            C.POINTER(C.c_int32), _i, _i, _i, _i, _i, _i, _i, C.POINTER(C.c_int32),
                                            C.POINTER(C.c_int32), _i64, C.POINTER(_i64)]),
    "ss_batch_mt_beam_opts": (_i, [_vp, _vp, _i, _i, _vp, C.POINTER(C.c_int32), C.POINTER(C.c_int32), _i, _f, _i,
                                   C.POINTER(C.c_int32), _i, C.POINTER(C.c_int32), C.POINTER(_f), C.POINTER(_f), _vp, _i,
                                   C.POINTER(SSMtSearchOpts)]),
    "ss_batch_mt_beam_continue_opts": (_i, [_vp, _vp, _i, _i, _vp, C.POINTER(C.c_int32), C.POINTER(C.c_int32), C.POINTER(C.c_int32),
                                            C.POINTER(C.c_int32), _i, _f, _i, C.POINTER(C.c_int32), _i, C.POINTER(C.c_int32),
                                            C.POINTER(_f), C.POINTER(_f), _vp, _i, C.POINTER(SSMtSearchOpts)]),
    "ss_batch_mt_beam_continue_plan_opts": (_i, [_i, _i, C.POINTER(C.c_int32), C.POINTER(C.c_int32), C.POINTER(C.c_int32),
                                                 C.POINTER(C.c_int32), _i, _i, _i, _i, _i, _i, _i, C.POINTER(C.c_int32),
                                                 C.POINTER(C.c_int32), _i64, C.POINTER(_i64), C.POINTER(SSMtSearchOpts)]),
    "ss_batch_mt_sample": (_i, [_vp, _vp, _i, _i, _vp, C.POINTER(C.c_int32), C.POINTER(C.c_int32), _i, _f, _i,
                                C.POINTER(C.c_int32), _i, C.POINTER(C.c_int32), C.POINTER(_f), C.POINTER(_f), _vp, _i,
                                C.POINTER(SSMtSearchOpts), C.POINTER(_i64), C.POINTER(SSMtSampleOpts)]),
    "ss_batch_mt_sample_continue": (_i, [_vp, _vp, _i, _i, _vp, C.POINTER(C.c_int32), C.POINTER(C.c_int32), C.POINTER(C.c_int32),
                                         C.POINTER(C.c_int32), _i, _f, _i, C.POINTER(C.c_int32), _i, C.POINTER(C.c_int32),
                                         C.POINTER(_f), C.POINTER(_f), _vp, _i, C.POINTER(SSMtSearchOpts), C.POINTER(_i64),
                                         C.POINTER(SSMtSampleOpts)]),
    "ss_batch_fbank_frames": (_i, [_vp, _vp, _i, C.POINTER(_vp), C.POINTER(C.c_int32), C.POINTER(C.c_int32), _f,
                                   C.POINTER(_vp)]),
    "ss_batch_fbank_frames_sr": (_i, [_vp, _vp, _i, C.POINTER(_vp), C.POINTER(C.c_int32), C.POINTER(C.c_int32), C.POINTER(C.c_int32),
                                      C.POINTER(_vp), C.POINTER(C.c_int32), C.POINTER(C.c_int32), C.POINTER(C.c_int32), _f,
                                      C.POINTER(_vp)]),
    "ss_fbank_sr_rows": (_i, [_i64, _i, _i, _i, C.POINTER(C.c_int32), C.POINTER(C.c_int32)]),
    "ss_batch_t2u_units": (_i, [_vp, _vp, _i, _vp, _i, C.POINTER(C.c_int32), _i, _i, _vp, _vp, _vp]),
    "ss_batch_vocoder_forward": (_i, [_vp, _vp, _i, _vp, C.POINTER(C.c_int32), _i, _vp, _vp, _i64, _vp,
                                      C.POINTER(_i64), C.POINTER(_i64)]),
    "ss_batch_t2u_units_pad": (_i, [_vp, _vp, _i, _vp, _i, C.POINTER(C.c_int32), C.POINTER(C.c_int32), _i, _i, _vp, _vp, _vp]),
    "ss_batch_mt_features": (_i, [_vp, _vp, _i, _vp, C.POINTER(C.c_int32), C.POINTER(C.c_int32), C.POINTER(C.c_int32),
                                  C.POINTER(C.c_int32), _vp, _i]),
    "ss_batch_mt_attention": (_i, [_vp, _vp, _i, _vp, C.POINTER(C.c_int32), C.POINTER(C.c_int32), C.POINTER(C.c_int32),
                                   C.POINTER(C.c_int32), _vp, _i, _vp, C.POINTER(_i64), _i64, _vp, _vp]),
    "ss_batch_mt_score": (_i, [_vp, _vp, _i, _vp, C.POINTER(C.c_int32), _i, C.POINTER(C.c_int32), C.POINTER(C.c_int32),
                               C.POINTER(C.c_int32), _vp, _i, _vp, _vp]),
    "ss_batch_vocoder_tail": (_i, [_vp, _vp, _i, _vp, C.POINTER(C.c_int32), C.POINTER(C.c_int32), C.POINTER(C.c_int32),
                                   C.POINTER(C.c_int32), _i, _vp, _i64, C.POINTER(C.c_int32), C.POINTER(C.c_int32),
                                   C.POINTER(_i64), C.POINTER(_i64)]),
    "ss_batch_unit_spans": (_i, [_vp, _vp, _i, _vp, C.POINTER(C.c_int32), C.POINTER(C.c_int32), C.POINTER(C.c_int32),
                                 C.POINTER(C.c_int32), _vp, _vp, _vp, _vp]),
    "ss_unit_spans_host": (_i, [_i, _vp, C.POINTER(C.c_int32), C.POINTER(C.c_int32), C.POINTER(C.c_int32), C.POINTER(C.c_int32), _vp,
                                _i, _i, _i, _i, _i, _vp, _vp]),
    "ss_op_unit_spans": (_i, [_vp, _i, _vp, C.POINTER(C.c_int32), C.POINTER(C.c_int32), C.POINTER(C.c_int32), C.POINTER(C.c_int32),
                              _vp, _i, _i, _i, _i, _i, _vp, _vp]),
    "ss_prof_enable": (_i, [_i]),
    "ss_prof_enable_hi": (_i, [_i]),
    "ss_prof_reset": (_i, []),
    "ss_prof_read": (_i, [_i, C.POINTER(C.c_double), C.POINTER(C.c_double), C.POINTER(_i64), C.POINTER(C.c_double)]),
    "ss_prof_totals": (_i, [_i, C.POINTER(C.c_double), C.POINTER(C.c_double), C.POINTER(_i64)]),
    "ss_prof_read_issued": (_i, [_i, C.POINTER(C.c_double)]),
    "ss_prof_shape_log": (_i, [_i]),
    "ss_prof_shape_dump": (_i, [C.c_char_p, _i]),
    "ss_prof_num_classes": (_i, []),
    "ss_prof_class_name": (C.c_char_p, [_i]),
    "ss_debug_force_tile": (_i, [_i, _i, _i]),
    "ss_op_ffn_fused": (_i, [_vp, _vp, _i, _vp, _i, _vp, _vp, _vp, _vp, _vp, _vp, _f, _vp, _vp, _i, _i, _i]),
    "ss_debug_ffn": (_i, [_i, _i, _i]),
    "ss_debug_rtlin": (_i, [_i, _i]),
    "ss_debug_rtlin_kb": (_i, [_i, _i]),
    "ss_debug_rtlin_kb_last": (_i, [C.POINTER(C.c_int32)]),
    "ss_debug_unit_l0_distinct": (_i, [_i]),
    "ss_debug_fbank_dense": (_i, [_i]),
    "ss_fbank_mel_ranges": (_i, [_vp, _i, _i, C.POINTER(C.c_int32)]),
    "ss_debug_conv_c64": (_i, [_i]),
    "ss_debug_conv_c256_rows": (_i, [_i]),
    "ss_debug_conv_c32": (_i, [_i]),
    "ss_debug_conv_c16": (_i, [_i]),
    "ss_debug_enc_step_launches": (_i64, []),
    "ss_debug_scratch_audit": (_i, [_vp, C.POINTER(C.c_size_t), C.POINTER(C.c_size_t)]),
    "ss_op_ln_linear": (_i, [_vp, _vp, _i, _vp, _vp, _vp, _vp, _vp, _i, _vp, _i, _i, _i, _i, _i, _f, _i]),
    "ss_op_ln_linear_ex": (_i, [_vp, _vp, _i, _vp, _vp, _vp, _vp, _vp, _vp, _i, _vp, _i, _i, _i, _i, _i, _f, _i, _i]),
    "ss_debug_last_logits": (_i, [_vp, _vp, _vp, _i64, C.POINTER(_i), C.POINTER(_i)]),
    "ss_debug_sk_errors": (_i, []),
    "ss_debug_attention_split": (_i, [_i]),
    "ss_debug_attention_q16": (_i, [_i]),
    "ss_op_conv_gemm": (_i, [_vp, _vp, _i, _vp, _vp, _vp, _i, _vp, _i, _vp, _i, _i, _i, _i, _i, _i, _i, _i, _i, _i,
                             _i, _f, _i, _f, _f, _i]),
    "ss_op_conv_gemm_ex": (_i, [_vp, C.POINTER(SSOpConvArgs)]),
    "ss_op_conv_gemm_rows": (_i, [_vp, C.POINTER(SSOpConvArgs), _i, _vp, _vp, _i]),
    "ss_op_conv_pair": (_i, [_vp, _vp, _i, _vp, _vp, _vp, _vp, _vp, _i, _vp, _i, _f, _vp, _i, _f, _i, _i, _i, _i, _i, _f, _vp, _i]),
    "ss_op_resblock_fused": (_i, [_vp, _vp, _i, _vp, _vp, _vp, _vp, _vp, _vp, _i, _vp, _i, _f, _i, _i, _i, _f, _vp, _i]),
    "ss_debug_slab": (_i, [_i, C.c_longlong]),
    "ss_op_conv_f16": (_i, [_vp, _vp, _vp, _vp, _vp, _vp, _vp, _vp, _i, _i, _i, _i, _i, _f, _i, _f, _vp, _i]),
    "ss_op_layernorm": (_i, [_vp, _vp, _i, _vp, _i, _vp, _vp, _i, _i, _f]),
    "ss_op_attention": (_i, [_vp, _vp, _i, _vp, _i, _vp, _i, _vp, _i, _i, _i, _i, _f, _i, _i, _vp, _i, _vp, _vp]),
    "ss_op_attention_ex": (_i, [_vp, C.POINTER(SSOpAttnArgs)]),
    "ss_op_attention_probs": (_i, [_vp, C.POINTER(SSOpAttnProbsArgs)]),
    "ss_op_attention_pool": (_i, [_vp, C.POINTER(SSOpPoolAttnArgs)]),
    "ss_debug_attention_no_mfma": (_i, [_i]),
    "ss_op_dwconv_bn_silu": (_i, [_vp, _vp, _i, _vp, _i, _vp, _i, _vp, _vp, _vp, _vp, _f, _i, _i, _i]),
    "ss_op_dwconv_bn_silu_ex": (_i, [_vp, _vp, _i, _vp, _i, _vp, _i, _vp, _vp, _vp, _vp, _f, _i, _i, _i, _vp, _i, _i]),
    "ss_op_pool_dwconv": (_i, [_vp, _vp, _vp, _i, _vp, _vp, _i, _vp, _vp, _vp, _vp, _f, _i, _vp, _i, _i]),
    "ss_op_pool_gather_rows": (_i, [_vp, _vp, _vp, _vp, _i, _i, _vp, _vp, _i, _i]),
    "ss_op_pool_gather_ids": (_i, [_vp, _vp, _vp, _vp, _i, _vp, _vp, _i, _i]),
    "ss_op_pool_stack_rows": (_i, [_vp, _vp, _vp, _i, _vp, _vp, _i, _i]),
    "ss_op_masked_argmax": (_i, [_vp, _vp, _i, _i, _i, _i, _i, _i, _i, _vp, _vp, _i, _i, _vp, _i]),
    "ss_op_ctc_collapse": (_i, [_vp, _vp, _i, _i, _i, _vp, _vp, _vp, _vp, _i]),
    "ss_op_masked_argmax_lprob": (_i, [_vp, _vp, _i, _i, _i, _i, _i, _i, _vp, _vp]),
    "ss_op_mt_token_scores": (_i, [_vp, _vp, _i, _i, _i, _vp, _vp, _vp]),
    "ss_debug_mt_score_form": (_i, [_i]),
    "ss_op_ctc_collapse_spans": (_i, [_vp, _vp, _vp, _i, _i, _i, _vp, _vp, _vp, _vp, _vp, _vp, _i]),
    "ss_op_ctc_align": (_i, [_vp, _vp, _i, _i, _i, _i, C.POINTER(C.c_int32), C.POINTER(C.c_int32), C.POINTER(C.c_int32), _vp, _vp, _vp,
                             _vp, _vp, _vp]),
    "ss_op_dur_predict": (_i, [_vp, _vp, _vp, _i, _vp, _vp, _vp, _i]),
    "ss_op_repeat_rows": (_i, [_vp, _vp, _vp, _i, _i, _vp, _i, _vp, _i]),
    "ss_op_embed_tokens": (_i, [_vp, _vp, _vp, _vp, _f, _i, _vp, _i, _i, _i, _i, _i]),
    "ss_op_embed_tokens_rows": (_i, [_vp, _vp, _vp, _vp, _i, _f, _i, _vp, _vp, _i, _i, _i, _i]),
    "ss_op_upsample_add_pos": (_i, [_vp, _vp, _i, _i, _vp, _f, _vp, _i]),
    "ss_op_gather_rows": (_i, [_vp, _vp, _vp, _i, _vp, _i, _i]),
    "ss_op_scatter_rows": (_i, [_vp, _vp, _vp, _i, _vp, _i, _i, _i, _i]),
    "ss_op_conv_post_tanh": (_i, [_vp, _vp, _i, _i, _vp, _vp, _f, _vp, _vp, _i]),
    "ss_op_conv_post_tanh_crop": (_i, [_vp, _vp, _i, _vp, _vp, _f, _vp, _vp, _i, _i]),
    "ss_op_spkr_pre_add": (_i, [_vp, _vp, _vp, _i, _i, _vp, _vp, _i, _vp, _i, _i, _i, _i, _f]),
    "ss_op_beam_topk": (_i, [_vp, _vp, _i, _i, _i, _i, _i, _vp, _vp, _vp, _vp, _i, _i, _i, _f, _vp, _vp]),
    "ss_op_beam_merge": (_i, [_vp, C.POINTER(SSOpBeamState), _i, _i, _i, _i, _i, _i, _i, _i]),
    "ss_op_beam_prefix_score": (_i, [_vp, _vp, _i, _i, _vp, _i, _i, _f, _vp]),
    "ss_op_beam_prefix_chain": (_i, [_vp, _vp, _vp, _vp, _i, _i, _vp, _vp]),
    "ss_op_beam_topk_opts": (_i, [_vp, _vp, _i, _i, _i, _i, _i, _vp, _vp, _vp, _vp, _i, _i, _i, _f, _vp, _vp, _f, _i, _vp, _vp, _i, _i,
                                  _vp, _vp, _vp]),
    "ss_op_beam_merge_opts": (_i, [_vp, C.POINTER(SSOpBeamState), _i, _i, _i, _i, _i, _i, _i, _i, _f]),
    "ss_op_beam_prefix_score_opts": (_i, [_vp, _vp, _i, _i, _vp, _i, _i, _f, _vp, _f]),
    "ss_op_sample_step": (_i, [_vp, _vp, _i, _i, _i, _i, _vp, _vp, _i, _i, _i, _f, _f, _i, _vp, _vp, _i, _i, _vp, _vp, _vp, _vp,
                               C.POINTER(SSMtSampleOpts), _vp, _vp, _vp, _vp]),
    "ss_op_sample_uniform": (_i, [_vp, _i, _vp, _vp, _vp, _vp, _vp, _vp]),
}

_lib = None


SS_ERR_ARG = 2
SS_ERR_CAPACITY = 4
SS_ERR_SCRATCH_CAP = 5
SS_ERR_STREAM_REPEAT = 8


class StreamSpeechHipError(RuntimeError):

    def __init__(self, msg, code=None):
        super().__init__(msg)
        self.code = code


def load():
    global _lib
    if _lib is not None:
        return _lib
    if not os.path.exists(LIB_PATH):
        raise StreamSpeechHipError(
            f"{LIB_PATH} not found: build it with streamspeech_amd/csrc/build.sh "
            "(or __graft_entry__.build()).  There is no CPU fallback for the product path.")
    import torch
    lib = C.CDLL(LIB_PATH)
    for name, (res, args) in SIGNATURES.items():
        try:
            fn = getattr(lib, name)
        except AttributeError as e:
            raise StreamSpeechHipError(f"{LIB_PATH} does not export {name}") from e
        fn.restype = res
        fn.argtypes = args
    if lib.ss_abi_version() != 2:
        raise StreamSpeechHipError("ABI version mismatch")
    _lib = lib
    return lib


def check(rc: int, what: str = ""):
    if rc != 0:
        msg = load().ss_error_string(rc).decode()
        raise StreamSpeechHipError(f"{what} failed: {msg} (code {rc})", rc)
```

Before: 6549.

## Fuse both 64-channel Winograd resblock convolutions into one slab kernel

Adds a kernel that runs both convolutions of a 64-channel HiFi-GAN resblock in one launch. The first conv's LeakyReLU output stays in LDS as a halo-extended slab and feeds the second conv directly, and the next block's input is prefetched during the second contraction. This removes a launch and the global write and read of the intermediate activation. In exchange, halo rows are recomputed, the kernel uses a large LDS footprint with one workgroup per CU, and it is enabled only for taps 3 and 7 through a default mask.

Result: no change. 6569, median of 4 (+0.3%).

```diff
diff --git a/include/streamspeech_hip.h b/include/streamspeech_hip.h
--- a/include/streamspeech_hip.h
+++ b/include/streamspeech_hip.h
@@ -481,6 +481,7 @@
 int ss_debug_fbank_dense(int dense);
 int ss_debug_conv_c64(int enable);
 int ss_debug_conv_c256_rows(int rows);
+int ss_debug_conv_c64_pair(int mask);
 int ss_debug_conv_c32(int enable);
 int ss_debug_conv_c16(int enable);
 int64_t ss_debug_enc_step_launches(void);
@@ -518,6 +519,9 @@
 int ss_op_conv_pair(void* stream, const float* dA, int lda, const float* dW1, const float* db1, const float* dW2, const float* db2,
                     float* dC, int ldc, const float* dR2, int ldr2, float div, float* dC2, int ldc2, float c2_slope, int C, int taps,
                     int dil, int M, int in_len, float slope, const int32_t* d_segs, int nseg);
+int ss_op_conv_c64w_pair(void* stream, const float* dA, int lda, const float* dW1, const float* db1, const float* dW2, const float* db2,
+                         float* dC, int ldc, const float* dR2, int ldr2, float div, int C, int taps, int dil, int M, int in_len,
+                         float slope, const int32_t* d_segs, int nseg);
 int ss_op_resblock_fused(void* stream, const float* dX, int ldx, const float* const* dW1, const float* const* dB1,
                          const float* const* dW2, const float* const* dB2, const int32_t* dil, float* dY, int ldy, const float* dR2,
                          int ldr2, float div, int C, int taps, int M, float slope, const int32_t* d_segs, int nseg);
diff --git a/streamspeech_amd/csrc/conv_c64w.hip b/streamspeech_amd/csrc/conv_c64w.hip
--- a/streamspeech_amd/csrc/conv_c64w.hip
+++ b/streamspeech_amd/csrc/conv_c64w.hip
@@ -369,6 +369,317 @@
   if (!conv_c64_eligible(a) || !conv_c64w_eligible(a)) return SS_ERR_ARG;
   return launch_cw<64>(a, stream);
 }
+
+namespace {
+constexpr int CWP_MAXROWS = 288;
+constexpr int cwp_halo(int taps, int dil) { return 2 * dil * (((taps - 1) / 2 + 2 * dil - 1) / (2 * dil)); }
+constexpr int cwp_bme(int taps, int dil) { return (256 - 2 * cwp_halo(taps, dil)) / (2 * dil) * (2 * dil); }
+constexpr int cwp_xrows(int taps, int dil) { return cwp_bme(taps, dil) + 2 * cwp_halo(taps, dil) + 3 * ((taps + 2) / 3) * dil; }
+constexpr size_t cwp_lds(int taps, int dil) {
+  return (size_t)(cwp_xrows(taps, dil) + cwp_bme(taps, dil) + 2 * cwp_halo(taps, dil)) * 68 * sizeof(float) + (CW_MAXSEG + 2) * sizeof(int);
+}
+constexpr bool cwp_fits(int taps, int dil) { return cwp_xrows(taps, dil) <= CWP_MAXROWS && cwp_lds(taps, dil) <= 160 * 1024 && cwp_bme(taps, dil) > 0; }
+static_assert(cwp_bme(3, 1) == 252 && cwp_bme(7, 1) == 248 && cwp_bme(11, 1) == 244 && cwp_bme(3, 3) == 240 && cwp_bme(11, 3) == 240 &&
+              cwp_bme(3, 5) == 230, "block heights of the fused pair");
+static_assert(cwp_fits(3, 1) && cwp_fits(7, 1) && cwp_fits(11, 1) && cwp_fits(3, 3) && cwp_fits(7, 3) && cwp_fits(11, 3) && cwp_fits(3, 5),
+              "both slabs and the segment table fit one CU's LDS, slab X the staging passes");
+}
+
+template <int DIL, int TAIL>
+__global__ __launch_bounds__(512, 1) void conv_c64w_pair_kernel(const GemmArgs p, const float* __restrict__ W1, const float* __restrict__ b1,
+                                                                 const int groups, const int xrows, const int bme, const int hl) {
+#if __HIP_DEVICE_COMPILE__
+  constexpr int C = 64, LDA = C + 4, CT = 2, CB = C / 16, RING = 2 * CT, TPR = C / 4, NT = 512, RPP = NT / TPR;
+  constexpr int NP = CWP_MAXROWS / RPP;
+  static_assert(NP * RPP == CWP_MAXROWS, "whole staging passes");
+  const int trows = bme + 2 * hl;
+  const int npair1 = trows / 2, npair2 = bme / 2;
+  const int halo2 = (p.taps - 1) / 2;
+  extern __shared__ __attribute__((aligned(16))) float smem[];
+  float* sX = smem;
+  float* sT = smem + xrows * LDA;
+  int* s_blk = reinterpret_cast<int*>(sT + trows * LDA);
+
+  const int t = threadIdx.x, lane = t & 63;
+  const int pq = __builtin_amdgcn_readfirstlane((t >> 6) & 3);
+  const int col0 = __builtin_amdgcn_readfirstlane(t >> 8) * 32;
+  const int r = lane & 15, g = lane >> 4;
+  const int Kw = groups * 4 * C;
+
+  SlabWalk<GemmArgs> w(p, s_blk, bme);
+  __syncthreads();
+  const int nblocks = w.nblocks();
+  const float slope = p.in_slope;
+
+  const __amdgpu_buffer_rsrc_t rsW1 = __builtin_amdgcn_make_buffer_rsrc((void*)W1, 0, CW_NUM_RECORDS, 0x00020000);
+  const __amdgpu_buffer_rsrc_t rsW2 = __builtin_amdgcn_make_buffer_rsrc((void*)p.W, 0, CW_NUM_RECORDS, 0x00020000);
+  const int vo = (r * Kw + 4 * g) * 4;
+  auto wload = [&](const __amdgpu_buffer_rsrc_t rs, int idx, int cc, int ct) -> f32x4 {
+    const int so = __builtin_amdgcn_readfirstlane(((col0 + ct * 16) * Kw + idx * C + cc * 16) * 4);
+    const u32x4 v = __builtin_amdgcn_raw_buffer_load_b128(rs, vo, so, 0);
+    return f32x4{__uint_as_float(v[0]), __uint_as_float(v[1]), __uint_as_float(v[2]), __uint_as_float(v[3])};
+  };
+
+  int blk = (int)blockIdx.x;
+  if (blk >= nblocks) return;
+  f32x4 ring[RING];
+#pragma unroll
+  for (int q = 0; q < RING; ++q) ring[q] = wload(rsW1, q / CT, 0, q % CT);
+
+  int toff1[2], toff2[2];
+  bool pv1[2], pv2[2];
+#pragma unroll
+  for (int i = 0; i < 2; ++i) {
+    const int pp = pq * 32 + i * 16 + r;
+    pv1[i] = pp < npair1;
+    pv2[i] = pp < npair2;
+    const int pc1 = pv1[i] ? pp : npair1 - 1, pc2 = pv2[i] ? pp : npair2 - 1;
+    toff1[i] = 2 * DIL * (pc1 / DIL) + pc1 % DIL;
+    toff2[i] = 2 * pc2;
+  }
+
+  f32x4 pre[NP];
+  auto slab_request = [&](int x0, int lo, int hi) __attribute__((always_inline)) {
+#pragma unroll
+    for (int u = 0; u < NP; ++u) {
+      const int gc = min(max(x0 + t / TPR + RPP * u, lo), hi - 1);
+      pre[u] = *reinterpret_cast<const f32x4*>(p.A + (size_t)gc * p.lda + (t % TPR) * 4);
+    }
+  };
+  auto slab_write = [&](int x0, int lo, int hi) __attribute__((always_inline)) {
+    const bool edge = (x0 < lo) || (x0 + xrows > hi);
+    float* dst = sX + (t / TPR) * LDA + (t % TPR) * 4;
+#pragma unroll
+    for (int u = 0; u < NP; ++u) {
+      const int rho = t / TPR + RPP * u;
+      f32x4 v = pre[u];
+      if (edge) {
+        const int gin = x0 + rho;
+        const bool ok = gin >= lo && gin < hi;
+#pragma unroll
+        for (int e = 0; e < 4; ++e) v[e] = ok ? v[e] : 0.f;
+      }
+#pragma unroll
+      for (int e = 0; e < 4; ++e) v[e] = fmaxf(v[e], v[e] * slope);
+      if (rho < xrows) *reinterpret_cast<f32x4*>(dst + u * RPP * LDA) = v;
+    }
+  };
+  w.locate(blk, p.in_len);
+  slab_request(w.m0 - hl - p.pad, w.seg_lo, w.seg_hi);
+  slab_write(w.m0 - hl - p.pad, w.seg_lo, w.seg_hi);
+
+  for (;;) {
+    const int m0 = w.m0, seg_lo = w.seg_lo, seg_hi = w.seg_hi;
+    const int m_hi = p.nseg > 0 ? seg_hi : min(seg_hi, p.M);
+    const int blk_next = blk + (int)gridDim.x;
+    const bool more_blocks = blk_next < nblocks;
+    __syncthreads();
+
+    f32x4 acc[4][2][CT];
+    f32x4 xa[2];
+    auto contract = [&](auto DILC, const float* pa0, const float* pa1, const __amdgpu_buffer_rsrc_t rs,
+                        const __amdgpu_buffer_rsrc_t rs_after) __attribute__((always_inline)) {
+      constexpr int DX = decltype(DILC)::value;
+#pragma unroll
+      for (int f = 0; f < 4; ++f)
+#pragma unroll
+        for (int i = 0; i < 2; ++i)
+#pragma unroll
+          for (int j = 0; j < CT; ++j) acc[f][i][j] = f32x4{0.f, 0.f, 0.f, 0.f};
+      auto rd = [&](const float* base, int j, int cc) -> f32x4 { return *reinterpret_cast<const f32x4*>(base + j * DX * LDA + cc * 16); };
+      auto xform = [&](int op, const f32x4 a, const f32x4 b) -> f32x4 { return op == 1 ? a + b : op == 0 ? a : a - b; };
+      xa[0] = xform(-1, rd(pa0, 0, 0), rd(pa0, 2, 0));
+      xa[1] = xform(-1, rd(pa1, 0, 0), rd(pa1, 2, 0));
+      auto group = [&](auto KIND, const int grp, const int kind_next, const float* pn0, const float* pn1, const int grp_next,
+                       const __amdgpu_buffer_rsrc_t rs_next) __attribute__((always_inline)) {
+        constexpr int K = decltype(KIND)::value, NC = cw_nc(K), NS = CB * NC;
+        static_assert(NS % 2 == 0 && NS >= 2, "ring slots keep their parity across groups");
+#pragma unroll
+        for (int ss = 0; ss < NS; ++ss) {
+          const int slot = cw_slot(K, ss % NC);
+          f32x4 na0, nb0, na1, nb1;
+          if (ss + 1 < NS) {
+            const int ccn = (ss + 1) / NC, nn = (ss + 1) % NC;
+            na0 = rd(pa0, cw_ja(K, nn), ccn); nb0 = rd(pa0, cw_jb(K, nn), ccn);
+            na1 = rd(pa1, cw_ja(K, nn), ccn); nb1 = rd(pa1, cw_jb(K, nn), ccn);
+          } else {
+            const int jb = kind_next == 0 ? 2 : 1;
+            na0 = rd(pn0, 0, 0); nb0 = *reinterpret_cast<const f32x4*>(pn0 + jb * (DX * LDA));
+            na1 = rd(pn1, 0, 0); nb1 = *reinterpret_cast<const f32x4*>(pn1 + jb * (DX * LDA));
+          }
+          f32x4 wf[CT];
+#pragma unroll
+          for (int j = 0; j < CT; ++j) {
+            const int q = ss * CT + j;
+            wf[j] = ring[q % RING];
+            const int s2 = ss + 2;
+            if (s2 < NS) ring[q % RING] = wload(rs, grp * 4 + cw_slot(K, s2 % NC), s2 / NC, j);
+            else ring[q % RING] = wload(rs_next, grp_next * 4 + (s2 == NS ? 0 : (kind_next == 1 ? 3 : 1)), 0, j);
+          }
+#pragma unroll
+          for (int e = 0; e < 4; ++e)
+#pragma unroll
+            for (int i = 0; i < 2; ++i)
+#pragma unroll
+              for (int j = 0; j < CT; ++j)
+                acc[slot][i][j] = __builtin_amdgcn_mfma_f32_16x16x4f32(wf[j][e], xa[i][e], acc[slot][i][j], 0, 0, 0);
+          if (ss + 1 < NS) {
+            xa[0] = xform(cw_op(K, (ss + 1) % NC), na0, nb0);
+            xa[1] = xform(cw_op(K, (ss + 1) % NC), na1, nb1);
+          } else {
+            xa[0] = kind_next == 1 ? na0 : na0 - nb0;
+            xa[1] = kind_next == 1 ? na1 : na1 - nb1;
+          }
+          __builtin_amdgcn_sched_barrier(0);
+        }
+      };
+      const int groups_full = groups - (TAIL ? 1 : 0);
+#pragma unroll 1
+      for (int grp = 0; grp + 1 < groups; ++grp) {
+        const float* pn0 = pa0 + 3 * DX * LDA;
+        const float* pn1 = pa1 + 3 * DX * LDA;
+        group(std::integral_constant<int, 0>{}, grp, grp + 1 == groups_full ? TAIL : 0, pn0, pn1, grp + 1, rs);
+        pa0 = pn0;
+        pa1 = pn1;
+      }
+      group(std::integral_constant<int, TAIL>{}, groups - 1, 0, pa0, pa1, 0, rs_after);
+    };
+
+    contract(std::integral_constant<int, DIL>{}, sX + toff1[0] * LDA + 4 * g, sX + toff1[1] * LDA + 4 * g, rsW1, rsW2);
+
+    {
+      f32x4 bb[CT];
+#pragma unroll
+      for (int j = 0; j < CT; ++j) bb[j] = b1 ? *reinterpret_cast<const f32x4*>(b1 + col0 + j * 16 + 4 * g) : f32x4{0.f, 0.f, 0.f, 0.f};
+#pragma unroll
+      for (int i = 0; i < 2; ++i) {
+        const int gr0 = m0 - hl + toff1[i], gr1 = gr0 + DIL;
+        const bool ok0 = gr0 >= seg_lo && gr0 < seg_hi, ok1 = gr1 >= seg_lo && gr1 < seg_hi;
+        float* d0 = sT + toff1[i] * LDA + col0 + 4 * g;
+#pragma unroll
+        for (int j = 0; j < CT; ++j) {
+          f32x4 y0 = (acc[0][i][j] + acc[1][i][j]) + acc[2][i][j];
+          f32x4 y1 = (acc[1][i][j] - acc[2][i][j]) - acc[3][i][j];
+          y0 += bb[j];
+          y1 += bb[j];
+#pragma unroll
+          for (int e = 0; e < 4; ++e) {
+            y0[e] = ok0 ? fmaxf(y0[e], y0[e] * slope) : 0.f;
+            y1[e] = ok1 ? fmaxf(y1[e], y1[e] * slope) : 0.f;
+          }
+          if (pv1[i]) {
+            *reinterpret_cast<f32x4*>(d0 + j * 16) = y0;
+            *reinterpret_cast<f32x4*>(d0 + DIL * LDA + j * 16) = y1;
+          }
+        }
+      }
+    }
+    __syncthreads();
+    int nx0 = 0, nlo = 0, nhi = 0;
+    if (more_blocks) {
+      w.locate(blk_next, p.in_len);
+      nx0 = w.m0 - hl - p.pad; nlo = w.seg_lo; nhi = w.seg_hi;
+      slab_request(nx0, nlo, nhi);
+    }
+
+    contract(std::integral_constant<int, 1>{}, sT + (toff2[0] + hl - halo2) * LDA + 4 * g, sT + (toff2[1] + hl - halo2) * LDA + 4 * g, rsW2, rsW1);
+
+    if (more_blocks) slab_write(nx0, nlo, nhi);
+
+    int le = lane;
+    asm volatile("" : "+v"(le));
+    const int cole = col0 + (le >> 4) * 4;
+    f32x4 y[4 * CT];
+    int mrow[4];
+#pragma unroll
+    for (int i = 0; i < 2; ++i) {
+#pragma unroll
+      for (int j = 0; j < CT; ++j) {
+        y[(i * 2) * CT + j] = (acc[0][i][j] + acc[1][i][j]) + acc[2][i][j];
+        y[(i * 2 + 1) * CT + j] = (acc[1][i][j] - acc[2][i][j]) - acc[3][i][j];
+      }
+      mrow[i * 2] = m0 + toff2[i];
+      mrow[i * 2 + 1] = m0 + toff2[i] + 1;
+    }
+#pragma unroll
+    for (int n = 0; n < 4 * CT; ++n) asm volatile("" : "+v"(y[n]));
+    f32x4 bb[CT];
+#pragma unroll
+    for (int j = 0; j < CT; ++j) bb[j] = f32x4{0.f, 0.f, 0.f, 0.f};
+    if (p.bias) {
+#pragma unroll
+      for (int j = 0; j < CT; ++j) bb[j] = *reinterpret_cast<const f32x4*>(p.bias + cole + j * 16);
+    }
+    slab_epi_batch(p, y, bb, [&](int q, int n) -> size_t {
+      return (size_t)min(mrow[n / CT], m_hi - 1) * (q == 0 ? p.ldr : p.ldr2) + cole + (n % CT) * 16;
+    });
+#pragma unroll
+    for (int q = 0; q < 4; ++q) {
+      if (pv2[q / 2] && mrow[q] < m_hi) {
+#pragma unroll
+        for (int j = 0; j < CT; ++j) slab_epi_store<false>(p, mrow[q], cole + j * 16, y[q * CT + j]);
+      }
+    }
+    if (!more_blocks) break;
+    blk = blk_next;
+  }
+#endif
+}
+
+static int cwp_bit(int taps) { return taps == 3 ? 1 : taps == 7 ? 2 : taps == 11 ? 4 : 0; }
+static void cwp_two_launches(const ConvC64wPairArgs& x, GemmArgs& a1, GemmArgs& a2) {
+  GemmArgs a;
+  a.lda = x.lda; a.ldc = a.ldr = x.lda; a.ldr2 = x.ldr2; a.M = x.M; a.in_len = x.in_len; a.N = a.Cin = x.ch; a.taps = x.taps; a.stride = 1;
+  a.same_rows = 1; a.in_act = ACT_LRELU; a.in_slope = x.slope; a.segs = x.segs; a.nseg = x.nseg;
+  a1 = a; a1.dil = x.dil; a1.pad = x.dil * (x.taps - 1) / 2; a1.Wwino = x.W1w; a1.bias = x.b1;
+  a2 = a; a2.dil = 1; a2.pad = (x.taps - 1) / 2; a2.Wwino = x.W2w; a2.bias = x.b2; a2.R = x.A; a2.R2 = x.R2; a2.div = x.div; a2.ldc = x.ldc;
+}
+bool conv_c64w_pair_eligible(const ConvC64wPairArgs& x) {
+  if (x.ch != 64 || !(disp().c64_pair_mask & cwp_bit(x.taps)) || (x.dil != 1 && x.dil != 3 && x.dil != 5)) return false;
+  if (!x.A || !x.C || x.A == x.C || !x.W1w || !x.W2w || x.M != x.in_len || !(x.slope > 0.f && x.slope < 1.f)) return false;
+  if (x.nseg < 0 || (x.nseg > 0 && !x.segs)) return false;
+  GemmArgs a1, a2;
+  cwp_two_launches(x, a1, a2);
+  if (!conv_c64_eligible(a1) || !conv_c64w_eligible(a1) || !conv_c64_eligible(a2) || !conv_c64w_eligible(a2)) return false;
+  return cwp_fits(x.taps, x.dil);
+}
+
+template <int DIL, int TAIL>
+static int launch_cwp_t(const ConvC64wPairArgs& x, hipStream_t stream) {
+  const int groups = (x.taps + 2) / 3, bme = cwp_bme(x.taps, x.dil), hl = cwp_halo(x.taps, x.dil), xrows = cwp_xrows(x.taps, x.dil);
+  const size_t lds = cwp_lds(x.taps, x.dil);
+  SS_MAX_LDS_ONCE((&conv_c64w_pair_kernel<DIL, TAIL>), 160 * 1024);
+  SkWorkspace* st = nullptr;
+  int rc = sk_workspace_acquire(stream, &st);
+  if (rc != SS_OK) return rc;
+  const int grid = slab_grid(1, st->cus, x.M, bme, x.nseg);
+  GemmArgs a1, p;
+  cwp_two_launches(x, a1, p);
+  p.A = x.A; p.W = x.W2w; p.C = x.C;
+  p.algo_flops = 2.0 * 2.0 * (double)x.M * 64 * x.taps * 64;
+  p.algo_bytes = 4.0 * (2.0 * (64.0 * x.taps * 64 + 64) + (double)x.M * 64 * (3 + (x.R2 ? 1 : 0)));
+  ProfRec rec{}; bool prof = false;
+  rc = prof_begin(p, stream, PROF_CONV_C64W_PAIR, rec, prof);
+  if (rc != SS_OK) return rc;
+  p.pad = a1.pad; p.dil = a1.dil;
+  hipLaunchKernelGGL((conv_c64w_pair_kernel<DIL, TAIL>), dim3(grid), dim3(512), lds, stream, p, x.W1w, x.b1, groups, xrows, bme, hl);
+  SS_LAUNCH_CHECK();
+  return prof_end(stream, rec, prof);
+}
+
+int launch_conv_c64w_pair(const ConvC64wPairArgs& x, hipStream_t stream) {
+  if (!conv_c64w_pair_eligible(x)) return SS_ERR_ARG;
+  switch (x.dil * 10 + x.taps % 3) {
+    case 10: return launch_cwp_t<1, 0>(x, stream);
+    case 11: return launch_cwp_t<1, 1>(x, stream);
+    case 12: return launch_cwp_t<1, 2>(x, stream);
+    case 30: return launch_cwp_t<3, 0>(x, stream);
+    case 31: return launch_cwp_t<3, 1>(x, stream);
+    case 32: return launch_cwp_t<3, 2>(x, stream);
+    case 50: return launch_cwp_t<5, 0>(x, stream);
+    default: return SS_ERR_ARG;
+  }
+}
 void conv_c32w_debug(int enable) { if (enable >= 0) dispatch_edit([enable](Dispatch& d) { d.c32w_on = enable ? 1 : 0; }); }
 bool conv_c32w_enabled() { return disp().c32w_on != 0; }
 bool conv_c32w_eligible(const GemmArgs& a) {
diff --git a/streamspeech_amd/csrc/debug_ops.hip b/streamspeech_amd/csrc/debug_ops.hip
--- a/streamspeech_amd/csrc/debug_ops.hip
+++ b/streamspeech_amd/csrc/debug_ops.hip
@@ -61,6 +61,24 @@
   return launch_conv_pair(dA, lda, dW1, db1, dW2, db2, dC, ldc, dR2, ldr2, div, dC2, ldc2, c2_slope, Cch, taps, dil, M, in_len, slope,
                           d_segs, nseg, (hipStream_t)stream);
 }
+extern "C" int ss_op_conv_c64w_pair(void* stream, const float* dA, int lda, const float* dW1, const float* db1, const float* dW2,
+                                    const float* db2, float* dC, int ldc, const float* dR2, int ldr2, float div, int Cch, int taps,
+                                    int dil, int M, int in_len, float slope, const int32_t* d_segs, int nseg) {
+  static thread_local std::map<hipStream_t, DevBuf> wino_tmps;
+  DevBuf& wt = wino_tmps[(hipStream_t)stream];
+  if (!dW1 || !dW2 || Cch != 64 || taps < 3 || taps > 11) return SS_ERR_ARG;
+  const size_t nw = (size_t)64 * ((taps + 2) / 3) * 4 * 64;
+  ConvC64wPairArgs x;
+  x.A = dA; x.lda = lda; x.b1 = db1; x.b2 = db2; x.C = dC; x.ldc = ldc; x.R2 = dR2; x.ldr2 = ldr2; x.div = div;
+  x.ch = Cch; x.taps = taps; x.dil = dil; x.M = M; x.in_len = in_len; x.slope = slope; x.segs = d_segs; x.nseg = nseg;
+  x.W1w = dW1; x.W2w = dW2;
+  if (!conv_c64w_pair_eligible(x)) return SS_ERR_ARG;
+  RET(wt.ensure(2 * nw * sizeof(float)));
+  RET(launch_wino_pack(dW1, wt.f(), 64, taps, (hipStream_t)stream));
+  RET(launch_wino_pack(dW2, wt.f() + nw, 64, taps, (hipStream_t)stream));
+  x.W1w = wt.f(); x.W2w = wt.f() + nw;
+  return launch_conv_c64w_pair(x, (hipStream_t)stream);
+}
 extern "C" int ss_op_resblock_fused(void* stream, const float* dX, int ldx, const float* const* dW1, const float* const* dB1,
                                     const float* const* dW2, const float* const* dB2, const int32_t* dil, float* dY, int ldy,
                                     const float* dR2, int ldr2, float div, int Cch, int taps, int M, float slope,
@@ -141,6 +159,11 @@
   return SS_OK;
 }
 extern "C" int ss_debug_conv_c256_rows(int rows) { return conv_c256w_rows_debug(rows); }
+extern "C" int ss_debug_conv_c64_pair(int mask) {
+  if (mask > 7) return SS_ERR_ARG;
+  conv_c64w_pair_debug(mask);
+  return SS_OK;
+}
 extern "C" int ss_debug_conv_c32(int enable) {
   if (enable == 4 || enable == 5) { conv_c32w_debug(enable == 5); return SS_OK; }
   conv_c32_debug(enable);
diff --git a/streamspeech_amd/csrc/dispatch.hip b/streamspeech_amd/csrc/dispatch.hip
--- a/streamspeech_amd/csrc/dispatch.hip
+++ b/streamspeech_amd/csrc/dispatch.hip
@@ -34,6 +34,7 @@
   d.no_sk2 = I("SS_NO_SK2", 0) ? 1 : 0; d.sk2_min_k64 = I("SS_SK2_MINK64", d.sk2_min_k64); d.sk2_spare_cus = I("SS_SK2_SPARE_CUS", 0);
   d.rt_wg_per_cu = I("SS_RTLIN_WG_PER_CU", 0); d.c32_min_k = I("SS_CONV_C32_MIN_K", d.c32_min_k); d.c16_min_k = I("SS_CONV_C16_MIN_K", d.c16_min_k);
   d.unit_l0_distinct = I("SS_UNIT_L0_DISTINCT", 1) ? 1 : 0; d.fbank_dense = I("SS_FBANK_DENSE", 0) ? 1 : 0;
+  d.c64_pair_mask = I("SS_CONV_C64_PAIR", d.c64_pair_mask) & 7;
   return d;
 }
 Dispatch& process_settings() { static Dispatch d = env_defaults(); return d; }
@@ -54,6 +55,10 @@
     d.c64_min_rows = set ? min_rows : dflt.c64_min_rows;
     d.c128w_min_rows = set ? min_rows : dflt.c128w_min_rows; d.c256w_min_rows = set ? min_rows : dflt.c256w_min_rows;
   });
+}
+void conv_c64w_pair_debug(int mask) {
+  const int dflt = env_defaults().c64_pair_mask;
+  dispatch_edit([=](Dispatch& d) { d.c64_pair_mask = mask < 0 ? dflt : (mask & 7); });
 }
 int conv_c256w_rows_debug(int rows) {
   if (rows != 0 && rows != 128 && rows != 256) return SS_ERR_ARG;
diff --git a/streamspeech_amd/csrc/dispatch.hpp b/streamspeech_amd/csrc/dispatch.hpp
--- a/streamspeech_amd/csrc/dispatch.hpp
+++ b/streamspeech_amd/csrc/dispatch.hpp
@@ -14,6 +14,7 @@
   long long c128w_min_rows = 65536, c256w_min_rows = 32768;
   int c256w_rows = 128;
   int c32_min_k = 7, c16_min_k = 11;
+  int c64_pair_mask = 3;
   int slab_grid_cap = 0;
   int sk_groups = 0;
   int sk2_spare_cus = 0;
diff --git a/streamspeech_amd/csrc/gemm.hpp b/streamspeech_amd/csrc/gemm.hpp
--- a/streamspeech_amd/csrc/gemm.hpp
+++ b/streamspeech_amd/csrc/gemm.hpp
@@ -122,6 +122,19 @@
 int launch_wino_pack(const float* W, float* WW, int C, int taps, hipStream_t stream);
 void conv_c64w_debug(int enable);
 bool conv_c64w_enabled();
+struct ConvC64wPairArgs {
+  const float* A = nullptr; int lda = 0;
+  const float *W1w = nullptr, *b1 = nullptr;
+  const float *W2w = nullptr, *b2 = nullptr;
+  float* C = nullptr; int ldc = 0;
+  const float* R2 = nullptr; int ldr2 = 0; float div = 0.f;
+  int ch = 64, taps = 3, dil = 1, M = 0, in_len = 0;
+  float slope = 0.1f;
+  const int* segs = nullptr; int nseg = 0;
+};
+bool conv_c64w_pair_eligible(const ConvC64wPairArgs& x);
+int launch_conv_c64w_pair(const ConvC64wPairArgs& x, hipStream_t stream);
+void conv_c64w_pair_debug(int mask);
 bool conv_wide_winograd_eligible(const GemmArgs& a, int ch);
 int launch_conv_c128w(const GemmArgs& a, hipStream_t stream);
 void conv_c128w_debug(int enable);
diff --git a/streamspeech_amd/csrc/prof.hip b/streamspeech_amd/csrc/prof.hip
--- a/streamspeech_amd/csrc/prof.hip
+++ b/streamspeech_amd/csrc/prof.hip
@@ -20,7 +20,7 @@
     "smallm_gemm<4,1>", "smallm_gemm<2,2>", "smallm_gemm<1,4>", "conv_sk<128,BN,32>",
     "conv_slab<32>", "conv_slab<16>", "conv_sk2<256,128,32>", "conv_sk2_bf16x3<256,128,32>",
     "resblock_fused<32>", "resblock_fused<16>", "ffn_fused<256,2048>", "rt_linear<48,256>", "conv_c64<256,64>", "conv_c32<256,32>", "conv_c16<256,16>", "conv_c64w<256,64>", "conv_c128w<256,128>", "conv_c32w<256,32>", "conv_c256w<256,128>", "rt_linear_kb<48,256>",
-    "conv_f16<64>", "conv_f16<128>", "conv_f16<256>"};
+    "conv_f16<64>", "conv_f16<128>", "conv_f16<256>", "conv_c64w_pair<64>"};
 static_assert(sizeof(kTileNames) / sizeof(kTileNames[0]) == kNumTileCfg, "one name per ProfCls, in enum order");
 static std::atomic<int> g_prof_mask{0};
 static std::atomic<int> g_prof_mask_hi{0};
@@ -110,7 +110,7 @@
   if (a.algo_bytes > 0) bytes = a.algo_bytes;
 }
 
-static bool prof_cls_winograd(ProfCls cls) { return cls >= PROF_CONV_C64W && cls <= PROF_CONV_C256W; }
+static bool prof_cls_winograd(ProfCls cls) { return (cls >= PROF_CONV_C64W && cls <= PROF_CONV_C256W) || cls == PROF_CONV_C64W_PAIR; }
 
 int prof_begin(const GemmArgs& a, hipStream_t stream, ProfCls cls, ProfRec& rec, bool& prof) {
   {
diff --git a/streamspeech_amd/csrc/prof.hpp b/streamspeech_amd/csrc/prof.hpp
--- a/streamspeech_amd/csrc/prof.hpp
+++ b/streamspeech_amd/csrc/prof.hpp
@@ -16,8 +16,9 @@
   PROF_CONV_C64W = 27, PROF_CONV_C128W = 28, PROF_CONV_C32W = 29, PROF_CONV_C256W = 30,
   PROF_RTLIN_KB = 31,
   PROF_CONV_F16_64 = 32, PROF_CONV_F16_128 = 33, PROF_CONV_F16_256 = 34,
+  PROF_CONV_C64W_PAIR = 35,
 };
-constexpr int kNumTileCfg = PROF_CONV_F16_256 + 1;
+constexpr int kNumTileCfg = PROF_CONV_C64W_PAIR + 1;
 void prof_enable(int cls_mask);
 void prof_enable_hi(int cls_mask);
 void prof_reset();
diff --git a/streamspeech_amd/csrc/vocoder.hip b/streamspeech_amd/csrc/vocoder.hip
--- a/streamspeech_amd/csrc/vocoder.hip
+++ b/streamspeech_amd/csrc/vocoder.hip
@@ -341,7 +341,20 @@
           cur = out;
           continue;
         }
-        const float* rin = dd == 0 ? b.bs : b.br;
+        if (c64 && C == 64 && !pa && !f16 && gnseg > 0) {
+          ConvC64wPairArgs x;
+          x.A = cur; x.lda = C; x.W1w = v->rb_c1[idx].ww; x.b1 = v->rb_c1[idx].b; x.W2w = v->rb_c2[idx].ww; x.b2 = v->rb_c2[idx].b;
+          x.C = dd == 2 ? b.bx : (cur == b.br ? b.br2 : b.br); x.ldc = C;
+          x.R2 = (dd == 2 && j > 0) ? b.bx : nullptr; x.ldr2 = C;
+          x.div = (dd == 2 && j == c.n_res - 1) ? (float)c.n_res : 0.f;
+          x.ch = C; x.taps = kr; x.dil = c.resblock_dilations[j][dd]; x.M = x.in_len = gM; x.slope = 0.1f; x.segs = gsegs; x.nseg = gnseg;
+          if (conv_c64w_pair_eligible(x)) {
+            RET(launch_conv_c64w_pair(x, s));
+            cur = x.C;
+            continue;
+          }
+        }
+        const float* rin = pa ? (dd == 0 ? b.bs : b.br) : cur;
         const float* rin_act = dd == 0 ? b.bsa : b.bra;
         GemmArgs a1 = mk(pa ? rin_act : rin, C, v->rb_c1[idx], C, kr, c.resblock_dilations[j][dd], b.bt, C);
         if (pa) { a1.act = ACT_LRELU; a1.act_slope = 0.1f; }
@@ -358,6 +371,7 @@
           if (pa_next && j == c.n_res - 1) a2.C2 = b.bxa;
         }
         RET(conv(a2, scale));
+        cur = a2.C;
       }
     }
   }
diff --git a/streamspeech_amd/lib.py b/streamspeech_amd/lib.py
--- a/streamspeech_amd/lib.py
+++ b/streamspeech_amd/lib.py
@@ -316,6 +316,7 @@
     "ss_fbank_mel_ranges": (_i, [_vp, _i, _i, C.POINTER(C.c_int32)]),
     "ss_debug_conv_c64": (_i, [_i]),
     "ss_debug_conv_c256_rows": (_i, [_i]),
+    "ss_debug_conv_c64_pair": (_i, [_i]),
     "ss_debug_conv_c32": (_i, [_i]),
     "ss_debug_conv_c16": (_i, [_i]),
     "ss_debug_enc_step_launches": (_i64, []),
@@ -331,6 +332,7 @@
     "ss_op_conv_gemm_ex": (_i, [_vp, C.POINTER(SSOpConvArgs)]),
     "ss_op_conv_gemm_rows": (_i, [_vp, C.POINTER(SSOpConvArgs), _i, _vp, _vp, _i]),
     "ss_op_conv_pair": (_i, [_vp, _vp, _i, _vp, _vp, _vp, _vp, _vp, _i, _vp, _i, _f, _vp, _i, _f, _i, _i, _i, _i, _i, _f, _vp, _i]),
+    "ss_op_conv_c64w_pair": (_i, [_vp, _vp, _i, _vp, _vp, _vp, _vp, _vp, _i, _vp, _i, _f, _i, _i, _i, _i, _i, _f, _vp, _i]),
     "ss_op_resblock_fused": (_i, [_vp, _vp, _i, _vp, _vp, _vp, _vp, _vp, _vp, _i, _vp, _i, _f, _i, _i, _i, _f, _vp, _i]),
     "ss_debug_slab": (_i, [_i, C.c_longlong]),
     "ss_op_conv_f16": (_i, [_vp, _vp, _vp, _vp, _vp, _vp, _vp, _vp, _i, _i, _i, _i, _i, _f, _i, _f, _vp, _i]),
```
